# sauloal/pykmer

Measured on AMD Instinct MI355X. Metric: bp/s k-mer counted (k=15, 1 GPU), higher is better.
Workload: dtype u8; 1 GPU; k=15 canonical k-mer count of one 800 Mbp synthetic genome per GPU (SURVEY 8d C2, seed 2+rank), 4^15 table resident in HBM; fasta_bytes=813333854, num_kmers=766212116, parallelism=1 independent genome(s)

## Files before the change

pykmer_amd/csrc/kmer_count.hip:

```cpp
#include "fasta_fsm.h"
#include "pk_kernels.h"

namespace pk {

constexpr int L2_WAVES = 7;

__global__ __launch_bounds__(WG) void k_chunk_l1(const uint8_t *__restrict__ fasta, uint64_t n_bytes, uint32_t n_chunks,
                                                 L1 *__restrict__ chunk_l1) {
    const uint32_t lane = threadIdx.x & 63u;
    const uint32_t chunk = blockIdx.x * (WG / 64) + (threadIdx.x >> 6);
    if (chunk >= n_chunks) return;
    const uint64_t base = (uint64_t)chunk * CHUNK;
    const uint32_t nb = (uint32_t)(n_bytes - base < (uint64_t)CHUNK ? n_bytes - base : (uint64_t)CHUNK);
    auto window = [&](uint32_t w) -> uint32_t {
        const uint32_t off = w * 256u + lane * 4u;
        if (off + 4u <= nb) return *reinterpret_cast<const uint32_t *>(fasta + base + off);
        uint32_t v = 0;
        for (uint32_t j = 0; off + j < nb && j < 4u; j++) v |= (uint32_t)fasta[base + off + j] << (8u * j);
        return v;
    };
    const uint32_t n_win = (nb + 255u) / 256u;
    int last_term = -1;
    for (int w = (int)n_win - 1; w >= 0 && last_term < 0; w--) {
        const uint32_t v = window((uint32_t)w);
        uint32_t tm = 0;
#pragma unroll
        for (uint32_t j = 0; j < 4; j++) tm |= is_term((v >> (8u * j)) & 0xffu) ? (1u << j) : 0u;
        const unsigned long long any = __ballot(tm != 0u);
        if (any) {
            const int hl = 63 - __builtin_clzll(any);
            const uint32_t tmh = (uint32_t)__builtin_amdgcn_readlane((int)tm, hl);
            last_term = w * 256 + hl * 4 + (31 - __builtin_clz(tmh));
        }
    }
    const uint32_t from = (uint32_t)(last_term + 1);
    uint32_t state = LS_START;
    bool found = false;
    for (uint32_t w = from / 256u; w < n_win && !found; w++) {
        const uint32_t v = window(w);
        uint32_t nz = 0;
#pragma unroll
        for (uint32_t j = 0; j < 4; j++) {
            const uint32_t idx = w * 256u + lane * 4u + j;
            nz |= (idx >= from && idx < nb && !is_ws((v >> (8u * j)) & 0xffu)) ? (1u << j) : 0u;
        }
        const unsigned long long any = __ballot(nz != 0u);
        if (any) {
            const int ll = __builtin_ctzll(any);
            const uint32_t m = (uint32_t)__builtin_amdgcn_readlane((int)nz, ll);
            const uint32_t word = (uint32_t)__builtin_amdgcn_readlane((int)v, ll);
            const uint32_t c = (word >> (8u * (uint32_t)__builtin_ctz(m))) & 0xffu;
            state = c == '>' ? (uint32_t)LS_HEADER : (uint32_t)LS_SEQ;
            found = true;
        }
    }
    if (lane == 0) chunk_l1[chunk] = nb ? l1_make(last_term >= 0, state) : 0u;
}

__global__ __launch_bounds__(WG, L2_WAVES) void k_chunk_l2(const uint8_t *__restrict__ fasta, uint64_t n_bytes,
                                                 const L1 *__restrict__ chunk_l1_state, L2 *__restrict__ chunk_l2,
                                                 LaneState *__restrict__ lane_state, PiecePack *__restrict__ packs,
                                                 uint32_t *__restrict__ chunk_odd, uint32_t km1) {
    __shared__ __attribute__((aligned(16))) uint8_t lds[WG * LDS_STRIDE];
    __shared__ L1 sh1[WG / 64];
    __shared__ L2 sh2[WG / 64];
    __shared__ uint16_t queue[WG];
    __shared__ uint32_t n_queued[2], n_header_pieces;
    __shared__ uint32_t res1[WG];
    __shared__ uint8_t ls_of[WG];
    const uint64_t base = (uint64_t)blockIdx.x * CHUNK;
    if (threadIdx.x < 2) n_queued[threadIdx.x] = 0;
    if (threadIdx.x == 2) n_header_pieces = 0;
    stage_chunk(fasta, base, n_bytes, lds);
    __syncthreads();
    const uint32_t nb = piece_len(base, n_bytes);
    const uint8_t *mine = lds + threadIdx.x * LDS_STRIDE;
    PieceMasks pm;
    PiecePack pk;
    uint32_t cw[4];
    piece_scan(mine, nb, pm, cw);
    const bool full = nb == (uint32_t)PIECE;
    const bool plain = (pm.blank | pm.gt) == 0ull;
    {
        const unsigned long long S = ~pm.term;
        piece_compact(pm.valid, S & ~pm.valid, cw, plain, (uint32_t)__popcll(S), (S & 1ull) != 0ull, pk);
        uint4 *dst = reinterpret_cast<uint4 *>(packs + (uint64_t)blockIdx.x * WG + threadIdx.x);
        dst[0] = make_uint4((uint32_t)pk.c_lo, (uint32_t)(pk.c_lo >> 32), (uint32_t)pk.c_hi, (uint32_t)(pk.c_hi >> 32));
        dst[1] = make_uint4((uint32_t)pk.restart, (uint32_t)(pk.restart >> 32), pk.meta, 0u);
    }
    const bool masks1 = full && lines_start_plain(pm);
    L1 my1 = l1_of_piece(pm);
    bool dirty = !plain;
    const bool q1 = !masks1;
    if (q1) queue[atomicAdd(&n_queued[0], 1u)] = (uint16_t)threadIdx.x;
    __syncthreads();
    for (uint32_t q0 = (threadIdx.x >> 6) * 64u; q0 < n_queued[0]; q0 += WG) {
        const uint32_t qi = q0 + (threadIdx.x & 63u);
        const bool work = qi < n_queued[0];
        const uint32_t pc = work ? queue[qi] : 0u;
        bool d;
        const L1 r = piece_l1_at(lds + pc * LDS_STRIDE, work ? piece_len_of(pc, base, n_bytes) : 0u, d);
        if (work) res1[pc] = r | (d ? 0x100u : 0u);
    }
    __syncthreads();
    if (q1) { my1 = res1[threadIdx.x] & 0xffu; dirty = (res1[threadIdx.x] >> 8) & 1u; }
    L1 tot1;
    const L1 st1 = wg_excl_scan_l1(my1, chunk_l1_state[blockIdx.x], sh1, &tot1);
    const uint32_t ls_in = l1_kind(st1);
    ls_of[threadIdx.x] = (uint8_t)ls_in;
    const bool clean = !dirty && ls_in != LS_HEADER;
    bool header_piece = false;
    unsigned long long H = 0;
    if (__any(!clean && masks1)) {
        H = header_text(pm, ls_in);
        header_piece = !clean && masks1 && first_byte_plain(pm, ls_in) && (pm.blank & ~H) == 0ull;
    }
    L2 my2 = l2_identity();
    if (clean) my2 = l2_of_clean_piece(pm, pk, nb, ls_in, km1);
    if (__any(header_piece)) {
        const unsigned long long seq = ~pm.term & ~H, valid = pm.valid & seq;
        PiecePack hk;
        piece_compact(header_piece ? valid : 0ull, header_piece ? ((seq & ~valid) | H) : 0ull, cw, true, 0u, false, hk);
        if (header_piece)
            my2 = l2_of_masks(pm.term, valid, (seq & ~valid) | H, seq, (uint32_t)__popcll(header_starts(pm, ls_in)), hk, nb, ls_in, km1);
    }
    const bool q2 = !clean && !header_piece;
    if (q2) queue[atomicAdd(&n_queued[1], 1u)] = (uint16_t)threadIdx.x;
    const unsigned long long hp_wave = __ballot(header_piece);
    if ((threadIdx.x & 63u) == 0u && hp_wave) atomicAdd(&n_header_pieces, (uint32_t)__popcll(hp_wave));
    __syncthreads();
    for (uint32_t q0 = (threadIdx.x >> 6) * 64u; q0 < n_queued[1]; q0 += WG) {
        const uint32_t qi = q0 + (threadIdx.x & 63u);
        const bool work = qi < n_queued[1];
        const uint32_t pc = work ? queue[qi] : 0u;
        const L2 r = piece_l2_at(lds + pc * LDS_STRIDE, work ? piece_len_of(pc, base, n_bytes) : 0u, ls_of[pc], km1);
        if (work) {
            uint32_t *out = reinterpret_cast<uint32_t *>(lds + pc * LDS_STRIDE);
            out[0] = r.flags; out[1] = r.bits; out[2] = r.rec; out[3] = (uint32_t)r.p_tail;
        }
    }
    __syncthreads();
    if (q2) {
        const uint32_t *in = reinterpret_cast<const uint32_t *>(mine);
        my2.flags = in[0]; my2.bits = in[1]; my2.rec = in[2]; my2.p_tail = in[3];
    }
    L2 total;
    const L2 rel = wg_excl_scan_l2(my2, l2_identity(), sh2, &total, km1);
    lane_state[(uint64_t)blockIdx.x * WG + threadIdx.x] = lane_state_pack(rel, ls_in, q2, header_piece);
    if (threadIdx.x == 0) {
        chunk_l2[blockIdx.x] = total;
        chunk_odd[blockIdx.x] = n_queued[1] + n_header_pieces;
    }
}

constexpr int SCAN_T = 1024;

template <typename S, class Compose, class Shfl>
__device__ __forceinline__ S tile_scan(const S &mine, const S &seed, S *sh, S *total, Compose compose, Shfl shfl_up1) {
    const int lane = threadIdx.x & 63, w = threadIdx.x >> 6;
    S inc = mine;
#pragma unroll
    for (int d = 1; d < 64; d <<= 1) {
        S o = shfl_up1(inc, d);
        if (lane >= d) inc = compose(o, inc);
    }
    if (lane == 63) sh[w] = inc;
    __syncthreads();
    S pre = seed, tot = seed;
    for (int j = 0; j < SCAN_T / 64; j++) { if (j == w) pre = tot; tot = compose(tot, sh[j]); }
    *total = tot;
    S up = shfl_up1(inc, 1);
    return lane == 0 ? pre : compose(pre, up);
}

__global__ __launch_bounds__(SCAN_T) void k_scan_l1_reduce(const L1 *__restrict__ in, uint32_t n, L1 *__restrict__ tile_tot) {
    __shared__ L1 sh[SCAN_T / 64];
    const uint32_t i = blockIdx.x * SCAN_T + threadIdx.x;
    L1 tot;
    tile_scan<L1>(i < n ? in[i] : 0u, 0u, sh, &tot, [](L1 a, L1 b) { return l1_compose(a, b); }, [](L1 v, int d) { return (L1)__shfl_up(v, d, 64); });
    if (threadIdx.x == 0) tile_tot[blockIdx.x] = tot;
}
__global__ __launch_bounds__(SCAN_T) void k_scan_l1_tiles(L1 *__restrict__ tile_tot, uint32_t n_tiles, Carry *carry, uint32_t *__restrict__ zero_words,
                                                          uint32_t n_zero) {
    __shared__ L1 sh[SCAN_T / 64];
    if (threadIdx.x < n_zero) zero_words[threadIdx.x] = 0u;
    L1 run = carry->l1;
    for (uint32_t t0 = 0; t0 < n_tiles; t0 += SCAN_T) {
        const uint32_t i = t0 + threadIdx.x;
        L1 tot;
        L1 ex = tile_scan<L1>(i < n_tiles ? tile_tot[i] : 0u, run, sh, &tot, [](L1 a, L1 b) { return l1_compose(a, b); },
                              [](L1 v, int d) { return (L1)__shfl_up(v, d, 64); });
        if (i < n_tiles) tile_tot[i] = ex;
        run = tot;
        __syncthreads();
    }
    if (threadIdx.x == 0) carry->l1 = run;
}
__global__ __launch_bounds__(SCAN_T) void k_scan_l1_apply(const L1 *__restrict__ in, uint32_t n, const L1 *__restrict__ tile_seed,
                                                          L1 *__restrict__ out_state) {
    __shared__ L1 sh[SCAN_T / 64];
    const uint32_t i = blockIdx.x * SCAN_T + threadIdx.x;
    L1 tot;
    L1 ex = tile_scan<L1>(i < n ? in[i] : 0u, tile_seed[blockIdx.x], sh, &tot, [](L1 a, L1 b) { return l1_compose(a, b); },
                          [](L1 v, int d) { return (L1)__shfl_up(v, d, 64); });
    if (i < n) out_state[i] = ex;
}

__global__ __launch_bounds__(SCAN_T) void k_scan_l2_reduce(const L2 *__restrict__ in, uint32_t n, L2 *__restrict__ tile_tot, uint32_t km1) {
    __shared__ L2 sh[SCAN_T / 64];
    const uint32_t i = blockIdx.x * SCAN_T + threadIdx.x;
    L2 tot;
    tile_scan<L2>(i < n ? in[i] : l2_identity(), l2_identity(), sh, &tot, [km1](const L2 &a, const L2 &b) { return l2_compose(a, b, km1); },
                  [](const L2 &v, int d) { return shfl_up_l2(v, d); });
    if (threadIdx.x == 0) tile_tot[blockIdx.x] = tot;
}
__global__ __launch_bounds__(SCAN_T) void k_scan_l2_tiles(L2 *__restrict__ tile_tot, uint32_t n_tiles, Carry *carry, uint32_t km1) {
    __shared__ L2 sh[SCAN_T / 64];
    L2 run = carry->l2;
    for (uint32_t t0 = 0; t0 < n_tiles; t0 += SCAN_T) {
        const uint32_t i = t0 + threadIdx.x;
        L2 tot;
        L2 ex = tile_scan<L2>(i < n_tiles ? tile_tot[i] : l2_identity(), run, sh, &tot,
                              [km1](const L2 &a, const L2 &b) { return l2_compose(a, b, km1); }, [](const L2 &v, int d) { return shfl_up_l2(v, d); });
        if (i < n_tiles) tile_tot[i] = ex;
        run = tot;
        __syncthreads();
    }
    if (threadIdx.x == 0) { carry->l2 = run; carry->n_recs = run.rec; if (km1 > 16u) carry->deep_in = carry->deep_out; }
}
__global__ __launch_bounds__(SCAN_T) void k_scan_l2_apply(const L2 *__restrict__ in, uint32_t n, const L2 *__restrict__ tile_seed,
                                                          L2 *__restrict__ out_state, uint32_t km1) {
    __shared__ L2 sh[SCAN_T / 64];
    const uint32_t i = blockIdx.x * SCAN_T + threadIdx.x;
    L2 tot;
    L2 ex = tile_scan<L2>(i < n ? in[i] : l2_identity(), tile_seed[blockIdx.x], sh, &tot,
                          [km1](const L2 &a, const L2 &b) { return l2_compose(a, b, km1); }, [](const L2 &v, int d) { return shfl_up_l2(v, d); });
    if (i < n) out_state[i] = ex;
}

__global__ __launch_bounds__(WG) void k_hist(const uint8_t *__restrict__ src, uint64_t n, unsigned long long *__restrict__ hist ) {
    __shared__ uint32_t h[WG / 64][256];
    for (int i = threadIdx.x; i < (WG / 64) * 256; i += WG) (&h[0][0])[i] = 0;
    __syncthreads();
    uint32_t *myh = h[threadIdx.x >> 6];
    uint64_t ones = 0;
    const uint64_t n16 = n / 16;
    for (uint64_t g = (uint64_t)blockIdx.x * WG + threadIdx.x; g < n16; g += (uint64_t)gridDim.x * WG) {
        const uint4 a = reinterpret_cast<const uint4 *>(src)[g];
        const uint32_t t[4] = {a.x, a.y, a.z, a.w};
#pragma unroll
        for (int j = 0; j < 16; j++) {
            const uint32_t v = (t[j >> 2] >> (8 * (j & 3))) & 0xffu;
            if (v == 1u) ones++;
            else if (v) atomicAdd(&myh[v], 1u);
        }
    }
    if (blockIdx.x == 0) {
        for (uint64_t i = n16 * 16 + threadIdx.x; i < n; i += WG) {
            const uint32_t x = src[i];
            if (x == 1u) ones++;
            else if (x) atomicAdd(&myh[x], 1u);
        }
    }
    for (int d = 32; d; d >>= 1) ones += __shfl_down((unsigned long long)ones, d, 64);
    if ((threadIdx.x & 63) == 0 && ones) atomicAdd(&hist[1], (unsigned long long)ones);
    __syncthreads();
    for (int b = threadIdx.x; b < 256; b += WG) {
        unsigned long long s = 0;
        for (int w = 0; w < WG / 64; w++) s += h[w][b];
        if (s) atomicAdd(&hist[b], s);
    }
}

void launch_chunk_l1(const uint8_t *fasta, uint64_t n, L1 *chunk_l1, uint32_t n_chunks, hipStream_t s) {
    hipLaunchKernelGGL(k_chunk_l1, dim3((n_chunks + WG / 64 - 1) / (WG / 64)), dim3(WG), 0, s, fasta, n, n_chunks, chunk_l1);
}
void launch_scan_l1(const L1 *in, uint32_t n_chunks, Carry *carry, L1 *out, L1 *tile_ws, PartSignals *zeroed, hipStream_t s) {
    static_assert(sizeof(PartSignals) % 4 == 0 && sizeof(PartSignals) / 4 <= SCAN_T, "k_scan_l1_tiles zeroes one word per thread");
    const uint32_t n_tiles = (n_chunks + SCAN_T - 1) / SCAN_T;
    hipLaunchKernelGGL(k_scan_l1_reduce, dim3(n_tiles), dim3(SCAN_T), 0, s, in, n_chunks, tile_ws);
    hipLaunchKernelGGL(k_scan_l1_tiles, dim3(1), dim3(SCAN_T), 0, s, tile_ws, n_tiles, carry, (uint32_t *)zeroed, (uint32_t)(sizeof(PartSignals) / 4));
    hipLaunchKernelGGL(k_scan_l1_apply, dim3(n_tiles), dim3(SCAN_T), 0, s, in, n_chunks, (const L1 *)tile_ws, out);
}
void launch_chunk_l2(const uint8_t *fasta, uint64_t n, const L1 *st1, L2 *chunk_l2, LaneState *lane_state, PiecePack *packs, uint32_t *chunk_odd, uint32_t n_chunks,
                     uint32_t k, hipStream_t s) {
    hipLaunchKernelGGL(k_chunk_l2, dim3(n_chunks), dim3(WG), 0, s, fasta, n, st1, chunk_l2, lane_state, packs, chunk_odd, k - 1);
}
void launch_scan_l2(const L2 *in, uint32_t n_chunks, Carry *carry, L2 *out, L2 *tile_ws, uint32_t k, hipStream_t s) {
    const uint32_t n_tiles = (n_chunks + SCAN_T - 1) / SCAN_T;
    hipLaunchKernelGGL(k_scan_l2_reduce, dim3(n_tiles), dim3(SCAN_T), 0, s, in, n_chunks, tile_ws, k - 1);
    hipLaunchKernelGGL(k_scan_l2_tiles, dim3(1), dim3(SCAN_T), 0, s, tile_ws, n_tiles, carry, k - 1);
    hipLaunchKernelGGL(k_scan_l2_apply, dim3(n_tiles), dim3(SCAN_T), 0, s, in, n_chunks, (const L2 *)tile_ws, out, k - 1);
}
static uint32_t stream_grid(uint64_t items_per_thread_units) {
    uint64_t g = (items_per_thread_units + WG - 1) / WG;
    if (g > 256u * 8u) g = 256u * 8u;
    if (g == 0) g = 1;
    return (uint32_t)g;
}
void launch_hist8(const uint8_t *table8, uint64_t n, unsigned long long *hist, hipStream_t s) {
    hipLaunchKernelGGL(k_hist, dim3(stream_grid(n / 16 + 1)), dim3(WG), 0, s, table8, n, hist);
}

}
```

pykmer_amd/csrc/kmer_fuse.hip:

```cpp
#include "part_common.h"

namespace pk {

__device__ __forceinline__ uint32_t smear_up(uint32_t x, uint32_t n) {
    const uint32_t y1 = x | (x << 1), y2 = y1 | (y1 << 2), y3 = y2 | (y2 << 4);
    if (n >= 16u) return y3 | (y3 << 8);
    uint32_t acc = 0, off = 0;
    if (n & 8u) { acc |= y3; off = 8; }
    if (n & 4u) { acc |= y2 << off; off += 4; }
    if (n & 2u) { acc |= y1 << off; off += 2; }
    if (n & 1u) { acc |= x << off; }
    return acc;
}

__device__ __forceinline__ unsigned long long bases_before_slot(const uint32_t *__restrict__ codes, const uint32_t *__restrict__ n_bases, uint32_t c,
                                                                const unsigned long long *__restrict__ stream_before) {
    unsigned long long before = 0;
    uint32_t have = 0;
    for (uint32_t cc = c; cc > 0 && have < 32u;) {
        cc--;
        const uint32_t n_cc = n_bases[cc];
        const uint32_t take = min(n_cc, 32u - have);
        if (take == 0) continue;
        const uint32_t p0 = n_cc - take, d0 = p0 >> 4, sh = 2u * (p0 & 15u);
        const uint32_t *pw = codes + (uint64_t)cc * SLOT_CODE_WORDS;
        const unsigned long long w01 = ((unsigned long long)pw[min(d0 + 1u, SLOT_CODE_WORDS - 1u)] << 32) | pw[d0];
        const unsigned long long w2 = pw[min(d0 + 2u, SLOT_CODE_WORDS - 1u)];
        unsigned long long x = sh ? ((w01 >> sh) | (w2 << (64u - sh))) : w01;
        if (take < 32u) x &= (1ull << (2u * take)) - 1ull;
        before |= x << (2u * (32u - have - take));
        have += take;
    }
    if (have < 32u) before |= *stream_before >> (2u * have);
    return before;
}

__global__ void k_deep_tail(const uint32_t *__restrict__ codes, const uint32_t *__restrict__ n_bases, uint32_t n_chunks,
                            const unsigned long long *__restrict__ before_in, unsigned long long *__restrict__ before_out,
                            const uint32_t *__restrict__ flags) {
    if (threadIdx.x != 0 || flags[0]) return;
    *before_out = bases_before_slot(codes, n_bases, n_chunks, before_in);
}

template <typename KT, bool COUNT, int NT, int PER, int NB, uint32_t HS, bool SLICED, bool DEEP, uint32_t KC = 0>
__global__ __launch_bounds__(NT, 4) void k_walk_sort(const uint32_t *__restrict__ codes, const uint32_t *__restrict__ restarts,
                                                  const uint32_t *__restrict__ n_bases, const L2 *__restrict__ chunk_l2_state,
                                                  PartPlan pl, uint32_t n_items, uint32_t stride, void *__restrict__ out,
                                                  uint32_t *__restrict__ cursor1, const uint32_t *__restrict__ cap_end, uint32_t dump,
                                                  uint32_t *__restrict__ flags, uint32_t tally_shift, uint32_t n_tally,
                                                  uint32_t *__restrict__ tally_rows, unsigned long long *__restrict__ side,
                                                  unsigned long long *__restrict__ side_n, uint64_t side_cap,
                                                  const unsigned long long *__restrict__ deep_before) {
    static_assert(NT * PER == TILE && PER % 16 == 0, "one slot per workgroup");
    static_assert(!DEEP || (PER == 16 && sizeof(KT) == 8 && SLICED), "deep windows: 64-bit k-mers, one code dword per thread, sliced table");
    constexpr int NW = PER / 16;
    constexpr bool WIDE = sizeof(KT) == 8;
    extern __shared__ __attribute__((aligned(16))) uint8_t smem[];
    ScatterLdsT<NB> &L = *reinterpret_cast<ScatterLdsT<NB> *>(smem);
    uint32_t *tally = reinterpret_cast<uint32_t *>(smem);
    __shared__ HotTable<COUNT ? 2u : HS> hot;
    const uint32_t k = KC ? KC : pl.k, km1 = k - 1;
    if (COUNT && flags[0]) return;
    if (COUNT) {
        for (uint32_t i = threadIdx.x; i < n_tally; i += NT) tally[i] = 0u;
    } else {
        for (uint32_t i = threadIdx.x; i < HS; i += NT) { hot.key[i] = 0ull; hot.val[i] = 0u; }
        if (threadIdx.x == 0) { hot.used = 0; L.pad_[1] = flags[0]; }
        for (uint32_t i = threadIdx.x; i < NB; i += NT) { L.hist[i] = 0; L.run[i] = 0; }
    }
    const uint32_t B = KC == 17 ? 512u : pl.B1, shift = KC == 17 ? 25u : pl.addr_bits - pl.b1;
    const uint32_t low_mask = shift >= 32 ? 0xffffffffu : ((1u << shift) - 1u);
    const bool out16 = KC == 17 ? false : pl.b2 == 0;
    const KT mask = (KT)((2u * k >= sizeof(KT) * 8u) ? ~(KT)0 : (((KT)1 << (2u * k)) - 1));
    const KT local_mask = (KT)((pl.addr_bits >= sizeof(KT) * 8u) ? ~(KT)0 : (((KT)1 << pl.addr_bits) - 1));
    uint32_t t = threadIdx.x;
    __syncthreads();
    if (!COUNT && L.pad_[1]) return;
    const uint32_t i_lo = COUNT ? blockIdx.x : blockIdx.x * pl.G1, i_hi = COUNT ? n_items : min(i_lo + pl.G1, n_items);
    const uint32_t i_step = COUNT ? gridDim.x : 1u;
    struct Fetched { uint32_t nb, prev0, pprev0, r_here, r_before, st_flags, st_bits, cur[NW]; };
    auto fetch = [&](uint32_t c, uint32_t t, Fetched &f) {
        const uint32_t *cw = codes + (uint64_t)c * SLOT_CODE_WORDS;
        const uint32_t *rw = restarts + (uint64_t)c * SLOT_RST_WORDS;
        f.nb = n_bases[c];
#pragma unroll
        for (int w = 0; w < NW; w++) f.cur[w] = cw[NW * t + w];
        f.prev0 = cw[t ? NW * t - 1 : 0];
        f.pprev0 = cw[NW * t > 1 ? NW * t - 2 : 0];
        const uint32_t ri = NW == 2 ? t : (t >> 1);
        f.r_here = rw[ri];
        f.r_before = rw[ri ? ri - 1 : 0];
        f.st_flags = chunk_l2_state[c].flags;
        f.st_bits = chunk_l2_state[c].bits;
    };
    Fetched nxt;
    auto settle = [&]() {
        __builtin_amdgcn_s_waitcnt(0x0F70);
        asm volatile("" : "+v"(nxt.nb), "+v"(nxt.prev0), "+v"(nxt.pprev0), "+v"(nxt.r_here), "+v"(nxt.r_before), "+v"(nxt.st_flags), "+v"(nxt.st_bits));
#pragma unroll
        for (int w = 0; w < NW; w++) asm volatile("" : "+v"(nxt.cur[w]));
    };
    auto locate = [&](uint32_t it, uint32_t &c, uint32_t &tt) -> bool {
        if (!COUNT) { c = it; tt = threadIdx.x; return true; }
        constexpr uint32_t WPW = NT / 64;
        const uint64_t g = (uint64_t)it * WPW + (threadIdx.x >> 6);
        const uint64_t q = stride == 1u ? g : g * stride + g % stride;
        c = (uint32_t)(q / WPW); tt = (uint32_t)(q % WPW) * 64u + (threadIdx.x & 63u);
        return q / WPW < pl.n_chunks;
    };
    uint32_t c_n = 0, t_n = threadIdx.x;
    bool ok_n = false;
    if (i_lo < i_hi) { ok_n = locate(i_lo, c_n, t_n); if (ok_n) fetch(c_n, t_n, nxt); }
    settle();
    for (uint32_t it = i_lo; it < i_hi; it += i_step) {
        const Fetched me = nxt;
        const uint32_t c = c_n;
        const bool ok = ok_n;
        if (COUNT) t = t_n;
        if (it + i_step < i_hi) { ok_n = locate(it + i_step, c_n, t_n); if (ok_n) fetch(c_n, t_n, nxt); }
        if (COUNT && !ok) { settle(); continue; }
        const uint32_t nb = (uint32_t)__builtin_amdgcn_readfirstlane((int)me.nb);
        if (nb == 0) { settle(); continue; }
        const bool live = (uint32_t)PER * t < nb;
        uint32_t cur[NW], prev0 = me.prev0, rbits[NW];
#pragma unroll
        for (int w = 0; w < NW; w++) { cur[w] = live ? me.cur[w] : 0u; rbits[w] = 0; }
        if (NW == 2) {
            rbits[0] = (me.r_here << 16) | (me.r_before >> 16);
            rbits[NW - 1] = me.r_here;
        } else {
            rbits[0] = (t & 1u) ? me.r_here : ((me.r_here << 16) | (me.r_before >> 16));
        }
        uint32_t pprev0 = me.pprev0;
        bool have_pp[NW];
        if (NW == 2) {
            have_pp[0] = t != 0 && ((me.r_before >> 13) & 7u) == 0u;
            have_pp[NW - 1] = t != 0 && ((me.r_before >> 29) & 7u) == 0u;
        } else {
            const unsigned long long rb = ((((unsigned long long)me.r_here) << 32) | me.r_before) >> (16u * (t & 1u));
            have_pp[0] = t > 1 && (((uint32_t)rb >> 13) & 7u) == 0u;
        }
        unsigned long long rb64 = 0;
        if (!DEEP) {
            if (t == 0) {
                const uint32_t len = (me.st_flags >> 8) & 0xffu;
                prev0 = revpairs32(me.st_bits);
                rbits[0] &= 0xffff0000u;
                if (len < km1) rbits[0] |= 1u << (16u - len);
            }
        } else {
            uint32_t r_before = me.r_before;
            if (t < 2) {
                const uint32_t len = (me.st_flags >> 8) & 0xffu;
                unsigned long long before = (unsigned long long)revpairs32(me.st_bits) << 32;
                if (len > 16u) before = bases_before_slot(codes, n_bases, c, deep_before);
                const uint32_t va = (uint32_t)(before >> 32), vb = (uint32_t)before;
                if (t == 0) { prev0 = va; pprev0 = vb; } else { pprev0 = va; }
                r_before = (len != 0u && len < km1) ? (1u << (32u - len)) : 0u;
            }
            rb64 = ((((unsigned long long)me.r_here) << 32) | r_before) >> (16u * (t & 1u));
        }
        const uint32_t n_mine = live ? min((uint32_t)PER, nb - (uint32_t)PER * t) : 0u;

        KT r[PER];
        uint32_t okm = 0;
#pragma unroll
        for (int w = 0; w < NW; w++) {
            const uint32_t prev = w ? cur[w ? w - 1 : 0] : prev0;
            const uint32_t cnt = n_mine > 16u * w ? min(16u, n_mine - 16u * w) : 0u;
            uint32_t has_x;
            if (DEEP) {
                const unsigned long long y1 = rb64 | (rb64 << 1), y2 = y1 | (y1 << 2), y3 = y2 | (y2 << 4), y4 = y3 | (y3 << 8);
                unsigned long long acc = 0;
                uint32_t off = 0;
                if (km1 & 16u) { acc |= y4; off = 16; }
                if (km1 & 8u) { acc |= y3 << off; off += 8; }
                if (km1 & 4u) { acc |= y2 << off; off += 4; }
                if (km1 & 2u) { acc |= y1 << off; }
                has_x = (uint32_t)(acc >> 16);
            } else {
                has_x = smear_up(rbits[w], km1);
            }
            const uint32_t hasmask = ~(has_x >> 16) & ((1u << cnt) - 1u);
            const uint32_t fprev = revpairs32(prev), fcur = revpairs32(cur[w]);
            const unsigned long long fwd64 = ((unsigned long long)fprev << 32) | fcur;
            const uint32_t fpp = DEEP ? revpairs32(pprev0) : 0u;
            unsigned long long rev64;
            uint32_t rev_top = 0;
            if (DEEP) {
                const uint32_t pre = 2u * (33u - k);
                const unsigned long long lo = ~(((unsigned long long)prev << 32) | pprev0);
                const uint32_t top = ~cur[w];
                rev64 = (lo >> pre) | ((unsigned long long)top << (64u - pre));
                rev_top = top >> pre;
            } else {
                rev64 = (~(((unsigned long long)cur[w] << 32) | prev)) >> (2u * (17u - k));
            }
            const uint32_t rlo = (uint32_t)rev64, rhi = (uint32_t)(rev64 >> 32);
            const unsigned long long B64 = ((unsigned long long)cur[w] << 32) | prev;
            const uint32_t pp = w ? prev0 : pprev0;
            auto repeats = [&](uint32_t p, uint32_t xr) -> uint32_t {
                const unsigned long long x = B64 ^ ((B64 << (2u * p)) | (pp >> (32u - 2u * p)));
                const unsigned long long m = ~(x | (x >> 1)) & 0x5555555555555555ull & (have_pp[w] ? ~0ull : ~((1ull << (2u * p)) - 1ull));
                const unsigned long long a1 = m & (m << 2), a2 = a1 & (a1 << 4), a3 = a2 & (a2 << 8);
                unsigned long long acc = ~0ull;
                uint32_t off = 0;
                if (k & 16u) { acc &= a3 & (a3 << 16); off = 16; }
                if (k & 8u) { acc &= a3 << (2u * off); off += 8; }
                if (k & 4u) { acc &= a2 << (2u * off); off += 4; }
                if (k & 2u) { acc &= a1 << (2u * off); off += 2; }
                if (k & 1u) { acc &= m << (2u * off); }
                uint32_t e = (uint32_t)(acc >> 32);
                e = (e | (e >> 1)) & 0x33333333u; e = (e | (e >> 2)) & 0x0f0f0f0fu; e = (e | (e >> 4)) & 0x00ff00ffu; e = (e | (e >> 8)) & 0xffffu;
                return e & ~xr & hasmask;
            };
            const uint32_t x1 = has_x | (has_x << 1), x2 = x1 | (x1 << 1), x3 = x2 | (x2 << 1);
            const uint32_t d1 = repeats(1, x1 >> 16);
            const uint32_t d2 = repeats(2, x2 >> 16) & ~d1;
            const uint32_t d3 = repeats(3, x3 >> 16) & ~d1 & ~d2;
            const uint32_t dup = d1 | d2 | d3;
            uint32_t emit = hasmask & ~dup, in_slice = 0;
#pragma unroll
            for (int j = 0; j < 16; j++) {
                KT f, rv;
                if (sizeof(KT) == 4) {
                    f = (KT)__builtin_amdgcn_alignbit(fprev, fcur, 2u * (15u - j)) & mask;
                    rv = (KT)__builtin_amdgcn_alignbit(rhi, rlo, 2u * j) & mask;
                } else if (!DEEP) {
                    f = (KT)(fwd64 >> (2u * (15u - j))) & mask;
                    rv = (KT)(rev64 >> (2u * j)) & mask;
                } else {
                    f = (KT)((fwd64 >> (2u * (15u - j))) | (j < 15 ? ((unsigned long long)fpp << (64u - 2u * (15u - j))) : 0ull)) & mask;
                    rv = (KT)((rev64 >> (2u * j)) | (j > 0 ? ((unsigned long long)rev_top << (64u - 2u * j)) : 0ull)) & mask;
                }
                KT canon = f < rv ? f : rv;
                bool has = true;
                if (SLICED) {
                    has = (uint32_t)((unsigned long long)canon >> pl.addr_bits) == pl.slice_index;
                    canon &= local_mask;
                }
                r[16 * w + j] = canon;
                if (SLICED) in_slice |= has ? (1u << j) : 0u;
            }
            if (SLICED) emit &= in_slice;
            okm |= emit << (16 * w);
            if (!COUNT && __any(dup != 0u)) {
                uint32_t left = SLICED ? (dup & in_slice) : dup;
                while (left) {
                    const uint32_t q = (uint32_t)__builtin_ctz(left);
                    const uint32_t p = ((d1 >> q) & 1u) ? 1u : (((d2 >> q) & 1u) ? 2u : 3u);
                    const uint32_t dp = p == 1u ? d1 : (p == 2u ? d2 : d3);
                    uint32_t cls = 0;
                    for (uint32_t x = q; x < 16u && ((dp >> x) & 1u); x += p) cls |= 1u << x;
                    unsigned long long fq = fwd64 >> (2u * (15u - q)), rq = rev64 >> (2u * q);
                    if (DEEP) {
                        if (q < 15u) fq |= (unsigned long long)fpp << (64u - 2u * (15u - q));
                        if (q > 0u) rq |= (unsigned long long)rev_top << (64u - 2u * q);
                    }
                    const KT kf = (KT)fq & mask, kr = (KT)rq & mask;
                    KT key = kf < kr ? kf : kr;
                    if (SLICED) key &= local_mask;
                    hot_insert(hot, (uint64_t)key, (uint32_t)__builtin_popcount(SLICED ? (cls & in_slice) : cls), side, side_n, side_cap);
                    left &= ~cls;
                }
            }
        }
        if (COUNT) {
#pragma unroll
            for (int j = 0; j < PER; j++)
                if ((okm >> j) & 1u) atomicAdd(&tally[(uint32_t)((uint64_t)r[j] >> tally_shift)], 1u);
            settle();
            continue;
        }
        uint8_t *out_hi = (!WIDE && !out16) ? reinterpret_cast<uint8_t *>(out) + level1_hi_plane_offset(pl.capacity1) : nullptr;
        bool hot_full = false;
        scatter_tile<KT, WIDE, NT, PER, NB, false, (WIDE ? 0 : 8), !WIDE>(L, r, okm, ~0u, shift, B, low_mask, out16, out, settle, cursor1, cap_end, dump, flags, out_hi,
                                                                         &hot.used, HS / 2, &hot_full);
        if (hot_full) hot_flush(hot, side, side_n, side_cap);
    }
    if (COUNT) {
        __syncthreads();
        for (uint32_t i = threadIdx.x; i < n_tally; i += NT) tally_rows[(uint64_t)blockIdx.x * n_tally + i] = tally[i];
        return;
    }
    hot_flush(hot, side, side_n, side_cap);
}

__device__ __forceinline__ uint32_t block_excl_scan_1024(uint32_t v, uint32_t *wsum, uint32_t &total) {
    const int lane = threadIdx.x & 63, w = threadIdx.x >> 6;
    uint32_t inc = v;
#pragma unroll
    for (int d = 1; d < 64; d <<= 1) { uint32_t o = __shfl_up(inc, d, 64); if (lane >= d) inc += o; }
    __syncthreads();
    if (lane == 63) wsum[w] = inc;
    __syncthreads();
    uint32_t pre = 0;
    total = 0;
    for (int i = 0; i < 16; i++) { if (i < w) pre += wsum[i]; total += wsum[i]; }
    return pre + inc - v;
}

__device__ __forceinline__ uint32_t room_for(unsigned long long h, double scale, uint32_t stride, uint32_t slack) {
    if (stride == 1) return (uint32_t)h;
    const unsigned long long est = (unsigned long long)((double)h * scale) + 1ull;
    return (uint32_t)(est + est / 8 + slack);
}

constexpr int PROV_ROWS = 32;
__global__ __launch_bounds__(1024) void k_provision(const uint32_t *__restrict__ tot, uint32_t n_tally, PartPlan pl, uint32_t n_sampled,
                                                    uint32_t stride, uint32_t *__restrict__ bucket_base, uint32_t *__restrict__ cursor1,
                                                    uint32_t *__restrict__ cap_end, uint32_t *__restrict__ final_start,
                                                    uint32_t *__restrict__ cursor2, uint32_t *__restrict__ cap2_end, uint32_t *flags) {
    __shared__ uint32_t wsum[16];
    __shared__ unsigned long long sum1[512];
    if (flags[0]) return;
    const uint32_t B1 = pl.B1;
    const bool two = n_tally > B1;
    const double scale = (double)pl.n_chunks / (double)n_sampled;
    const uint32_t lane = threadIdx.x & 63u, w = threadIdx.x >> 6;
    for (uint32_t i = threadIdx.x; i < 512; i += 1024) sum1[i] = 0ull;
    __syncthreads();
    const uint32_t seg = (((n_tally + 15u) / 16u) + 63u) & ~63u;
    const uint32_t rows = seg / 64u;
    uint32_t h[PROV_ROWS], room[PROV_ROWS];
#pragma unroll
    for (int r = 0; r < PROV_ROWS; r++) {
        const uint32_t i = w * seg + (uint32_t)r * 64u + lane;
        h[r] = ((uint32_t)r < rows && i < n_tally) ? tot[i] : 0u;
    }
    uint32_t wave_total = 0;
#pragma unroll
    for (int r = 0; r < PROV_ROWS; r++) {
        room[r] = 0;
        if ((uint32_t)r < rows) {
            const uint32_t i = w * seg + (uint32_t)r * 64u + lane;
            const bool in = i < n_tally;
            if (two && pl.b2 >= 6u) {
                const uint32_t row = (uint32_t)__builtin_amdgcn_readlane((int)wave_incl_scan_u32(in ? h[r] : 0u), 63);
                if (lane == 0 && row) atomicAdd(&sum1[i >> pl.b2], (unsigned long long)row);
            } else if (in && h[r]) atomicAdd(&sum1[two ? (i >> pl.b2) : i], (unsigned long long)h[r]);
            if (two) {
                const uint32_t mine = in ? ((room_for(h[r], scale, stride, 2048u) + 7u) & ~7u) : 0u;
                const uint32_t inc = wave_incl_scan_u32(mine);
                room[r] = mine;
                h[r] = wave_total + inc - mine;
                wave_total += (uint32_t)__builtin_amdgcn_readlane((int)inc, 63);
            }
        }
    }
    if (two) {
        if (lane == 0) wsum[w] = wave_total;
        __syncthreads();
        uint32_t pre = 0, total2 = 0;
        for (uint32_t i = 0; i < 16; i++) { if (i < w) pre += wsum[i]; total2 += wsum[i]; }
#pragma unroll
        for (int r = 0; r < PROV_ROWS; r++) {
            const uint32_t i = w * seg + (uint32_t)r * 64u + lane;
            if ((uint32_t)r < rows && i < n_tally) {
                const uint32_t a = pre + h[r];
                final_start[i] = a; cursor2[i] = a; cap2_end[i] = a + room[r];
            }
        }
        if (threadIdx.x == 0) {
            final_start[n_tally] = total2;
            if ((uint64_t)total2 > pl.capacity2) flags[0] = 1u;
        }
    }
    __syncthreads();
    uint32_t room1 = 0;
    if (threadIdx.x < B1) room1 = (room_for(sum1[threadIdx.x], scale, stride, 4096u) + 3u) & ~3u;
    uint32_t total1;
    const uint32_t base = block_excl_scan_1024(room1, wsum, total1);
    if (threadIdx.x < B1) { bucket_base[threadIdx.x] = base; cursor1[threadIdx.x] = base; cap_end[threadIdx.x] = base + room1; }
    if (threadIdx.x == 0) {
        bucket_base[B1] = total1;
        if ((uint64_t)total1 > pl.capacity1) flags[0] = 1u;
    }
}

__global__ __launch_bounds__(1024) void k_level1_finish(const uint32_t *__restrict__ cursor1, const uint32_t *__restrict__ bucket_base,
                                                        const uint32_t *__restrict__ cap_end, PartPlan pl, uint32_t *__restrict__ bucket_end,
                                                        uint32_t *__restrict__ wg2_start, const uint32_t *__restrict__ flags) {
    __shared__ uint32_t wsum[16];
    if (flags[0]) return;
    const uint32_t d = threadIdx.x, B1 = pl.B1;
    if (d < B1) bucket_end[d] = min(cursor1[d], cap_end[d]);
    if (B1 >= 8u) {
        const uint32_t per = B1 >> 3;
        uint32_t g2 = 0;
        if (d < B1) {
            const uint32_t b = (d % per) * 8u + d / per;
            const uint32_t size2 = min(cursor1[b], cap_end[b]) - bucket_base[b];
            g2 = (uint32_t)(((uint64_t)size2 + pl.R2 - 1) / pl.R2);
        }
        uint32_t sum_g2;
        const uint32_t ps = block_excl_scan_1024(g2, wsum, sum_g2);
        if (d < B1) wg2_start[d] = ps;
        if (d == 0) wg2_start[B1] = sum_g2;
    }
}

__global__ __launch_bounds__(256) void k_tally_sum(const uint32_t *__restrict__ rows, uint32_t n_rows, uint32_t n_cols, uint32_t *__restrict__ tot) {
    const uint32_t col = blockIdx.x * 256u + threadIdx.x;
    if (col >= n_cols) return;
    uint32_t acc[16] = {0, 0, 0, 0, 0, 0, 0, 0, 0, 0, 0, 0, 0, 0, 0, 0};
    uint32_t r = 0;
    for (; r + 16 <= n_rows; r += 16) {
#pragma unroll
        for (int u = 0; u < 16; u++) acc[u] += rows[(uint64_t)(r + u) * n_cols + col];
    }
    for (; r < n_rows; r++) acc[0] += rows[(uint64_t)r * n_cols + col];
    uint32_t sum = 0;
#pragma unroll
    for (int u = 0; u < 16; u++) sum += acc[u];
    tot[col] = sum;
}

typedef ScatterLdsT<128> FuseLdsNarrow;
constexpr size_t FUSE_LDS_NARROW = offsetof(FuseLdsNarrow, dig);

#define PK_WS_NARROW(COUNT, SLICED) k_walk_sort<uint32_t, COUNT, 512, 32, 128, 512, SLICED, false>
#define PK_WS_K15(COUNT) k_walk_sort<uint32_t, COUNT, 512, 32, 128, 512, false, false, 15>
#define PK_WS_K17(COUNT) k_walk_sort<uint64_t, COUNT, 1024, 16, 512, 1024, false, false, 17>
#define PK_WS_WIDE(COUNT, SLICED) k_walk_sort<uint64_t, COUNT, 1024, 16, 512, 1024, SLICED, false>
#define PK_WS_DEEP(COUNT) k_walk_sort<uint64_t, COUNT, 1024, 16, 512, 1024, true, true>

void fuse_set_attributes() {
    auto set = [](const void *f, size_t bytes) { hipFuncSetAttribute(f, hipFuncAttributeMaxDynamicSharedMemorySize, (int)bytes); };
    set((const void *)PK_WS_NARROW(false, false), FUSE_LDS_NARROW); set((const void *)PK_WS_NARROW(false, true), FUSE_LDS_NARROW);
    set((const void *)PK_WS_NARROW(true, false), 131072); set((const void *)PK_WS_NARROW(true, true), 131072);
    set((const void *)PK_WS_K15(false), FUSE_LDS_NARROW); set((const void *)PK_WS_K15(true), 131072);
    set((const void *)PK_WS_K17(false), SCATTER_LDS_WIDE); set((const void *)PK_WS_K17(true), 65536);
    set((const void *)PK_WS_WIDE(false, false), SCATTER_LDS_WIDE); set((const void *)PK_WS_WIDE(false, true), SCATTER_LDS_WIDE);
    set((const void *)PK_WS_WIDE(true, false), 65536); set((const void *)PK_WS_WIDE(true, true), 65536);
    set((const void *)PK_WS_DEEP(false), SCATTER_LDS_WIDE); set((const void *)PK_WS_DEEP(true), 65536);
}

template <bool COUNT, typename... Args>
static void launch_ws(const PartPlan &pl, uint32_t grid, size_t lds, hipStream_t s, Args... args) {
    const bool sliced = pl.slice_bits != 0;
    if (pl.k > 17) hipLaunchKernelGGL((PK_WS_DEEP(COUNT)), dim3(grid), dim3(1024), lds, s, args...);
    else if (pl.k > 15) {
        if (sliced) hipLaunchKernelGGL((PK_WS_WIDE(COUNT, true)), dim3(grid), dim3(1024), lds, s, args...);
        else if (pl.k == 17 && pl.b1 == 9) hipLaunchKernelGGL((PK_WS_K17(COUNT)), dim3(grid), dim3(1024), lds, s, args...);
        else hipLaunchKernelGGL((PK_WS_WIDE(COUNT, false)), dim3(grid), dim3(1024), lds, s, args...);
    } else {
        if (sliced) hipLaunchKernelGGL((PK_WS_NARROW(COUNT, true)), dim3(grid), dim3(512), lds, s, args...);
        else if (pl.k == 15 && pl.b1 == 7) hipLaunchKernelGGL((PK_WS_K15(COUNT)), dim3(grid), dim3(512), lds, s, args...);
        else hipLaunchKernelGGL((PK_WS_NARROW(COUNT, false)), dim3(grid), dim3(512), lds, s, args...);
    }
}

void launch_provision(const PartPlan &pl, const PartBuffers &b, const L2 *st2, uint32_t stride, const Carry *carry, hipStream_t s) {
    const uint32_t n_sampled = (pl.n_chunks + stride - 1) / stride;
    const uint32_t grid = n_sampled < COUNT_WGS ? n_sampled : COUNT_WGS;
    const uint32_t n_tally = pl.n_tally;
    const uint32_t tally_shift = n_tally > pl.B1 ? pl.fb_bits : pl.addr_bits - pl.b1;
    launch_ws<true>(pl, grid, (size_t)n_tally * 4, s, b.codes, b.restarts, b.n_bases, st2, pl, n_sampled, stride, (void *)nullptr, (uint32_t *)nullptr,
                    (const uint32_t *)nullptr, 0u, b.flags, tally_shift, n_tally, b.tally_rows, (unsigned long long *)nullptr,
                    (unsigned long long *)nullptr, (uint64_t)0, (const unsigned long long *)&carry->deep_in);
    hipLaunchKernelGGL(k_tally_sum, dim3((n_tally + 255u) / 256u), dim3(256), 0, s, (const uint32_t *)b.tally_rows, grid, n_tally, b.tally_tot);
    hipLaunchKernelGGL(k_provision, dim3(1), dim3(1024), 0, s, (const uint32_t *)b.tally_tot, n_tally, pl, n_sampled, stride, b.bucket_base, b.cursor1,
                       b.cap_end, b.final_start, b.cursor2, b.cap2_end, b.flags);
}

void launch_walk_sort(const PartPlan &pl, const PartBuffers &b, const L2 *st2, const Carry *carry, hipStream_t s) {
    const uint32_t dump = (uint32_t)pl.capacity1;
    launch_ws<false>(pl, pl.n_wg1, pl.k > 15 ? SCATTER_LDS_WIDE : FUSE_LDS_NARROW, s, b.codes, b.restarts, b.n_bases, st2, pl, pl.n_chunks, 1u, b.out1,
                     b.cursor1, (const uint32_t *)b.cap_end, dump, b.flags, 0u, 0u, (uint32_t *)nullptr, b.side, b.side_n, b.side_cap,
                     (const unsigned long long *)&carry->deep_in);
    hipLaunchKernelGGL(k_level1_finish, dim3(1), dim3(1024), 0, s, (const uint32_t *)b.cursor1, (const uint32_t *)b.bucket_base,
                       (const uint32_t *)b.cap_end, pl, b.bucket_end, b.wg2_start, (const uint32_t *)b.flags);
}

void launch_deep_tail(const PartPlan &pl, const PartBuffers &b, Carry *carry, hipStream_t s) {
    hipLaunchKernelGGL(k_deep_tail, dim3(1), dim3(64), 0, s, (const uint32_t *)b.codes, (const uint32_t *)b.n_bases, pl.n_chunks,
                       (const unsigned long long *)&carry->deep_in, (unsigned long long *)&carry->deep_out, (const uint32_t *)b.flags);
}

}
```

pykmer_amd/csrc/kmer_part.hip:

```cpp
#include <cstddef>
#include <string>
#include <type_traits>
#include "../../include/pykmer_hip.h"
#include "part_common.h"

namespace pk {

int set_error(int code, const std::string &msg);

__global__ __launch_bounds__(1024) void k_sample2(const uint32_t *__restrict__ in, const uint32_t *__restrict__ bucket_base,
                                                  const uint32_t *__restrict__ bucket_end, PartPlan pl, uint32_t stride2,
                                                  uint32_t *__restrict__ tally, uint32_t *__restrict__ sampled_n,
                                                  const uint32_t *__restrict__ flags) {
    __shared__ uint32_t h[512];
    __shared__ uint32_t n_seen;
    if (flags[0]) return;
    const uint32_t b = blockIdx.x, lo = bucket_base[b], hi = bucket_end[b];
    if (threadIdx.x < 512) h[threadIdx.x] = 0;
    if (threadIdx.x == 0) n_seen = 0;
    __syncthreads();
    const uint32_t n_grp = (hi - lo + 255u) / 256u, n_sgrp = (n_grp + stride2 - 1u) / stride2;
    const uint32_t mask = pl.B2 - 1u, shift = pl.fb_bits, w = threadIdx.x >> 6, lane = threadIdx.x & 63u;
    uint32_t mine = 0;
    for (uint32_t s0 = 0; s0 < n_sgrp; s0 += 8u * 16u) {
        uint4 v[8];
        uint32_t n_ok[8];
#pragma unroll
        for (int u = 0; u < 8; u++) {
            const uint32_t sg = s0 + (uint32_t)u * 16u + w;
            const uint64_t i = (uint64_t)lo + (uint64_t)sg * stride2 * 256u + lane * 4u;
            n_ok[u] = (sg < n_sgrp && i < hi) ? (uint32_t)min((uint64_t)4, (uint64_t)hi - i) : 0u;
            v[u] = n_ok[u] ? *reinterpret_cast<const uint4 *>(in + i) : make_uint4(0, 0, 0, 0);
        }
#pragma unroll
        for (int u = 0; u < 8; u++) {
            const uint32_t r4[4] = {v[u].x, v[u].y, v[u].z, v[u].w};
#pragma unroll
            for (uint32_t e = 0; e < 4; e++)
                if (e < n_ok[u]) { atomicAdd(&h[(r4[e] >> shift) & mask], 1u); mine++; }
        }
    }
    for (int d = 32; d; d >>= 1) mine += __shfl_down(mine, d, 64);
    if ((threadIdx.x & 63) == 0 && mine) atomicAdd(&n_seen, mine);
    __syncthreads();
    if (threadIdx.x < pl.B2) tally[(uint64_t)b * pl.B2 + threadIdx.x] = h[threadIdx.x];
    if (threadIdx.x == 0) sampled_n[b] = n_seen;
}
__global__ __launch_bounds__(1024) void k_rooms2(const uint32_t *__restrict__ tally, const uint32_t *__restrict__ sampled_n,
                                                 const uint32_t *__restrict__ bucket_base, const uint32_t *__restrict__ bucket_end, PartPlan pl,
                                                 uint32_t stride2, uint32_t n_final, uint32_t *__restrict__ final_start,
                                                 uint32_t *__restrict__ cap2_end, uint32_t *__restrict__ block_tot, const uint32_t *__restrict__ flags) {
    __shared__ uint32_t wsum[16];
    if (flags[0]) return;
    const uint32_t i = blockIdx.x * 1024u + threadIdx.x;
    uint32_t room = 0;
    if (i < n_final) {
        const uint32_t b = i >> pl.b2, hcount = tally[i];
        if (stride2 == 1u) room = hcount;
        else {
            const uint32_t seen = sampled_n[b], n_b = bucket_end[b] - bucket_base[b];
            const unsigned long long est = seen ? (unsigned long long)((double)hcount * ((double)n_b / (double)seen)) + 1ull : 0ull;
            room = (uint32_t)(est + est / 4 + 4096u);
        }
        room = (room + 7u) & ~7u;
    }
    uint32_t inc = room;
    const int lane = threadIdx.x & 63, w = threadIdx.x >> 6;
#pragma unroll
    for (int d = 1; d < 64; d <<= 1) { const uint32_t o = __shfl_up(inc, d, 64); if (lane >= d) inc += o; }
    if (lane == 63) wsum[w] = inc;
    __syncthreads();
    uint32_t pre = 0, total = 0;
    for (int j = 0; j < 16; j++) { if (j < w) pre += wsum[j]; total += wsum[j]; }
    if (i < n_final) { final_start[i] = pre + inc - room; cap2_end[i] = room; }
    if (threadIdx.x == 0) block_tot[blockIdx.x] = total;
}
__global__ __launch_bounds__(1024) void k_bases2(uint32_t n_blocks, uint32_t n_final, PartPlan pl, uint32_t *__restrict__ block_tot,
                                                 uint32_t *__restrict__ final_start, uint32_t *__restrict__ flags) {
    __shared__ uint32_t wsum[16];
    if (flags[0]) return;
    const uint32_t v = threadIdx.x < n_blocks ? block_tot[threadIdx.x] : 0u;
    uint32_t inc = v;
    const int lane = threadIdx.x & 63, w = threadIdx.x >> 6;
#pragma unroll
    for (int d = 1; d < 64; d <<= 1) { const uint32_t o = __shfl_up(inc, d, 64); if (lane >= d) inc += o; }
    if (lane == 63) wsum[w] = inc;
    __syncthreads();
    uint32_t pre = 0, total = 0;
    for (int j = 0; j < 16; j++) { if (j < w) pre += wsum[j]; total += wsum[j]; }
    if (threadIdx.x < n_blocks) block_tot[threadIdx.x] = pre + inc - v;
    __shared__ unsigned long long total64;
    if (threadIdx.x == 0) total64 = 0ull;
    __syncthreads();
    unsigned long long mine = v;
    for (int d = 32; d; d >>= 1) mine += __shfl_down(mine, d, 64);
    if (lane == 0 && mine) atomicAdd(&total64, mine);
    __syncthreads();
    if (threadIdx.x == 0) {
        final_start[n_final] = total;
        if (total64 > pl.capacity2) flags[0] = 1u;
    }
}
__global__ __launch_bounds__(1024) void k_starts2(uint32_t n_final, const uint32_t *__restrict__ block_base, uint32_t *__restrict__ final_start,
                                                  uint32_t *__restrict__ cursor2, uint32_t *__restrict__ cap2_end, const uint32_t *__restrict__ flags) {
    if (flags[0]) return;
    const uint32_t i = blockIdx.x * 1024u + threadIdx.x;
    if (i >= n_final) return;
    const uint32_t a = block_base[blockIdx.x] + final_start[i];
    final_start[i] = a; cursor2[i] = a; cap2_end[i] = a + cap2_end[i];
}

template <int NT, int PER, bool REC24 = false>
__global__ __launch_bounds__(NT, 4) void k_scatter2(const uint32_t *__restrict__ in, const uint32_t *__restrict__ wg2_start,
                                                   const uint32_t *__restrict__ bucket_base, const uint32_t *__restrict__ bucket_end, PartPlan pl,
                                                   void *__restrict__ out, uint32_t *__restrict__ cursor, const uint32_t *__restrict__ cap_end,
                                                   uint32_t dump, uint32_t *__restrict__ flags) {
    extern __shared__ __attribute__((aligned(16))) uint8_t smem[];
    ScatterLds &L = *reinterpret_cast<ScatterLds *>(smem);
    if (flags[0]) return;
    const uint32_t B = pl.B2, shift = pl.fb_bits;
    const uint32_t low_mask = (1u << shift) - 1u;
    for (uint32_t i = threadIdx.x; i < 512; i += NT) { L.hist[i] = 0; L.run[i] = 0; }
    __syncthreads();
    typedef uint32_t Quad __attribute__((ext_vector_type(4)));
    typedef uint32_t Pair __attribute__((ext_vector_type(2)));
    const uint16_t *in_lo = reinterpret_cast<const uint16_t *>(in);
    const uint8_t *in_hi = reinterpret_cast<const uint8_t *>(in) + level1_hi_plane_offset(pl.capacity1);
    auto item = [&](uint32_t b, uint32_t lo, uint32_t hi) {
        auto fetch = [&](uint32_t win, Quad (&v)[PER / 4]) {
            const uint32_t v_hi = min(hi, win + (uint32_t)TILE);
#pragma unroll
            for (int j = 0; j < PER / 4; j++) {
                const uint32_t i = win + (threadIdx.x + j * NT) * 4u;
                v[j] = Quad{0u, 0u, 0u, 0u};
                if (i < v_hi) {
                    if (REC24) {
                        const Pair l = *reinterpret_cast<const Pair *>(in_lo + i);
                        v[j] = Quad{l.x, l.y, *reinterpret_cast<const uint32_t *>(in_hi + i), 0u};
                    } else v[j] = *reinterpret_cast<const Quad *>(in + i);
                }
            }
        };
        Quad nxt[PER / 4];
        auto settle = [&]() {
            __builtin_amdgcn_s_waitcnt(0x0F70);
#pragma unroll
            for (int j = 0; j < PER / 4; j++) asm volatile("" : "+v"(nxt[j]));
        };
        fetch(lo & ~3u, nxt);
        settle();
        for (uint32_t win = lo & ~3u; win < hi; win += TILE) {
            const uint32_t v_lo = max(lo, win), v_hi = min(hi, win + (uint32_t)TILE);
            const uint32_t n_tile = v_hi - v_lo;
            uint32_t r[PER];
#pragma unroll
            for (int j = 0; j < PER / 4; j++) {
                if (REC24) {
                    r[j * 4] = __builtin_amdgcn_perm(nxt[j].z, nxt[j].x, 0x0c040100u);
                    r[j * 4 + 1] = __builtin_amdgcn_perm(nxt[j].z, nxt[j].x, 0x0c050302u);
                    r[j * 4 + 2] = __builtin_amdgcn_perm(nxt[j].z, nxt[j].y, 0x0c060100u);
                    r[j * 4 + 3] = __builtin_amdgcn_perm(nxt[j].z, nxt[j].y, 0x0c070302u);
                } else { r[j * 4] = nxt[j].x; r[j * 4 + 1] = nxt[j].y; r[j * 4 + 2] = nxt[j].z; r[j * 4 + 3] = nxt[j].w; }
            }
            const bool full = v_lo == win && n_tile == (uint32_t)TILE;
            uint32_t okm = 0;
            if (!full) {
#pragma unroll
                for (int j = 0; j < PER / 4; j++) {
                    const uint32_t i = win + (threadIdx.x + j * NT) * 4u;
#pragma unroll
                    for (int e = 0; e < 4; e++) okm |= (i + e >= v_lo && i + e < v_hi) ? (1u << (j * 4 + e)) : 0u;
                }
            }
            if (win + TILE < hi) fetch(win + TILE, nxt);
            uint32_t *cl = cursor + (uint64_t)b * B;
            const uint32_t *ce = cap_end + (uint64_t)b * B;
            if (full) scatter_tile<uint32_t, false, NT, PER, 512, true, 8, REC24>(L, r, 0u, n_tile, shift, B, low_mask, true, out, settle, cl, ce, dump, flags);
            else scatter_tile<uint32_t, false, NT, PER, 512, false, 8, REC24>(L, r, okm, n_tile, shift, B, low_mask, true, out, settle, cl, ce, dump, flags);
        }
    };
    const uint32_t *pos = wg2_start;
    const uint32_t per = pl.B1 >> 3;
    const uint32_t o_lo = (blockIdx.x & 7u) * per, o_hi = o_lo + per, first = blockIdx.x >> 3, step = gridDim.x >> 3;
    const uint32_t w_end = pos[o_hi];
    for (uint32_t w = pos[o_lo] + first; w < w_end; w += step) {
        uint32_t a = o_lo, z = o_hi;
        while (z - a > 1) { const uint32_t m = (a + z) >> 1; if (pos[m] <= w) a = m; else z = m; }
        const uint32_t b = (a % per) * 8u + a / per;
        const uint64_t s = (uint64_t)bucket_base[b] + (uint64_t)(w - pos[a]) * pl.R2;
        const uint64_t e = min(s + pl.R2, (uint64_t)bucket_end[b]);
        item(b, (uint32_t)s, (uint32_t)e);
    }
}

constexpr uint32_t K6_PIECE = 65024;
constexpr int K6_BYTES_LDS = 65536 + 1024 + 128;

__device__ __forceinline__ int wave_sum_i32(int v) {
    v += __builtin_amdgcn_update_dpp(0, v, 0x128, 0xf, 0xf, false);
    v += __builtin_amdgcn_update_dpp(0, v, 0x124, 0xf, 0xf, false);
    v += __builtin_amdgcn_update_dpp(0, v, 0x122, 0xf, 0xf, false);
    v += __builtin_amdgcn_update_dpp(0, v, 0x121, 0xf, 0xf, false);
    return __builtin_amdgcn_readlane(v, 0) + __builtin_amdgcn_readlane(v, 16) + __builtin_amdgcn_readlane(v, 32) +
           __builtin_amdgcn_readlane(v, 48);
}

typedef unsigned short U16x2 __attribute__((ext_vector_type(2)));
__device__ __forceinline__ uint32_t clamp255_pair(uint32_t x) {
    const U16x2 lim = {255, 255};
    return __builtin_bit_cast(uint32_t, __builtin_elementwise_min(__builtin_bit_cast(U16x2, x), lim));
}
__device__ __forceinline__ uint32_t pack_low_bytes(uint32_t x0, uint32_t x1) {
    return __builtin_amdgcn_perm(x1, x0, 0x06040200u);
}

struct SliceTally {
    int d1 = 0, d2 = 0;
    __device__ __forceinline__ void add_dword(int *dh, uint32_t x, int sign) {
        uint32_t p0 = x & 0x01010101u, p1 = (x >> 1) & 0x01010101u;
        uint32_t rest = p0 & p1;
        const uint32_t high = x & 0xfcfcfcfcu;
        if (high) {
            const uint32_t big = (((high & 0x7f7f7f7fu) + 0x7f7f7f7fu) | high) & 0x80808080u;
            const uint32_t keep = ~(big >> 7);
            p0 &= keep; p1 &= keep;
            rest = (p0 & p1) | (big >> 7);
        }
        const int n1 = (int)__builtin_popcount(p0 & ~p1), n2 = (int)__builtin_popcount(p1 & ~p0);
        d1 += sign * n1; d2 += sign * n2;
        while (rest) {
            const int bit = __ffs(rest) - 1;
            atomicAdd(&dh[(x >> bit) & 0xffu], sign);
            rest &= rest - 1u;
        }
    }
};

template <int T, bool LEAN, bool NOREC = false>
__device__ __forceinline__ void bucket_count_body(const uint16_t *__restrict__ recs, const uint32_t *__restrict__ final_start,
                                                  const uint32_t *__restrict__ final_end, uint32_t fb_bits, uint32_t split_bits,
                                                  uint8_t *__restrict__ table8, uint32_t fresh, unsigned long long *__restrict__ hist_rep, uint8_t *smem,
                                                  int *dh, uint32_t wg) {
    uint32_t *cnt = reinterpret_cast<uint32_t *>(smem);
    const uint32_t fb = wg >> split_bits, part = wg & ((1u << split_bits) - 1u);
    const uint32_t start = final_start[fb], end = final_end ? final_end[fb] : final_start[fb + 1];
    const uint32_t part_bits = fb_bits - split_bits;
    const uint32_t n_addr = 1u << part_bits;
    uint8_t *slice = table8 + ((uint64_t)fb << fb_bits) + (uint64_t)part * n_addr;
    if (start == end) {
        if (fresh) {
            if (n_addr >= 16) for (uint32_t g = threadIdx.x; g < n_addr / 16; g += T) reinterpret_cast<uint4 *>(slice)[g] = make_uint4(0, 0, 0, 0);
            else for (uint32_t a = threadIdx.x; a < n_addr; a += T) slice[a] = 0;
        }
        return;
    }
    const uint32_t base = start & ~7u;
    const uint32_t i_first = base + threadIdx.x * 8;
    uint4 v_first = make_uint4(0, 0, 0, 0);
    if (i_first < min(base + K6_PIECE, end)) v_first = *reinterpret_cast<const uint4 *>(recs + i_first);
    const bool by_rec = NOREC ? false : (((end - start) >> split_bits) < n_addr / 4 || n_addr < 16);
    SliceTally tally;
    for (uint32_t i = threadIdx.x; i < 256; i += T) dh[i] = 0;
    if (fresh) {
        if (n_addr >= 8) for (uint32_t g = threadIdx.x; g < n_addr / 8; g += T) reinterpret_cast<uint4 *>(cnt)[g] = make_uint4(0, 0, 0, 0);
        else for (uint32_t a = threadIdx.x; a < max(n_addr / 2, 1u); a += T) cnt[a] = 0u;
    } else if (n_addr >= 16) {
        if (!by_rec) __syncthreads();
        for (uint32_t g = threadIdx.x; g < n_addr / 16; g += T) {
            uint4 v = reinterpret_cast<const uint4 *>(slice)[g];
            uint32_t w[4] = {v.x, v.y, v.z, v.w};
            if (!by_rec) {
#pragma unroll
                for (int q = 0; q < 4; q++) tally.add_dword(dh, w[q], -1);
            }
#pragma unroll
            for (int q = 0; q < 8; q++)
                cnt[g * 8 + q] = __builtin_amdgcn_perm(0u, w[q >> 1], (q & 1) ? 0x0c030c02u : 0x0c010c00u);
        }
    } else {
        for (uint32_t a = threadIdx.x; a < n_addr / 2; a += T) cnt[a] = slice[2 * a] | ((uint32_t)slice[2 * a + 1] << 16);
    }
    __syncthreads();
    auto bump = [&](uint32_t a, uint32_t n) {
        const uint32_t sh = 16u * (a & 1u);
        if (!by_rec) { atomicAdd(&cnt[a >> 1], n << sh); return; }
        int &d1 = tally.d1, &d2 = tally.d2;
        const uint32_t c = (atomicAdd(&cnt[a >> 1], n << sh) >> sh) & 0xffffu;
        const uint32_t oc = c > 255u ? 255u : c, nc = c + n > 255u ? 255u : c + n;
        if (oc == nc) return;
        if (nc == 1u) d1++;
        else if (nc == 2u && oc == 1u) { d2++; d1--; }
        else {
            atomicAdd(&dh[nc], 1);
            if (oc) atomicAdd(&dh[oc], -1);
        }
    };
    auto count8 = [&](const uint4 &v, uint32_t i) {
        const uint32_t w[4] = {v.x, v.y, v.z, v.w};
        if (LEAN && !by_rec) {
            const bool interior = i >= start && i + 8u <= end;
            uint8_t *cb = reinterpret_cast<uint8_t *>(cnt);
#pragma unroll
            for (int q = 0; q < 8; q++) {
                const uint32_t x = w[q >> 1];
                const uint32_t off = (q & 1) ? ((x >> 15) & 0x1fffcu) : ((x << 1) & 0x1fffcu);
                const uint32_t low = (q & 1) ? ((x >> 16) & 1u) : (x & 1u);
                uint32_t val = low * 0xffffu + 1u;
                if (!interior) val = (i + q >= start && i + q < end) ? val : 0u;
                __hip_atomic_fetch_add(reinterpret_cast<uint32_t *>(cb + off), val, __ATOMIC_RELAXED, __HIP_MEMORY_SCOPE_WORKGROUP);
            }
            return;
        }
        uint32_t pa = 0, pn = 0;
#pragma unroll
        for (int q = 0; q < 8; q++) {
            const uint32_t idx = i + q;
            const uint32_t full = (w[q >> 1] >> (16 * (q & 1))) & 0xffffu;
            const bool in = idx >= start && idx < end && (full >> part_bits) == part;
            const uint32_t a = full & (n_addr - 1u);
            if (in && pn && a == pa) pn++;
            else {
                if (pn) bump(pa, pn);
                pa = a; pn = in ? 1u : 0u;
            }
        }
        if (pn) bump(pa, pn);
    };
    auto count8_sparse = [&](const uint4 &v, uint32_t i) {
        const uint32_t w[4] = {v.x, v.y, v.z, v.w};
        uint32_t old[8];
        bool in[8];
        const bool interior = i >= start && i + 8u <= end;
#pragma unroll
        for (int q = 0; q < 8; q++) {
            const uint32_t idx = i + q;
            const uint32_t full = (w[q >> 1] >> (16 * (q & 1))) & 0xffffu;
            in[q] = (interior || (idx >= start && idx < end)) && (full >> part_bits) == part;
            const uint32_t a = full & (n_addr - 1u), sh = 16u * (a & 1u);
            old[q] = (atomicAdd(&cnt[a >> 1], in[q] ? (1u << sh) : 0u) >> sh) & 0xffffu;
        }
#pragma unroll
        for (int q = 0; q < 8; q++) {
            const uint32_t c = old[q];
            if (!in[q] || c >= 255u) continue;
            if (c == 0u) tally.d1++;
            else if (c == 1u) { tally.d2++; tally.d1--; }
            else { atomicAdd(&dh[c + 1u], 1); atomicAdd(&dh[c], -1); }
        }
    };
    constexpr int NIT = (K6_PIECE + T * 8 - 1) / (T * 8);
    if (end - base <= (uint32_t)T * 8u) {
        if (i_first < end) { if (by_rec) count8_sparse(v_first, i_first); else count8(v_first, i_first); }
        __syncthreads();
    } else {
        for (uint32_t p0 = base; p0 < end; p0 += K6_PIECE) {
            const uint32_t p1 = min(p0 + K6_PIECE, end);
            uint4 v[NIT];
#pragma unroll
            for (int it = 0; it < NIT; it++) {
                const uint32_t i = p0 + (threadIdx.x + it * T) * 8;
                v[it] = make_uint4(0, 0, 0, 0);
                if (i < p1) v[it] = (it == 0 && p0 == base) ? v_first : *reinterpret_cast<const uint4 *>(recs + i);
            }
#pragma unroll
            for (int it = 0; it < NIT; it++) {
                const uint32_t i = p0 + (threadIdx.x + it * T) * 8;
                if (i < p1) count8(v[it], i);
            }
            __syncthreads();
            if (p1 < end) {
                for (uint32_t a = threadIdx.x; a < max(n_addr / 2, 1u); a += T) {
                    cnt[a] = clamp255_pair(cnt[a]);
                }
                __syncthreads();
            }
        }
    }
    if (n_addr >= 16) {
        for (uint32_t g = threadIdx.x; g < n_addr / 16; g += T) {
            const uint4 c0 = reinterpret_cast<const uint4 *>(cnt)[g * 2], c1 = reinterpret_cast<const uint4 *>(cnt)[g * 2 + 1];
            const uint32_t o[4] = {pack_low_bytes(clamp255_pair(c0.x), clamp255_pair(c0.y)), pack_low_bytes(clamp255_pair(c0.z), clamp255_pair(c0.w)),
                                   pack_low_bytes(clamp255_pair(c1.x), clamp255_pair(c1.y)), pack_low_bytes(clamp255_pair(c1.z), clamp255_pair(c1.w))};
            if (!by_rec) {
#pragma unroll
                for (int q = 0; q < 4; q++) tally.add_dword(dh, o[q], 1);
            }
            reinterpret_cast<uint4 *>(slice)[g] = make_uint4(o[0], o[1], o[2], o[3]);
        }
    } else {
        for (uint32_t a = threadIdx.x; a < n_addr / 2; a += T) {
            uint32_t x = cnt[a], lo = x & 0xffffu, hi = x >> 16;
            slice[2 * a] = (uint8_t)(lo > 255u ? 255u : lo);
            slice[2 * a + 1] = (uint8_t)(hi > 255u ? 255u : hi);
        }
    }
    const int d1 = wave_sum_i32(tally.d1), d2 = wave_sum_i32(tally.d2);
    if ((threadIdx.x & 63) == 0) {
        if (d1) atomicAdd(&dh[1], d1);
        if (d2) atomicAdd(&dh[2], d2);
    }
    __syncthreads();
    for (uint32_t i = threadIdx.x; i < 256; i += T) {
        const int v = dh[i];
        if (v) atomicAdd(&hist_rep[(uint64_t)(blockIdx.x % HIST_REPLICAS) * 256 + i], (unsigned long long)(long long)v);
    }
}

template <int T>
__global__ __launch_bounds__(T) void k_bucket_count(const uint16_t *__restrict__ recs, const uint32_t *__restrict__ final_start,
                                                    const uint32_t *__restrict__ final_end, uint32_t fb_bits, uint32_t split_bits,
                                                    uint8_t *__restrict__ table8, uint32_t fresh, unsigned long long *__restrict__ hist_rep,
                                                    const uint32_t *__restrict__ flags) {
    extern __shared__ __attribute__((aligned(16))) uint8_t smem[];
    __shared__ int dh[256];
    if (flags[0]) return;
    bucket_count_body<T, true>(recs, final_start, final_end, fb_bits, split_bits, table8, fresh, hist_rep, smem, dh, blockIdx.x);
}
template <int T, bool FRESH>
__global__ __launch_bounds__(T) __attribute__((amdgpu_waves_per_eu(8, 8)))
void k_bucket_count_half_lean(const uint16_t *__restrict__ recs, const uint32_t *__restrict__ final_start, const uint32_t *__restrict__ final_end,
                              uint32_t fb_bits, uint32_t split_bits, uint8_t *__restrict__ table8, uint32_t fresh, unsigned long long *__restrict__ hist_rep,
                              const uint32_t *__restrict__ flags) {
    extern __shared__ __attribute__((aligned(16))) uint8_t smem[];
    __shared__ int dh[256];
    if (flags[0]) return;
    bucket_count_body<T, true, true>(recs, final_start, final_end, 15u, 0u, table8, FRESH ? 1u : 0u, hist_rep, smem, dh, blockIdx.x);
}

template <int T>
__global__ __launch_bounds__(T) __attribute__((amdgpu_waves_per_eu(8, 8)))
void k_bucket_count_bytes(const uint16_t *__restrict__ recs, const uint32_t *__restrict__ final_start, const uint32_t *__restrict__ final_end,
                          uint8_t *__restrict__ table8, uint32_t fresh, unsigned long long *__restrict__ hist_rep,
                          const uint32_t *__restrict__ flags) {
    extern __shared__ __attribute__((aligned(128))) uint8_t smem[];
    constexpr uint32_t N_ADDR = 65536u;
    int *dh = reinterpret_cast<int *>(smem + N_ADDR);
    uint32_t *wrap_flag = reinterpret_cast<uint32_t *>(smem + N_ADDR + 1024);
    if (flags[0]) return;
    const uint32_t fb = blockIdx.x;
    const uint32_t start = final_start[fb], end = final_end ? final_end[fb] : final_start[fb + 1];
    uint4 *slice = reinterpret_cast<uint4 *>(table8 + ((uint64_t)fb << 16));
    uint4 *img = reinterpret_cast<uint4 *>(smem);
    if (start == end) {
        if (fresh) for (uint32_t g = threadIdx.x; g < N_ADDR / 16; g += T) slice[g] = make_uint4(0, 0, 0, 0);
        return;
    }
    bool recount = end - start >= 16384u;
    int d1 = 0, d2 = 0;
    if (!recount) {
        const uint32_t base = start & ~7u;
        const uint32_t i_first = base + threadIdx.x * 8;
        uint4 v = make_uint4(0, 0, 0, 0);
        if (i_first < end) v = *reinterpret_cast<const uint4 *>(recs + i_first);
        for (uint32_t i = threadIdx.x; i < 256; i += T) dh[i] = 0;
        if (threadIdx.x == 0) *wrap_flag = 0u;
        if (fresh) { for (uint32_t g = threadIdx.x; g < N_ADDR / 16; g += T) img[g] = make_uint4(0, 0, 0, 0); }
        else { for (uint32_t g = threadIdx.x; g < N_ADDR / 16; g += T) img[g] = slice[g]; }
        __syncthreads();
        uint32_t *cnt = reinterpret_cast<uint32_t *>(smem);
        bool wrapped = false;
        for (uint32_t p0 = base; p0 < end; p0 += (uint32_t)T * 8u) {
            const uint32_t i = p0 + threadIdx.x * 8;
            if (i >= end) continue;
            if (p0 != base) v = *reinterpret_cast<const uint4 *>(recs + i);
            const uint32_t w[4] = {v.x, v.y, v.z, v.w};
            const bool interior = i >= start && i + 8u <= end;
            uint32_t old[8];
            bool in[8];
#pragma unroll
            for (int q = 0; q < 8; q++) {
                const uint32_t a = (w[q >> 1] >> (16 * (q & 1))) & 0xffffu, sh = 8u * (a & 3u);
                in[q] = interior || (i + q >= start && i + q < end);
                old[q] = (atomicAdd(&cnt[a >> 2], in[q] ? (1u << sh) : 0u) >> sh) & 0xffu;
            }
#pragma unroll
            for (int q = 0; q < 8; q++) {
                const uint32_t c = old[q];
                if (!in[q]) continue;
                if (c == 0u) d1++;
                else if (c == 1u) { d2++; d1--; }
                else if (c == 255u) wrapped = true;
                else { atomicAdd(&dh[c + 1u], 1); atomicAdd(&dh[c], -1); }
            }
        }
        if (wrapped) *wrap_flag = 1u;
        __syncthreads();
        recount = *wrap_flag != 0u;
        __syncthreads();
    }
    if (recount) {
        if (threadIdx.x == 0) atomicAdd(const_cast<uint32_t *>(&flags[1]), 1u);
        bucket_count_body<T, false>(recs, final_start, final_end, 16u, 1u, table8, fresh, hist_rep, smem, dh, 2u * fb);
        __syncthreads();
        bucket_count_body<T, false>(recs, final_start, final_end, 16u, 1u, table8, fresh, hist_rep, smem, dh, 2u * fb + 1u);
        return;
    }
    for (uint32_t g = threadIdx.x; g < N_ADDR / 16; g += T) slice[g] = img[g];
    d1 = wave_sum_i32(d1); d2 = wave_sum_i32(d2);
    if ((threadIdx.x & 63) == 0) {
        if (d1) atomicAdd(&dh[1], d1);
        if (d2) atomicAdd(&dh[2], d2);
    }
    __syncthreads();
    for (uint32_t i = threadIdx.x; i < 256; i += T) {
        const int x = dh[i];
        if (x) atomicAdd(&hist_rep[(uint64_t)(blockIdx.x % HIST_REPLICAS) * 256 + i], (unsigned long long)(long long)x);
    }
}

__device__ __forceinline__ void hist_reduce(unsigned long long *__restrict__ hist_rep, unsigned long long *__restrict__ hist) {
    if (threadIdx.x >= 256) return;
    unsigned long long acc = 0;
    for (uint32_t r = 0; r < HIST_REPLICAS; r++) {
        acc += hist_rep[(uint64_t)r * 256 + threadIdx.x];
        hist_rep[(uint64_t)r * 256 + threadIdx.x] = 0ull;
    }
    if (acc) atomicAdd(&hist[threadIdx.x], acc);
}

constexpr uint32_t AS_SLOTS = 4096, AS_WGS = 64;

__device__ __forceinline__ void table_sat_add(uint8_t *table8, uint64_t addr, uint32_t cnt, int *dh) {
    unsigned int *word = reinterpret_cast<unsigned int *>(table8 + (addr & ~3ull));
    const uint32_t sh = (uint32_t)(addr & 3ull) * 8u;
    unsigned int old = *word;
    while (true) {
        uint32_t b = (old >> sh) & 0xffu;
        uint32_t nb = b + cnt > 255u ? 255u : b + cnt;
        if (nb == b) return;
        unsigned int want = (old & ~(0xffu << sh)) | (nb << sh);
        unsigned int prev = atomicCAS(word, old, want);
        if (prev == old) {
            atomicAdd(&dh[nb], 1);
            if (b) atomicAdd(&dh[b], -1);
            return;
        }
        old = prev;
    }
}

__global__ __launch_bounds__(WG) void k_apply_side(const unsigned long long *__restrict__ side, const unsigned long long *__restrict__ side_n,
                                                   uint64_t side_cap, uint8_t *__restrict__ table8, unsigned long long *__restrict__ hist,
                                                   unsigned long long *__restrict__ hist_rep, const uint32_t *__restrict__ flags) {
    __shared__ unsigned long long key[AS_SLOTS];
    if (flags[0]) return;
    static_assert(WG >= 256, "one thread per histogram bin");
    if (blockIdx.x == 0) hist_reduce(hist_rep, hist);
    __shared__ uint32_t val[AS_SLOTS];
    __shared__ int dh[256];
    unsigned long long n = *side_n;
    if (n > side_cap) n = side_cap;
    const unsigned long long per = (n + gridDim.x - 1) / gridDim.x;
    const unsigned long long lo = per * blockIdx.x, hi = lo + per < n ? lo + per : n;
    if (lo >= hi) return;
    for (uint32_t i = threadIdx.x; i < AS_SLOTS; i += WG) { key[i] = 0ull; val[i] = 0u; }
    dh[threadIdx.x & 255u] = 0;
    __syncthreads();
    for (unsigned long long i = lo + threadIdx.x; i < hi; i += WG) {
        const unsigned long long e = side[i];
        const uint64_t addr = e >> SIDE_CNT_BITS;
        const uint32_t cnt = (uint32_t)(e & ((1ull << SIDE_CNT_BITS) - 1ull));
        const unsigned long long kk = addr + 1ull;
        uint32_t h = (uint32_t)((addr * 0x9E3779B97F4A7C15ull) >> 40) & (AS_SLOTS - 1u);
        bool done = false;
        for (uint32_t t = 0; t < 32 && !done; t++) {
            unsigned long long old = atomicCAS(&key[h], 0ull, kk);
            if (old == 0ull || old == kk) {
                uint32_t before = atomicAdd(&val[h], cnt);
                if (before + cnt < before) atomicExch(&val[h], 0xffffffffu);
                done = true;
            }
            h = (h + 1u) & (AS_SLOTS - 1u);
        }
        if (!done) table_sat_add(table8, addr, cnt > 255u ? 255u : cnt, dh);
    }
    __syncthreads();
    for (uint32_t i = threadIdx.x; i < AS_SLOTS; i += WG)
        if (key[i] != 0ull) table_sat_add(table8, key[i] - 1ull, val[i] > 255u ? 255u : val[i], dh);
    __syncthreads();
    if (threadIdx.x < 256 && dh[threadIdx.x]) atomicAdd(&hist[threadIdx.x], (unsigned long long)(long long)dh[threadIdx.x]);
}

PartPlan make_part_plan(uint32_t k, uint64_t n_bytes, uint32_t slice_bits, uint32_t slice_index) {
    PartPlan pl;
    pl.k = k;
    pl.slice_bits = slice_bits;
    pl.slice_index = slice_index;
    pl.addr_bits = 2 * k - slice_bits;
    pl.fb_bits = pl.addr_bits < 16 ? pl.addr_bits : 16;
    if (k <= 15 && pl.addr_bits >= 24 && n_bytes >= (((uint64_t)1 << pl.addr_bits) >> 3)) pl.fb_bits = 15;
    const uint32_t bucket_bits = pl.addr_bits - pl.fb_bits;
    const uint32_t one_level_max = k <= 15 ? 7u : 9u;
    pl.b1 = bucket_bits <= one_level_max ? bucket_bits : (bucket_bits + 1) / 2;
    if (pl.b1 > one_level_max) pl.b1 = one_level_max;
    pl.b2 = bucket_bits - pl.b1;
    pl.B1 = 1u << pl.b1;
    pl.B2 = 1u << pl.b2;
    pl.n_chunks = (uint32_t)((n_bytes + CHUNK - 1) / CHUNK);
    pl.n_wg0 = pl.n_chunks < 1024u ? pl.n_chunks : 1024u;
    if (pl.n_wg0 == 0) pl.n_wg0 = 1;
    pl.G = (pl.n_chunks + pl.n_wg0 - 1) / pl.n_wg0;
    if (pl.G == 0) pl.G = 1;
    const uint32_t wg1 = 4096u;
    pl.n_wg1 = pl.n_chunks < wg1 ? pl.n_chunks : wg1;
    if (pl.n_wg1 == 0) pl.n_wg1 = 1;
    pl.G1 = (pl.n_chunks + pl.n_wg1 - 1) / pl.n_wg1;
    if (pl.G1 == 0) pl.G1 = 1;
    pl.R2 = 4u * TILE;
    pl.sample_stride = pl.n_chunks >= 1024u ? 16u : 1u;
    const uint64_t nfb = (uint64_t)pl.B1 * pl.B2;
    pl.n_tally = (pl.b2 && nfb <= 32768 && pl.addr_bits <= 30) ? (uint32_t)nfb : pl.B1;
    pl.sample2 = (pl.b2 && pl.n_tally == pl.B1 && nfb <= 262144 && pl.B1 >= 8u) ? 1u : 0u;
    const uint64_t est1 = (uint64_t)pl.n_chunks * TILE + pl.B1, est2 = (uint64_t)pl.n_chunks * TILE + nfb;
    pl.capacity1 = est1 + est1 / 8 + (uint64_t)pl.B1 * 4100;
    pl.capacity2 = pl.sample2 ? est2 + est2 / 4 + nfb * 4104 : est2 + est2 / 8 + nfb * 2056;
    return pl;
}

static uint32_t bucket_split(const PartPlan &pl, uint64_t n_bytes) {
    return pl.fb_bits == 16 && n_bytes / ((uint64_t)pl.B1 * pl.B2) < 8192u ? 1u : 0u;
}

int part_plan_check(const PartPlan &pl, uint64_t n_bytes) {
    const auto no = [](const std::string &what) { return set_error(PK_ERR_HIP, "partition plan outside the kernels' limits: " + what); };
    const uint32_t max_B1 = pl.k <= 15 ? 128u : 512u;
    if (pl.B1 > max_B1 || pl.B2 > 512u || pl.fb_bits > 16u)
        return no(std::to_string(pl.B1) + " x " + std::to_string(pl.B2) + " buckets of 2^" + std::to_string(pl.fb_bits) + " addresses; the LDS arrays hold " +
                  std::to_string(max_B1) + " x 512 of 2^16");
    if (pl.b2 && pl.n_tally == pl.B1 && !pl.sample2) return no("two levels, but neither the sampling launch nor sample2 lays out the final buckets");
    if (pl.k <= 15 && pl.b2 && pl.addr_bits - pl.b1 > 24u)
        return no(std::to_string(pl.addr_bits - pl.b1) + " address bits behind the level-1 digit; its 3-byte records hold 24");
    if (bucket_split(pl, n_bytes) > 1u) return no("the bucket count is laid out for whole and half buckets");
    return PK_OK;
}

size_t part_workspace(const PartPlan &pl, uint64_t n_bytes, uint8_t *base, PartBuffers *view) {
    PartBuffers unused, &b = view ? *view : unused;
    const size_t nfb = (size_t)pl.B1 * pl.B2, rec1 = (size_t)(pl.capacity1 + TILE + 64);
    size_t o = 0;
    const auto place = [&](auto *&p, size_t bytes, bool packed = false) {
        p = reinterpret_cast<std::remove_reference_t<decltype(p)>>(reinterpret_cast<uintptr_t>(base) + o);
        o += bytes;
        if (!packed) o = (o + 255) & ~(size_t)255;
    };
    place(b.codes, (size_t)pl.n_chunks * SLOT_CODE_WORDS * 4);
    place(b.restarts, (size_t)pl.n_chunks * SLOT_RST_WORDS * 4);
    place(b.n_bases, (size_t)pl.n_chunks * 4);
    place(b.tally_rows, (size_t)COUNT_WGS * pl.n_tally * 4);
    const bool s2 = pl.sample2 != 0;
    place(b.tally_tot, (s2 ? nfb : pl.n_tally) * 4, s2);
    place(b.sampled_n, s2 ? (size_t)pl.B1 * 4 : 0, true);
    place(b.block_tot, s2 ? 1024 * 4 : 0);
    if (!s2) b.sampled_n = b.block_tot = nullptr;
    for (uint32_t **p : {&b.bucket_base, &b.bucket_end, &b.cursor1, &b.cap_end, &b.wg2_start}) place(*p, (size_t)(pl.B1 + 1) * 4);
    for (uint32_t **p : {&b.final_start, &b.cursor2, &b.cap2_end}) place(*p, (nfb + 1) * 4);
    place(b.out1, !pl.b2 ? rec1 * 2 : pl.k <= 15 ? level1_hi_plane_offset(pl.capacity1) + rec1 : rec1 * 4);
    place(b.out2, !pl.b2 ? 256 : (size_t)(pl.capacity2 + TILE + 64) * 2);
    b.side_cap = n_bytes + 16;
    place(b.side, (size_t)b.side_cap * 8);
    place(b.signals, sizeof(PartSignals));
    b.side_n = &b.signals->side_n;
    b.flags = b.signals->flags;
    return o;
}

void part_set_attributes() {
    fuse_set_attributes();
    hipFuncSetAttribute((const void *)k_scatter2<512, 32>, hipFuncAttributeMaxDynamicSharedMemorySize, (int)SCATTER_LDS_NARROW);
    hipFuncSetAttribute((const void *)k_scatter2<512, 32, true>, hipFuncAttributeMaxDynamicSharedMemorySize, (int)SCATTER_LDS_NARROW);
    hipFuncSetAttribute((const void *)k_bucket_count<1024>, hipFuncAttributeMaxDynamicSharedMemorySize, 128 * 1024);
    hipFuncSetAttribute((const void *)k_bucket_count_half_lean<1024, true>, hipFuncAttributeMaxDynamicSharedMemorySize, 128 * 1024);
    hipFuncSetAttribute((const void *)k_bucket_count_half_lean<1024, false>, hipFuncAttributeMaxDynamicSharedMemorySize, 128 * 1024);
    hipFuncSetAttribute((const void *)k_bucket_count_bytes<1024>, hipFuncAttributeMaxDynamicSharedMemorySize, K6_BYTES_LDS);
}

extern "C" int pk_diag_occupancy(int which) {
    int n = -1;
    hipError_t e = hipErrorInvalidValue;
    if (which == 0) e = hipOccupancyMaxActiveBlocksPerMultiprocessor(&n, (const void *)k_bucket_count<1024>, 1024, 128 * 1024);
    if (which == 1) e = hipOccupancyMaxActiveBlocksPerMultiprocessor(&n, (const void *)k_bucket_count_bytes<1024>, 1024, K6_BYTES_LDS);
    if (which == 2) e = hipOccupancyMaxActiveBlocksPerMultiprocessor(&n, (const void *)k_bucket_count_half_lean<1024, true>, 1024, 65536);
    if (which == 3) e = hipOccupancyMaxActiveBlocksPerMultiprocessor(&n, (const void *)k_scatter2<512, 32>, 512, SCATTER_LDS_NARROW);
    return e == hipSuccess ? n : -(int)e;
}

int launch_partitioned(const PartPlan &pl, const PartBuffers &b, const L2 *st2, uint64_t n_bytes, uint32_t stride, const Carry *carry, uint8_t *table8,
                       unsigned long long *hist, unsigned long long *hist_rep, bool fresh, const PartEvents &ev, hipStream_t s) {
    const uint32_t nfb = pl.B1 * pl.B2;
    const uint32_t *flags = b.flags;
    const char *failed = nullptr;
    hipError_t why = hipSuccess;
    const auto stage = [&](const char *name) { if (!failed && (why = hipGetLastError()) != hipSuccess) failed = name; };
    launch_provision(pl, b, st2, stride, carry, s);
    stage("bucket layout");
    hipEventRecord(ev.sort_begin, s);
    launch_walk_sort(pl, b, st2, carry, s);
    stage("level-1 sort");
    hipEventRecord(ev.sort_end, s);
    const uint16_t *final_recs = (const uint16_t *)b.out1;
    const uint32_t *k6_start = b.bucket_base, *k6_end = b.bucket_end;
    if (pl.sample2) {
        const uint32_t stride2 = stride == 1u ? 1u : 16u, n_blocks = (nfb + 1023u) / 1024u;
        const uint32_t *base1 = b.bucket_base, *end1 = b.bucket_end;
        hipLaunchKernelGGL(k_sample2, dim3(pl.B1), dim3(1024), 0, s, (const uint32_t *)b.out1, base1, end1, pl, stride2, b.tally_tot, b.sampled_n, flags);
        hipLaunchKernelGGL(k_rooms2, dim3(n_blocks), dim3(1024), 0, s, (const uint32_t *)b.tally_tot, (const uint32_t *)b.sampled_n, base1, end1, pl, stride2,
                           nfb, b.final_start, b.cap2_end, b.block_tot, flags);
        hipLaunchKernelGGL(k_bases2, dim3(1), dim3(1024), 0, s, n_blocks, nfb, pl, b.block_tot, b.final_start, b.flags);
        hipLaunchKernelGGL(k_starts2, dim3(n_blocks), dim3(1024), 0, s, nfb, (const uint32_t *)b.block_tot, b.final_start, b.cursor2, b.cap2_end, flags);
        stage("final-bucket rooms");
    }
    if (pl.b2) {
        const uint32_t grid2 = 4096u;
        hipLaunchKernelGGL((pl.k <= 15 ? &k_scatter2<512, 32, true> : &k_scatter2<512, 32>), dim3(grid2), dim3(512), SCATTER_LDS_NARROW, s,
                           (const uint32_t *)b.out1, b.wg2_start, b.bucket_base, b.bucket_end, pl, b.out2, b.cursor2, (const uint32_t *)b.cap2_end,
                           (uint32_t)pl.capacity2, b.flags);
        stage("level 2");
        final_recs = (const uint16_t *)b.out2; k6_start = b.final_start; k6_end = b.cursor2;
    }
    hipEventRecord(ev.part_end, s);
    const uint32_t split = bucket_split(pl, n_bytes);
    const size_t part_addrs = (size_t)1 << (pl.fb_bits - split);
    const size_t lds6 = part_addrs * 2 < 64 ? 64 : part_addrs * 2;
    const uint32_t n_rows6 = (uint32_t)(nfb << split);
    const auto count = [&](auto kernel, uint32_t grid, size_t lds, auto... geometry) {
        hipLaunchKernelGGL(kernel, dim3(grid), dim3(1024), lds, s, final_recs, k6_start, k6_end, geometry..., table8, fresh ? 1u : 0u, hist_rep, flags);
    };
    if (pl.fb_bits == 15 && fresh) count(k_bucket_count_half_lean<1024, true>, n_rows6, lds6, pl.fb_bits, split);
    else if (pl.fb_bits == 15) count(k_bucket_count_half_lean<1024, false>, n_rows6, lds6, pl.fb_bits, split);
    else if (split) count(k_bucket_count_bytes<1024>, nfb, K6_BYTES_LDS);
    else count(k_bucket_count<1024>, n_rows6, lds6, pl.fb_bits, split);
    stage("bucket count");
    hipLaunchKernelGGL(k_apply_side, dim3(AS_WGS), dim3(WG), 0, s, b.side, b.side_n, b.side_cap, table8, hist, hist_rep, flags);
    stage("side list");
    return failed ? set_error(PK_ERR_HIP, std::string("partition pipeline: the launch of the ") + failed + " failed: " + hipGetErrorString(why)) : PK_OK;
}

}
```

pykmer_amd/csrc/pk_api.hip:

```cpp
#include <hip/hip_runtime.h>

#include <algorithm>
#include <array>
#include <cstdarg>
#include <cstdio>
#include <cstdlib>
#include <cstring>
#include <functional>
#include <memory>
#include <mutex>
#include <string>
#include <thread>
#include <vector>

#include "../../include/pykmer_hip.h"
#include "pk_kernels.h"

using namespace pk;

static thread_local std::string g_err;

static int fail(int code, const char *fmt, ...) {
    char buf[512];
    va_list ap;
    va_start(ap, fmt);
    vsnprintf(buf, sizeof buf, fmt, ap);
    va_end(ap);
    g_err = buf;
    return code;
}

namespace pk { int set_error(int code, const std::string &msg) { g_err = msg; return code; } }

#define HIPCHK(expr)                                                                                          \
    do {                                                                                                      \
        hipError_t _e = (expr);                                                                               \
        if (_e != hipSuccess) return fail(PK_ERR_HIP, "%s failed: %s (%s:%d)", #expr, hipGetErrorString(_e), __FILE__, __LINE__); \
    } while (0)

extern "C" int pk_version(void) { return PK_ABI_VERSION; }

extern "C" int pk_last_error(char *buf, size_t n) {
    if (!buf || n == 0) return PK_ERR_ARG;
    snprintf(buf, n, "%s", g_err.c_str());
    return PK_OK;
}

extern "C" int pk_device_count(void) {
    int n = 0;
    if (hipGetDeviceCount(&n) != hipSuccess) return 0;
    return n;
}

extern "C" int pk_warm(int device) {
    HIPCHK(hipSetDevice(device));
    HIPCHK(hipFree(nullptr));
    pk::part_set_attributes();
    return PK_OK;
}

static int check_k(int k, int slice_bits = 0, int slice_index = 0) {
    if (k <= 0 || (k % 2) == 0) return fail(PK_ERR_ARG, "kmer_len must be positive and odd (tools.py:165-167), got %d", k);
    if (k > 21) return fail(PK_ERR_ARG, "kmer_len %d not supported by the device path (max 21)", k);
    if (slice_bits < 0 || slice_bits > 2 * k || slice_bits > 16) return fail(PK_ERR_ARG, "bad number of address slices for kmer_len %d", k);
    if (2 * k - slice_bits > 34)
        return fail(PK_ERR_ARG, "kmer_len %d needs a table of 4^%d bytes; one indexer holds 2^34 (16 GiB): count it in %d address slices "
                                "(pk_indexer_create_slice)", k, k, 1 << (2 * k - 34));
    if (slice_index < 0 || slice_index >= (1 << slice_bits)) return fail(PK_ERR_ARG, "slice index %d outside 0..%d", slice_index, (1 << slice_bits) - 1);
    return PK_OK;
}

namespace {
int reserve_exact(void **p, size_t *cap, size_t need) {
    if (need <= *cap) return PK_OK;
    if (*p) HIPCHK(hipFree(*p));
    *p = nullptr;
    *cap = 0;
    HIPCHK(hipMalloc(p, need));
    *cap = need;
    return PK_OK;
}

template <class T> struct DevBuf {
    T *p = nullptr;
    size_t bytes = 0;
    DevBuf() = default;
    DevBuf(DevBuf &&o) noexcept { swap(o); }
    DevBuf &operator=(DevBuf &&o) noexcept { swap(o); return *this; }
    ~DevBuf() { if (p) hipFree(p); }
    void swap(DevBuf &o) { std::swap(p, o.p); std::swap(bytes, o.bytes); }
    int reserve(size_t need) { return reserve_exact((void **)&p, &bytes, need); }
    int grow_keep(size_t need, hipStream_t s) {
        if (need <= bytes) return PK_OK;
        DevBuf larger;
        int rc = larger.reserve(need);
        if (rc) return rc;
        HIPCHK(hipMemsetAsync(larger.p, 0, need, s));
        if (bytes) HIPCHK(hipMemcpyAsync(larger.p, p, bytes, hipMemcpyDeviceToDevice, s));
        HIPCHK(hipStreamSynchronize(s));
        swap(larger);
        return PK_OK;
    }
};
}

namespace {
constexpr int MAX_DEVICES = 64;
constexpr size_t BOUNCE_HALF = 8u << 20;
constexpr int MAX_COPY_THREADS = 16;
struct Bouncer {
    std::mutex mu;
    int threads = 0;
    uint8_t *pinned[MAX_COPY_THREADS] = {};
    hipStream_t stream[MAX_COPY_THREADS] = {};
    hipEvent_t ev[MAX_COPY_THREADS][2] = {};
};
Bouncer g_bounce[MAX_DEVICES];

int bouncer_for(int device, Bouncer **out) {
    if (device < 0 || device >= MAX_DEVICES) return fail(PK_ERR_ARG, "device ordinal %d out of range", device);
    Bouncer &b = g_bounce[device];
    static std::mutex init_mu;
    std::lock_guard<std::mutex> init_lock(init_mu);
    if (!b.threads) {
        const char *env = getenv("PK_COPY_THREADS");
        int t = env ? atoi(env) : 8;
        t = std::max(1, std::min(t, MAX_COPY_THREADS));
        auto make = [&]() -> int {
            for (int i = 0; i < t; i++) {
                HIPCHK(hipHostMalloc((void **)&b.pinned[i], 2 * BOUNCE_HALF, hipHostMallocDefault));
                HIPCHK(hipStreamCreateWithFlags(&b.stream[i], hipStreamNonBlocking));
                HIPCHK(hipEventCreateWithFlags(&b.ev[i][0], hipEventDisableTiming));
                HIPCHK(hipEventCreateWithFlags(&b.ev[i][1], hipEventDisableTiming));
            }
            return PK_OK;
        };
        if (int rc = make()) {
            for (int i = 0; i < t; i++) {
                if (b.pinned[i]) hipHostFree(b.pinned[i]);
                if (b.stream[i]) hipStreamDestroy(b.stream[i]);
                for (auto &e : b.ev[i]) if (e) hipEventDestroy(e);
                b.pinned[i] = nullptr; b.stream[i] = nullptr; b.ev[i][0] = b.ev[i][1] = nullptr;
            }
            return rc;
        }
        b.threads = t;
    }
    *out = &b;
    return PK_OK;
}

int bounce_copy(void *dev, void *host, size_t n, bool to_device, int device) {
    if (n == 0) return PK_OK;
    HIPCHK(hipSetDevice(device));
    if (n < (4u << 20)) {
        HIPCHK(to_device ? hipMemcpy(dev, host, n, hipMemcpyHostToDevice) : hipMemcpy(host, dev, n, hipMemcpyDeviceToHost));
        return PK_OK;
    }
    Bouncer *b = nullptr;
    int rc = bouncer_for(device, &b);
    if (rc) return rc;
    std::lock_guard<std::mutex> lock(b->mu);
    const size_t n_pieces = (n + BOUNCE_HALF - 1) / BOUNCE_HALF;
    const int T = (int)std::min<size_t>((size_t)b->threads, n_pieces);
    std::vector<hipError_t> errs(T, hipSuccess);
    auto work = [&](int t) {
        hipError_t e = hipSetDevice(device);
        size_t pending_off[2] = {0, 0}, pending_len[2] = {0, 0};
        int h = 0;
        for (size_t p = (size_t)t; p < n_pieces && e == hipSuccess; p += (size_t)T, h ^= 1) {
            const size_t off = p * BOUNCE_HALF, len = std::min(BOUNCE_HALF, n - off);
            uint8_t *half = b->pinned[t] + (size_t)h * BOUNCE_HALF;
            if (to_device) {
                e = hipEventSynchronize(b->ev[t][h]);
                if (e != hipSuccess) break;
                memcpy(half, (const uint8_t *)host + off, len);
                e = hipMemcpyAsync((uint8_t *)dev + off, half, len, hipMemcpyHostToDevice, b->stream[t]);
                if (e == hipSuccess) e = hipEventRecord(b->ev[t][h], b->stream[t]);
            } else {
                if (pending_len[h]) {
                    e = hipEventSynchronize(b->ev[t][h]);
                    if (e != hipSuccess) break;
                    memcpy((uint8_t *)host + pending_off[h], half, pending_len[h]);
                }
                e = hipMemcpyAsync(half, (const uint8_t *)dev + off, len, hipMemcpyDeviceToHost, b->stream[t]);
                if (e == hipSuccess) e = hipEventRecord(b->ev[t][h], b->stream[t]);
                pending_off[h] = off; pending_len[h] = len;
            }
        }
        if (e == hipSuccess) e = hipStreamSynchronize(b->stream[t]);
        if (!to_device && e == hipSuccess)
            for (int q = 0; q < 2; q++)
                if (pending_len[q]) memcpy((uint8_t *)host + pending_off[q], b->pinned[t] + (size_t)q * BOUNCE_HALF, pending_len[q]);
        errs[t] = e;
    };
    std::vector<std::thread> th;
    for (int t = 1; t < T; t++) th.emplace_back(work, t);
    work(0);
    for (auto &x : th) x.join();
    for (int t = 0; t < T; t++)
        if (errs[t] != hipSuccess) return fail(PK_ERR_HIP, "host <-> device copy failed: %s", hipGetErrorString(errs[t]));
    return PK_OK;
}
}

extern "C" int pk_dev_alloc(void **dev_out, uint64_t n_bytes, int device) {
    if (!dev_out) return fail(PK_ERR_ARG, "null output pointer");
    HIPCHK(hipSetDevice(device));
    HIPCHK(hipMalloc(dev_out, n_bytes + 64));
    return PK_OK;
}
extern "C" int pk_dev_free(void *dev, int device) {
    if (!dev) return PK_OK;
    HIPCHK(hipSetDevice(device));
    HIPCHK(hipFree(dev));
    return PK_OK;
}
extern "C" int pk_dev_upload(void *dev_dst, const void *host_src, uint64_t n_bytes, int device) {
    if (n_bytes && (!dev_dst || !host_src)) return fail(PK_ERR_ARG, "null pointer");
    return bounce_copy(dev_dst, const_cast<void *>(host_src), n_bytes, true, device);
}
extern "C" int pk_dev_download(void *host_dst, const void *dev_src, uint64_t n_bytes, int device) {
    if (n_bytes && (!host_dst || !dev_src)) return fail(PK_ERR_ARG, "null pointer");
    return bounce_copy(const_cast<void *>(dev_src), host_dst, n_bytes, false, device);
}

extern "C" int pk_dev_mem_info(uint64_t *free_out, uint64_t *total_out, int device) {
    HIPCHK(hipSetDevice(device));
    size_t f = 0, t = 0;
    HIPCHK(hipMemGetInfo(&f, &t));
    if (free_out) *free_out = f;
    if (total_out) *total_out = t;
    return PK_OK;
}

namespace {
struct Stream {
    hipStream_t s = nullptr;
    Stream() = default;
    Stream(const Stream &) = delete;
    ~Stream() { if (s) hipStreamDestroy(s); }
    operator hipStream_t() const { return s; }
};

struct Events {
    hipEvent_t reset_begin = nullptr, reset_end = nullptr;
    hipEvent_t scan_begin = nullptr, scan_end = nullptr;
    hipEvent_t squeeze_begin = nullptr, squeeze_end = nullptr;
    hipEvent_t sort_begin = nullptr, sort_end = nullptr;
    hipEvent_t part_end = nullptr;
    hipEvent_t bucket_end = nullptr;
    hipEvent_t final_begin = nullptr, final_end = nullptr;
    hipEvent_t lookup_begin = nullptr, lookup_end = nullptr;
    Events() = default;
    Events(const Events &) = delete;
    ~Events() { for (hipEvent_t *e : all()) if (*e) hipEventDestroy(*e); }
    std::array<hipEvent_t *, 14> all() {
        return {&reset_begin, &reset_end, &scan_begin, &scan_end, &squeeze_begin, &squeeze_end, &sort_begin, &sort_end, &part_end, &bucket_end,
                &final_begin, &final_end, &lookup_begin, &lookup_end};
    }
};
}

struct pk_indexer {
    int k = 0, device = 0;
    int slice_bits = 0, slice_index = 0;
    uint64_t n = 0;
    Stream stream;
    Events ev;
    DevBuf<uint8_t> table8;
    struct Tail { Carry carry; unsigned long long hist[256]; FqCarry fq; };
    DevBuf<Tail> tail, tail0;
    struct Pinned { Tail tail; uint32_t flags[4]; } *pin = nullptr;
    bool tail_on_host = false;
    bool zero_timed = true;
    DevBuf<unsigned long long> hist_rep;
    DevBuf<DevRec> recs;
    DevBuf<L1> c_l1, c_l1s;
    DevBuf<L2> c_l2, c_l2s;
    DevBuf<LaneState> lane_state;
    DevBuf<PiecePack> packs;
    DevBuf<uint32_t> chunk_odd;
    DevBuf<L1> t_l1;
    DevBuf<L2> t_l2;
    DevBuf<uint8_t> staging[2];
    uint64_t bytes_fed = 0, n_recs = 0;
    bool finished = false;
    double t_scan = 0, t_squeeze = 0, t_sort = 0, t_final = 0, t_zero = 0, t_part = 0, t_bucket = 0;
    int feeds = 0, relayouts = 0;
    uint64_t recounted = 0;
    bool table_fresh = true;
    DevBuf<uint8_t> ws;
    int format = PK_FORMAT_FASTA;
    bool fed = false;
    DevBuf<FqSum> fq_sums;
    DevBuf<FqState> fq_st;
    DevBuf<uint8_t> fq_out[2];
    int fq_buf = 0;
    uint64_t fq_pending = 0;
    DevBuf<FqRec> fq_recs;
    uint64_t fq_need = 0;
    bool fq_failed = false;
    std::string fq_err;
    bool query = false;
    std::vector<const uint8_t *> q_tables;
    int q_min = 1, q_max = 255;
    DevBuf<unsigned long long> q_P;
    DevBuf<unsigned long long> q_hits, q_depth;
    uint64_t q_windows = 0, q_p_done = 0;

    uint64_t recs_cap() const { return recs.bytes / sizeof(DevRec); }
    uint64_t fq_recs_cap() const { return fq_recs.bytes / sizeof(FqRec); }
    ~pk_indexer() {
        hipSetDevice(device);
        if (stream) hipStreamSynchronize(stream);
        if (pin) hipHostFree(pin);
    }
};

static int ix_reset(pk_indexer *ix) {
    HIPCHK(hipSetDevice(ix->device));
    HIPCHK(hipEventRecord(ix->ev.reset_begin, ix->stream));
    HIPCHK(hipMemcpyAsync(ix->tail.p, ix->tail0.p, sizeof(pk_indexer::Tail), hipMemcpyDeviceToDevice, ix->stream));
    ix->tail_on_host = false;
    if (ix->recs.p) HIPCHK(hipMemsetAsync(ix->recs.p, 0, ix->recs.bytes, ix->stream));
    for (DevBuf<unsigned long long> *b : {&ix->q_P, &ix->q_hits, &ix->q_depth})
        if (b->p) HIPCHK(hipMemsetAsync(b->p, 0, b->bytes, ix->stream));
    ix->q_windows = ix->q_p_done = 0;
    HIPCHK(hipEventRecord(ix->ev.reset_end, ix->stream));
    ix->zero_timed = false;
    ix->t_zero = 0;
    ix->bytes_fed = ix->n_recs = 0;
    ix->finished = false;
    ix->table_fresh = true;
    ix->t_scan = ix->t_squeeze = ix->t_sort = ix->t_final = ix->t_part = ix->t_bucket = 0;
    ix->feeds = ix->relayouts = 0; ix->recounted = 0;
    ix->fed = false;
    ix->fq_pending = 0; ix->fq_need = 0; ix->fq_failed = false; ix->fq_err.clear();
    return PK_OK;
}

static void time_reset(pk_indexer *ix) {
    if (ix->zero_timed) return;
    float ms = 0;
    if (hipEventElapsedTime(&ms, ix->ev.reset_begin, ix->ev.reset_end) == hipSuccess) ix->t_zero = ms * 1e-3;
    ix->zero_timed = true;
}

static int read_tail(pk_indexer *ix) {
    HIPCHK(hipMemcpyAsync(&ix->pin->tail, ix->tail.p, sizeof(pk_indexer::Tail), hipMemcpyDeviceToHost, ix->stream));
    HIPCHK(hipStreamSynchronize(ix->stream));
    HIPCHK(hipGetLastError());
    time_reset(ix);
    ix->tail_on_host = true;
    return PK_OK;
}

static void hist_with_zeros(const unsigned long long *h, uint64_t n, uint64_t hist256_out[256]) {
    uint64_t nonzero = 0;
    for (int v = 1; v < 256; v++) { hist256_out[v] = h[v]; nonzero += h[v]; }
    hist256_out[0] = n - nonzero;
}

extern "C" void pk_indexer_destroy(pk_indexer *ix) { delete ix; }

static int create_indexer(pk_indexer **out, int k, int device, int slice_index, int n_slices, bool query);

extern "C" int pk_indexer_create(pk_indexer **out, int k, int device) { return create_indexer(out, k, device, 0, 1, false); }

extern "C" int pk_indexer_create_slice(pk_indexer **out, int k, int device, int slice_index, int n_slices) {
    return create_indexer(out, k, device, slice_index, n_slices, false);
}

extern "C" int pk_query_create(pk_indexer **out, int k, int device) {
    if (k > 17) return fail(PK_ERR_ARG, "a query takes kmer_len <= 17 (one unsliced table), got %d", k);
    return create_indexer(out, k, device, 0, 1, true);
}

static int create_indexer(pk_indexer **out, int k, int device, int slice_index, int n_slices, bool query) {
    if (!out) return fail(PK_ERR_ARG, "null output pointer");
    *out = nullptr;
    int slice_bits = 0;
    while (slice_bits < 30 && (1 << slice_bits) < n_slices) slice_bits++;
    if (n_slices < 1 || (1 << slice_bits) != n_slices) return fail(PK_ERR_ARG, "the number of address slices must be a power of two, got %d", n_slices);
    int rc = check_k(k, slice_bits, slice_index);
    if (rc) return rc;
    HIPCHK(hipSetDevice(device));
    std::unique_ptr<pk_indexer> ix(new pk_indexer());
    ix->k = k; ix->device = device; ix->slice_bits = slice_bits; ix->slice_index = slice_index;
    ix->n = 1ULL << (2 * k - slice_bits);
    ix->query = query;
    HIPCHK(hipStreamCreateWithFlags(&ix->stream.s, hipStreamNonBlocking));
    for (hipEvent_t *e : ix->ev.all()) HIPCHK(hipEventCreate(e));
    if (!query && (rc = ix->table8.reserve(std::max<uint64_t>(ix->n, 16)))) return rc;
    if ((rc = ix->tail.reserve(sizeof(pk_indexer::Tail)))) return rc;
    if ((rc = ix->tail0.reserve(sizeof(pk_indexer::Tail)))) return rc;
    HIPCHK(hipHostMalloc(&ix->pin, sizeof(*ix->pin), hipHostMallocDefault));
    {
        Carry c;
        memset(&c, 0, sizeof c);
        c.l1 = 8u | 1u | (LS_START << 1);
        c.l2.flags = F_NONID | F_PRESET | F_BRK;
        HIPCHK(hipMemset(ix->tail0.p, 0, sizeof(pk_indexer::Tail)));
        HIPCHK(hipMemcpy(&ix->tail0.p->carry, &c, sizeof c, hipMemcpyHostToDevice));
        FqCarry q;
        memset(&q, 0, sizeof q);
        q.st.ws = q.in.ws = 1;
        q.err = q.trail = ~0ull;
        q.prev4 = q.prev4_in = 0x0a0a0a0au;
        HIPCHK(hipMemcpy(&ix->tail0.p->fq, &q, sizeof q, hipMemcpyHostToDevice));
    }
    if ((rc = ix->hist_rep.reserve((size_t)HIST_REPLICAS * 256 * sizeof(unsigned long long)))) return rc;
    HIPCHK(hipMemset(ix->hist_rep.p, 0, ix->hist_rep.bytes));
    if ((rc = ix->recs.reserve(4096 * sizeof(DevRec)))) return rc;
    if (query && (rc = ix->q_P.reserve(4096 * sizeof(unsigned long long)))) return rc;
    part_set_attributes();
    if ((rc = ix_reset(ix.get()))) return rc;
    *out = ix.release();
    return PK_OK;
}

extern "C" int pk_indexer_reset(pk_indexer *ix) {
    if (!ix) return fail(PK_ERR_ARG, "null indexer");
    return ix_reset(ix);
}

static int ensure_chunks(pk_indexer *ix, uint32_t n_chunks) {
    const size_t n = n_chunks;
    int rc;
    if ((rc = ix->c_l1.reserve(n * sizeof(L1)))) return rc;
    if ((rc = ix->c_l1s.reserve(n * sizeof(L1)))) return rc;
    if ((rc = ix->c_l2.reserve(n * sizeof(L2)))) return rc;
    if ((rc = ix->c_l2s.reserve(n * sizeof(L2)))) return rc;
    if ((rc = ix->lane_state.reserve(n * WG * sizeof(LaneState)))) return rc;
    if ((rc = ix->packs.reserve(n * WG * sizeof(PiecePack)))) return rc;
    if ((rc = ix->chunk_odd.reserve(n * sizeof(uint32_t)))) return rc;
    if ((rc = ix->t_l1.reserve((n / 1024 + 1) * sizeof(L1)))) return rc;
    return ix->t_l2.reserve((n / 1024 + 1) * sizeof(L2));
}

static int ensure_recs(pk_indexer *ix, uint64_t need) {
    if (need <= ix->recs_cap()) return PK_OK;
    const uint64_t cap = std::max<uint64_t>(need, std::max<uint64_t>(1024, ix->recs_cap() * 2));
    int rc = ix->recs.grow_keep(cap * sizeof(DevRec), ix->stream);
    if (rc || !ix->query) return rc;
    const size_t row = ix->q_tables.size() * sizeof(unsigned long long);
    if ((rc = ix->q_P.grow_keep(cap * sizeof(unsigned long long), ix->stream))) return rc;
    if ((rc = ix->q_hits.grow_keep(cap * row, ix->stream))) return rc;
    return ix->q_depth.grow_keep(cap * row, ix->stream);
}

static const uint64_t FEED_MAX = 2ULL << 30;
static uint64_t feed_max_for(int k) { return k <= 15 ? (1ULL << 30) : FEED_MAX; }

static bool plan_fits_u32(const PartPlan &pl) {
    const uint64_t lim = (pl.k <= 15 ? (1ULL << 31) : (1ULL << 32)) - (16384 + 64);
    return pl.capacity1 < lim && pl.capacity2 < lim;
}

extern "C" int pk_diag_plan(int k, uint64_t n_bytes, uint64_t out[8]) {
    if (!out) return fail(PK_ERR_ARG, "null output");
    int rc = check_k(k, k > 17 ? 2 * k - 34 : 0, 0);
    if (rc) return rc;
    if (n_bytes == 0) n_bytes = feed_max_for(k);
    const PartPlan pl = make_part_plan((uint32_t)k, n_bytes, k > 17 ? (uint32_t)(2 * k - 34) : 0u, 0u);
    out[0] = feed_max_for(k); out[1] = pl.capacity1; out[2] = pl.capacity2; out[3] = pl.B1; out[4] = pl.B2; out[5] = pl.fb_bits;
    out[6] = pl.n_chunks; out[7] = plan_fits_u32(pl) ? 1 : 0;
    return PK_OK;
}

static int query_feed_piece(pk_indexer *ix, const uint8_t *f, uint64_t n_bytes);

static int feed_piece(pk_indexer *ix, const uint8_t *f, uint64_t n_bytes) {
    if (ix->query) return query_feed_piece(ix, f, n_bytes);
    const uint32_t n_chunks = (uint32_t)((n_bytes + CHUNK - 1) / CHUNK);
    int rc = ensure_chunks(ix, n_chunks);
    if (rc) return rc;
    PartPlan pl = make_part_plan((uint32_t)ix->k, n_bytes, (uint32_t)ix->slice_bits, (uint32_t)ix->slice_index);
    if (!plan_fits_u32(pl)) return fail(PK_ERR_ARG, "feed of %llu bytes needs record positions beyond 2^32 (internal limit); split it", (unsigned long long)n_bytes);
    if ((rc = part_plan_check(pl, n_bytes))) return rc;
    if ((rc = ix->ws.reserve(part_workspace(pl, n_bytes)))) return rc;
    PartBuffers pb;
    part_workspace(pl, n_bytes, ix->ws.p, &pb);
    Carry *carry = &ix->tail.p->carry;
    const Events &ev = ix->ev;
    HIPCHK(hipEventRecord(ev.scan_begin, ix->stream));
    launch_chunk_l1(f, n_bytes, ix->c_l1.p, n_chunks, ix->stream);
    launch_scan_l1(ix->c_l1.p, n_chunks, carry, ix->c_l1s.p, ix->t_l1.p, pb.signals, ix->stream);
    launch_chunk_l2(f, n_bytes, ix->c_l1s.p, ix->c_l2.p, ix->lane_state.p, ix->packs.p, ix->chunk_odd.p, n_chunks, (uint32_t)ix->k, ix->stream);
    launch_scan_l2(ix->c_l2.p, n_chunks, carry, ix->c_l2s.p, ix->t_l2.p, (uint32_t)ix->k, ix->stream);
    HIPCHK(hipEventRecord(ev.scan_end, ix->stream));
    bool squeeze = true;
    uint64_t squeezed_cap = 0;
    uint32_t stride = pl.sample_stride;
    for (int attempt = 0;; attempt++) {
        if (attempt) HIPCHK(hipMemsetAsync(pb.signals, 0, sizeof(PartSignals), ix->stream));
        if (squeeze) {
            squeezed_cap = ix->recs_cap();
            HIPCHK(hipEventRecord(ev.squeeze_begin, ix->stream));
            launch_squeeze(pl, pb, f, n_bytes, ix->bytes_fed, ix->lane_state.p, ix->packs.p, ix->c_l2s.p, ix->chunk_odd.p, ix->recs.p, squeezed_cap, carry,
                           ix->stream);
            if (ix->k > 17) launch_deep_tail(pl, pb, carry, ix->stream);
            HIPCHK(hipEventRecord(ev.squeeze_end, ix->stream));
        }
        if ((rc = launch_partitioned(pl, pb, ix->c_l2s.p, n_bytes, stride, carry, ix->table8.p, ix->tail.p->hist, ix->hist_rep.p, ix->table_fresh,
                                     {ev.sort_begin, ev.sort_end, ev.part_end}, ix->stream)))
            return rc;
        HIPCHK(hipEventRecord(ev.bucket_end, ix->stream));
        volatile uint32_t *got = ix->pin->flags;
        HIPCHK(hipMemcpyAsync(ix->pin->flags, pb.flags, sizeof ix->pin->flags, hipMemcpyDeviceToHost, ix->stream));
        if ((rc = read_tail(ix))) return rc;
        if (!got[0]) { ix->recounted += got[1]; break; }
        if (attempt >= 3) return fail(PK_ERR_HIP, "the feed's layout did not settle (internal error, flag %u)", got[0]);
        if (got[0] == 2u) {
            rc = ensure_recs(ix, ix->pin->tail.carry.n_recs);
            if (rc) return rc;
            squeeze = true;
        } else {
            if (stride == 1) return fail(PK_ERR_HIP, "level-1 buckets overflowed an exact layout (internal error)");
            stride = 1;
            squeeze = false;
            ix->relayouts++;
        }
    }
    if (ix->pin->tail.carry.n_recs > squeezed_cap)
        return fail(PK_ERR_HIP, "feed counted without its squeeze: %llu records, %llu slots (internal error)",
                    (unsigned long long)ix->pin->tail.carry.n_recs, (unsigned long long)squeezed_cap);
    const uint64_t recs_before = ix->n_recs;
    ix->n_recs = ix->pin->tail.carry.n_recs;
    rc = ensure_recs(ix, ix->n_recs + 2 * (ix->n_recs - recs_before) + 1024);
    if (rc) return rc;
    ix->table_fresh = false;
    float scan = 0, squeeze_ms = 0, part = 0, bucket = 0, sort = 0;
    HIPCHK(hipEventElapsedTime(&scan, ev.scan_begin, ev.scan_end));
    HIPCHK(hipEventElapsedTime(&squeeze_ms, ev.squeeze_begin, ev.squeeze_end));
    HIPCHK(hipEventElapsedTime(&part, ev.squeeze_end, ev.part_end));
    HIPCHK(hipEventElapsedTime(&bucket, ev.part_end, ev.bucket_end));
    HIPCHK(hipEventElapsedTime(&sort, ev.sort_begin, ev.sort_end));
    ix->t_scan += scan * 1e-3; ix->t_squeeze += squeeze_ms * 1e-3; ix->t_part += part * 1e-3; ix->t_bucket += bucket * 1e-3; ix->t_sort += sort * 1e-3;
    ix->feeds++;
    ix->bytes_fed += n_bytes;
    return PK_OK;
}

static int query_feed_piece(pk_indexer *ix, const uint8_t *f, uint64_t n_bytes) {
    if (ix->q_tables.empty()) return fail(PK_ERR_STATE, "pk_query_set_tables comes before the first feed");
    const uint32_t n_chunks = (uint32_t)((n_bytes + CHUNK - 1) / CHUNK);
    int rc = ensure_chunks(ix, n_chunks);
    if (rc) return rc;
    const PartPlan pl = make_part_plan((uint32_t)ix->k, n_bytes, 0u, 0u);
    if ((rc = ix->ws.reserve(query_workspace(n_chunks)))) return rc;
    PartBuffers pb;
    QueryBuffers qb;
    query_workspace(n_chunks, ix->ws.p, &pb, &qb);
    Carry *carry = &ix->tail.p->carry;
    const Events &ev = ix->ev;
    const uint32_t N = (uint32_t)ix->q_tables.size();
    HIPCHK(hipEventRecord(ev.scan_begin, ix->stream));
    launch_chunk_l1(f, n_bytes, ix->c_l1.p, n_chunks, ix->stream);
    launch_scan_l1(ix->c_l1.p, n_chunks, carry, ix->c_l1s.p, ix->t_l1.p, pb.signals, ix->stream);
    launch_chunk_l2(f, n_bytes, ix->c_l1s.p, ix->c_l2.p, ix->lane_state.p, ix->packs.p, ix->chunk_odd.p, n_chunks, (uint32_t)ix->k, ix->stream);
    launch_scan_l2(ix->c_l2.p, n_chunks, carry, ix->c_l2s.p, ix->t_l2.p, (uint32_t)ix->k, ix->stream);
    HIPCHK(hipEventRecord(ev.scan_end, ix->stream));
    uint64_t squeezed_cap = 0;
    for (int attempt = 0;; attempt++) {
        if (attempt) HIPCHK(hipMemsetAsync(pb.signals, 0, sizeof(PartSignals), ix->stream));
        squeezed_cap = ix->recs_cap();
        HIPCHK(hipEventRecord(ev.squeeze_begin, ix->stream));
        launch_squeeze(pl, pb, f, n_bytes, ix->bytes_fed, ix->lane_state.p, ix->packs.p, ix->c_l2s.p, ix->chunk_odd.p, ix->recs.p, squeezed_cap, carry,
                       ix->stream);
        HIPCHK(hipEventRecord(ev.squeeze_end, ix->stream));
        HIPCHK(hipEventRecord(ev.lookup_begin, ix->stream));
        launch_query_scan(pl, pb, qb, ix->c_l2s.p, ix->q_windows, ix->recs.p, carry, ix->q_p_done, ix->q_P.p, ix->stream);
        for (uint32_t t0 = 0; t0 < N; t0 += QUERY_MAX_TABLES)
            launch_query_lookup(pl, pb, qb, ix->c_l2s.p, ix->q_P.p, carry, ix->q_tables.data() + t0, std::min(QUERY_MAX_TABLES, N - t0), N, t0,
                                (uint32_t)ix->q_min, (uint32_t)ix->q_max, ix->q_hits.p, ix->q_depth.p, ix->stream);
        HIPCHK(hipEventRecord(ev.lookup_end, ix->stream));
        HIPCHK(hipGetLastError());
        volatile uint32_t *got = ix->pin->flags;
        HIPCHK(hipMemcpyAsync(ix->pin->flags, pb.flags, sizeof ix->pin->flags, hipMemcpyDeviceToHost, ix->stream));
        if ((rc = read_tail(ix))) return rc;
        if (!got[0]) break;
        if (got[0] != 2u || attempt >= 3) return fail(PK_ERR_HIP, "the query feed did not settle (internal error, flag %u)", got[0]);
        if ((rc = ensure_recs(ix, ix->pin->tail.carry.n_recs))) return rc;
    }
    if (ix->pin->tail.carry.n_recs > squeezed_cap)
        return fail(PK_ERR_HIP, "feed looked up without its squeeze: %llu records, %llu slots (internal error)",
                    (unsigned long long)ix->pin->tail.carry.n_recs, (unsigned long long)squeezed_cap);
    const uint64_t recs_before = ix->n_recs;
    ix->n_recs = ix->pin->tail.carry.n_recs;
    ix->q_windows = ix->pin->tail.carry.num_kmers;
    ix->q_p_done = ix->n_recs;
    if ((rc = ensure_recs(ix, ix->n_recs + 2 * (ix->n_recs - recs_before) + 1024))) return rc;
    float scan = 0, squeeze_ms = 0, lookup = 0;
    HIPCHK(hipEventElapsedTime(&scan, ev.scan_begin, ev.scan_end));
    HIPCHK(hipEventElapsedTime(&squeeze_ms, ev.squeeze_begin, ev.squeeze_end));
    HIPCHK(hipEventElapsedTime(&lookup, ev.lookup_begin, ev.lookup_end));
    ix->t_scan += scan * 1e-3; ix->t_squeeze += squeeze_ms * 1e-3; ix->t_part += lookup * 1e-3;
    ix->feeds++;
    ix->bytes_fed += n_bytes;
    return PK_OK;
}

extern "C" int pk_query_set_tables(pk_indexer *ix, const void *const *dev_tables, int N, int min_count, int max_count) {
    if (!ix) return fail(PK_ERR_ARG, "null indexer");
    if (!ix->query) return fail(PK_ERR_STATE, "not a query indexer (pk_query_create)");
    if (ix->fed || ix->finished) return fail(PK_ERR_STATE, "the tables are set before the first feed (reset the indexer first)");
    if (N < 1 || !dev_tables) return fail(PK_ERR_ARG, "need at least one table");
    if (min_count < 1 || max_count > 255 || min_count > max_count) return fail(PK_ERR_ARG, "count window must satisfy 1 <= min <= max <= 255, got %d-%d", min_count, max_count);
    for (int i = 0; i < N; i++)
        if (!dev_tables[i]) return fail(PK_ERR_ARG, "table %d is a null pointer", i);
    HIPCHK(hipSetDevice(ix->device));
    ix->q_tables.assign((const uint8_t *const *)dev_tables, (const uint8_t *const *)dev_tables + N);
    ix->q_min = min_count; ix->q_max = max_count;
    const size_t need = ix->recs_cap() * (size_t)N * sizeof(unsigned long long);
    for (DevBuf<unsigned long long> *b : {&ix->q_hits, &ix->q_depth}) {
        int rc = b->reserve(need);
        if (rc) return rc;
        HIPCHK(hipMemsetAsync(b->p, 0, b->bytes, ix->stream));
    }
    return PK_OK;
}

extern "C" int pk_query_results(pk_indexer *ix, uint64_t *hits_out, uint64_t *depth_out, uint64_t recs_cap) {
    if (!ix) return fail(PK_ERR_ARG, "null indexer");
    if (!ix->query) return fail(PK_ERR_STATE, "not a query indexer (pk_query_create)");
    if (!ix->finished) return fail(PK_ERR_STATE, "call pk_indexer_finish first");
    if (ix->n_recs > recs_cap) return fail(PK_ERR_RECS_CAP, "%llu records, capacity %llu", (unsigned long long)ix->n_recs, (unsigned long long)recs_cap);
    if (ix->n_recs == 0) return PK_OK;
    if (!hits_out || !depth_out) return fail(PK_ERR_ARG, "null output pointer");
    HIPCHK(hipSetDevice(ix->device));
    const size_t n = ix->n_recs * ix->q_tables.size() * sizeof(uint64_t);
    HIPCHK(hipMemcpy(hits_out, ix->q_hits.p, n, hipMemcpyDeviceToHost));
    HIPCHK(hipMemcpy(depth_out, ix->q_depth.p, n, hipMemcpyDeviceToHost));
    return PK_OK;
}

static const char *fq_rule_text(uint32_t rule) {
    switch (rule) {
    case FQ_RULE_AT: return "line 1 must begin with '@' (after an empty line 1 only line terminators may follow)";
    case FQ_RULE_GT: return "line 2 must not begin with '>'";
    case FQ_RULE_PLUS: return "line 3 must begin with '+'";
    case FQ_RULE_LEN: return "line 4 must be as long as line 2";
    default: return "the stream ends inside the record";
    }
}

static int fq_fail(pk_indexer *ix, uint64_t rec, uint32_t rule) {
    uint64_t line1 = 0;
    if (rec < ix->fq_recs_cap()) HIPCHK(hipMemcpy(&line1, &ix->fq_recs.p[rec].line1, sizeof line1, hipMemcpyDeviceToHost));
    fail(PK_ERR_FORMAT, "malformed FASTQ: record %llu (line 1 at byte %llu): %s", (unsigned long long)rec + 1, (unsigned long long)line1,
         fq_rule_text(rule));
    ix->fq_failed = true;
    ix->fq_err = g_err;
    return PK_ERR_FORMAT;
}

static int fq_verdict(pk_indexer *ix) {
    const FqCarry &q = ix->pin->tail.fq;
    uint64_t rec = ~0ull;
    uint32_t rule = 0;
    if (q.err != ~0ull) { rec = q.err >> 3; rule = (uint32_t)(q.err & 7u); }
    if (q.trail != ~0ull) {
        const uint64_t tr = q.trail / 4u;
        if (rec != ~0ull && rec >= tr) rec = ~0ull;
        if (q.full > q.trail + 1u && tr < rec) { rec = tr; rule = FQ_RULE_AT; }
    }
    return rec == ~0ull ? PK_OK : fq_fail(ix, rec, rule);
}

static int fq_ensure_recs(pk_indexer *ix, uint64_t need) {
    if (need <= ix->fq_recs_cap()) return PK_OK;
    return ix->fq_recs.grow_keep(std::max<uint64_t>(need, 2 * ix->fq_recs_cap()) * sizeof(FqRec), ix->stream);
}

static int fq_flush(pk_indexer *ix) {
    if (ix->fq_pending) {
        const uint64_t n = ix->fq_pending;
        ix->fq_pending = 0;
        return feed_piece(ix, ix->fq_out[ix->fq_buf ^ 1].p, n);
    }
    return read_tail(ix);
}

static int fq_feed_piece(pk_indexer *ix, const uint8_t *f, uint64_t n) {
    const uint32_t n_chunks = (uint32_t)((n + CHUNK - 1) / CHUNK);
    const int b = ix->fq_buf;
    int rc;
    if ((rc = ix->fq_sums.reserve((size_t)n_chunks * sizeof(FqSum)))) return rc;
    if ((rc = ix->fq_st.reserve((size_t)n_chunks * sizeof(FqState)))) return rc;
    if ((rc = ix->fq_out[b].reserve(n + 64))) return rc;
    if ((rc = fq_ensure_recs(ix, ix->fq_need + n / 256 + 1024))) return rc;
    FqCarry *carry = &ix->tail.p->fq;
    launch_fq_front(f, n, ix->fq_sums.p, ix->fq_st.p, ix->fq_out[b].p, ix->fq_recs.p, ix->fq_recs_cap(), carry, ix->stream);
    HIPCHK(hipGetLastError());
    if ((rc = fq_flush(ix))) return rc;
    if (ix->pin->tail.fq.need > ix->fq_recs_cap()) {
        if ((rc = fq_ensure_recs(ix, ix->pin->tail.fq.need + n / 256 + 1024))) return rc;
        launch_fq_write(f, n, ix->fq_st.p, ix->fq_out[b].p, ix->fq_recs.p, ix->fq_recs_cap(), carry, ix->stream);
        HIPCHK(hipGetLastError());
        if ((rc = fq_flush(ix))) return rc;
    }
    const FqCarry &q = ix->pin->tail.fq;
    ix->fq_need = q.need;
    if ((rc = fq_verdict(ix))) return rc;
    ix->fq_pending = q.st.out - q.in.out;
    ix->fq_buf = b ^ 1;
    return PK_OK;
}

static int fq_end_check(pk_indexer *ix) {
    const FqCarry &q = ix->pin->tail.fq;
    if (q.trail != ~0ull) return PK_OK;
    const uint32_t role = (uint32_t)(q.st.line & 3u);
    const uint64_t rec = q.st.line / 4u;
    if (role == 0u && q.st.curlen == 0) return PK_OK;
    if (role == 3u && q.st.curlen > 0) {
        uint64_t len2 = 0;
        if (rec < ix->fq_recs_cap()) HIPCHK(hipMemcpy(&len2, &ix->fq_recs.p[rec].len2, sizeof len2, hipMemcpyDeviceToHost));
        return len2 == q.st.curlen ? PK_OK : fq_fail(ix, rec, FQ_RULE_LEN);
    }
    return fq_fail(ix, rec, FQ_RULE_END);
}

extern "C" int pk_indexer_set_format(pk_indexer *ix, int format) {
    if (!ix) return fail(PK_ERR_ARG, "null indexer");
    if (format != PK_FORMAT_FASTA && format != PK_FORMAT_FASTQ) return fail(PK_ERR_ARG, "unknown input format %d", format);
    if (ix->fed || ix->finished) return fail(PK_ERR_STATE, "the input format is set before the first feed (reset the indexer first)");
    ix->format = format;
    return PK_OK;
}

extern "C" int pk_indexer_fastq_stats(pk_indexer *ix, uint64_t out[4]) {
    if (!ix || !out) return fail(PK_ERR_ARG, "null argument");
    if (ix->format != PK_FORMAT_FASTQ) return fail(PK_ERR_STATE, "not a FASTQ indexer");
    for (int i = 0; i < 4; i++) out[i] = 0;
    if (!ix->fed) return PK_OK;
    const FqCarry &q = ix->pin->tail.fq;
    const uint64_t lines = q.st.line + (q.st.curlen > 0 ? 1u : 0u);
    out[0] = q.trail != ~0ull ? q.trail / 4u : (lines + 3u) / 4u;
    out[1] = lines;
    out[2] = q.bytes_fed;
    out[3] = q.st.out;
    return PK_OK;
}

extern "C" int pk_indexer_feed_device(pk_indexer *ix, const void *dev_fasta, uint64_t n_bytes) {
    if (!ix) return fail(PK_ERR_ARG, "null indexer");
    if (ix->finished) return fail(PK_ERR_STATE, "indexer already finished; reset it first");
    if (n_bytes == 0) return PK_OK;
    if (!dev_fasta || ((uintptr_t)dev_fasta & 15u)) return fail(PK_ERR_ARG, "device FASTA pointer must be non-null and 16-byte aligned");
    if (n_bytes > (1ULL << 40)) return fail(PK_ERR_ARG, "feed of %llu bytes too large; split it", (unsigned long long)n_bytes);
    HIPCHK(hipSetDevice(ix->device));
    const uint8_t *f = (const uint8_t *)dev_fasta;
    const uint64_t piece_max = feed_max_for(ix->k);
    const bool fastq = ix->format == PK_FORMAT_FASTQ;
    if (fastq && ix->fq_failed) return fail(PK_ERR_FORMAT, "%s", ix->fq_err.c_str());
    ix->fed = true;
    for (uint64_t off = 0; off < n_bytes; off += piece_max) {
        const uint64_t len = std::min(piece_max, n_bytes - off);
        int rc = fastq ? fq_feed_piece(ix, f + off, len) : feed_piece(ix, f + off, len);
        if (rc) return rc;
    }
    return PK_OK;
}

extern "C" int pk_indexer_feed(pk_indexer *ix, const uint8_t *host_fasta, uint64_t n_bytes) {
    if (!ix) return fail(PK_ERR_ARG, "null indexer");
    if (n_bytes == 0) return PK_OK;
    if (!host_fasta) return fail(PK_ERR_ARG, "null FASTA pointer");
    HIPCHK(hipSetDevice(ix->device));
    const char *env = getenv("PK_FEED_PIECE");
    uint64_t piece = env ? strtoull(env, nullptr, 10) : (256ULL << 20);
    piece = std::max<uint64_t>(1 << 20, std::min<uint64_t>(piece, 1ULL << 30)) & ~15ULL;
    const uint64_t n_pieces = (n_bytes + piece - 1) / piece;
    const uint64_t buf_bytes = std::min(piece, n_bytes) + 64;
    const int n_bufs = n_pieces > 1 ? 2 : 1;
    int rc = PK_OK;
    for (int i = 0; i < n_bufs; i++)
        if ((rc = ix->staging[i].reserve(buf_bytes))) return rc;
    auto upload = [&](uint64_t p) -> int {
        const uint64_t off = p * piece, len = std::min(piece, n_bytes - off);
        return bounce_copy(ix->staging[p & 1].p, const_cast<uint8_t *>(host_fasta) + off, len, true, ix->device);
    };
    if ((rc = upload(0))) return rc;
    for (uint64_t p = 0; p < n_pieces; p++) {
        int up_rc = PK_OK;
        std::string up_err;
        std::thread next;
        if (p + 1 < n_pieces) next = std::thread([&]() { up_rc = upload(p + 1); if (up_rc) up_err = g_err; });
        const uint64_t off = p * piece, len = std::min(piece, n_bytes - off);
        rc = pk_indexer_feed_device(ix, ix->staging[p & 1].p, len);
        if (next.joinable()) next.join();
        if (rc) return rc;
        if (up_rc) { g_err = up_err; return up_rc; }
    }
    return PK_OK;
}

extern "C" int pk_indexer_finish(pk_indexer *ix, uint64_t *num_kmers_out, uint64_t *total_bp_out, uint64_t hist256_out[256],
                                 uint64_t *n_recs_out) {
    if (!ix) return fail(PK_ERR_ARG, "null indexer");
    HIPCHK(hipSetDevice(ix->device));
    if (!ix->finished && ix->format == PK_FORMAT_FASTQ) {
        if (ix->fq_failed) return fail(PK_ERR_FORMAT, "%s", ix->fq_err.c_str());
        if (ix->fq_pending) {
            int rc = fq_flush(ix);
            if (rc) return rc;
        }
    }
    if (!ix->finished) {
        if (ix->tail_on_host && (!ix->table_fresh || ix->query)) {
            ix->t_final = 0;
        } else {
            HIPCHK(hipEventRecord(ix->ev.final_begin, ix->stream));
            if (ix->table_fresh && !ix->query) {
                HIPCHK(hipMemsetAsync(ix->table8.p, 0, ix->table8.bytes, ix->stream));
                ix->table_fresh = false;
            }
            HIPCHK(hipEventRecord(ix->ev.final_end, ix->stream));
            int rc = read_tail(ix);
            if (rc) return rc;
            float ms = 0;
            HIPCHK(hipEventElapsedTime(&ms, ix->ev.final_begin, ix->ev.final_end));
            ix->t_final = ms * 1e-3;
        }
        if (ix->format == PK_FORMAT_FASTQ) {
            int rc = fq_end_check(ix);
            if (rc) return rc;
        }
        ix->finished = true;
    }
    const Carry &c = ix->pin->tail.carry;
    if (num_kmers_out) *num_kmers_out = c.num_kmers;
    if (total_bp_out) *total_bp_out = c.total_bp;
    if (n_recs_out) *n_recs_out = c.n_recs;
    if (hist256_out) {
        if (ix->query) memset(hist256_out, 0, 256 * sizeof(uint64_t));
        else hist_with_zeros(ix->pin->tail.hist, ix->n, hist256_out);
    }
    return PK_OK;
}

extern "C" int pk_indexer_records(pk_indexer *ix, pk_record *recs_out, uint64_t recs_cap) {
    if (!ix) return fail(PK_ERR_ARG, "null indexer");
    if (ix->n_recs > recs_cap) return fail(PK_ERR_RECS_CAP, "%llu records, capacity %llu", (unsigned long long)ix->n_recs, (unsigned long long)recs_cap);
    if (ix->n_recs == 0) return PK_OK;
    if (!recs_out) return fail(PK_ERR_ARG, "null records pointer");
    HIPCHK(hipSetDevice(ix->device));
    std::vector<DevRec> tmp(ix->n_recs);
    HIPCHK(hipMemcpy(tmp.data(), ix->recs.p, ix->n_recs * sizeof(DevRec), hipMemcpyDeviceToHost));
    for (uint64_t i = 0; i < ix->n_recs; i++) {
        recs_out[i].name_off = tmp[i].name_off;
        recs_out[i].name_len = tmp[i].name_end > tmp[i].name_off ? tmp[i].name_end - tmp[i].name_off : 0;
        recs_out[i].seq_len = tmp[i].seq_len;
        recs_out[i].n_valid_kmers = tmp[i].n_valid;
    }
    if (ix->format == PK_FORMAT_FASTQ) {
        if (ix->n_recs > ix->fq_recs_cap()) return fail(PK_ERR_HIP, "FASTQ record array too small (internal error)");
        std::vector<FqRec> fq(ix->n_recs);
        HIPCHK(hipMemcpy(fq.data(), ix->fq_recs.p, ix->n_recs * sizeof(FqRec), hipMemcpyDeviceToHost));
        for (uint64_t i = 0; i < ix->n_recs; i++) recs_out[i].name_off = fq[i].line1 + 1;
    }
    return PK_OK;
}

extern "C" int pk_indexer_table_to_host(pk_indexer *ix, uint8_t *table_out) {
    if (!ix || !table_out) return fail(PK_ERR_ARG, "null argument");
    if (ix->query) return fail(PK_ERR_STATE, "a query indexer holds no table");
    if (!ix->finished) return fail(PK_ERR_STATE, "call pk_indexer_finish first");
    return bounce_copy(ix->table8.p, table_out, ix->n, false, ix->device);
}

extern "C" int pk_indexer_table_slice_to_host(pk_indexer *ix, uint8_t *dst, uint64_t offset, uint64_t n_bytes) {
    if (!ix || !dst) return fail(PK_ERR_ARG, "null argument");
    if (ix->query) return fail(PK_ERR_STATE, "a query indexer holds no table");
    if (!ix->finished) return fail(PK_ERR_STATE, "call pk_indexer_finish first");
    if (offset > ix->n || n_bytes > ix->n - offset) return fail(PK_ERR_ARG, "slice outside the table");
    return bounce_copy(ix->table8.p + offset, dst, n_bytes, false, ix->device);
}

extern "C" int pk_indexer_table_device(pk_indexer *ix, const void **dev_table_out) {
    if (!ix || !dev_table_out) return fail(PK_ERR_ARG, "null argument");
    if (ix->query) return fail(PK_ERR_STATE, "a query indexer holds no table");
    if (!ix->finished) return fail(PK_ERR_STATE, "call pk_indexer_finish first");
    *dev_table_out = ix->table8.p;
    return PK_OK;
}

extern "C" int pk_indexer_table_slice_to_device(pk_indexer *ix, void *dev_dst, uint64_t offset, uint64_t n_bytes) {
    if (!ix || !dev_dst) return fail(PK_ERR_ARG, "null argument");
    if (ix->query) return fail(PK_ERR_STATE, "a query indexer holds no table");
    if (!ix->finished) return fail(PK_ERR_STATE, "call pk_indexer_finish first");
    if (offset > ix->n || n_bytes > ix->n - offset) return fail(PK_ERR_ARG, "slice outside the table");
    HIPCHK(hipSetDevice(ix->device));
    HIPCHK(hipMemcpy(dev_dst, ix->table8.p + offset, n_bytes, hipMemcpyDeviceToDevice));
    return PK_OK;
}

extern "C" int pk_indexer_timings(pk_indexer *ix, double out[10]) {
    if (!ix || !out) return fail(PK_ERR_ARG, "null argument");
    for (int i = 0; i < 10; i++) out[i] = 0;
    out[0] = ix->t_scan; out[1] = ix->t_squeeze; out[2] = ix->t_final; out[3] = ix->t_zero; out[4] = (double)ix->feeds;
    out[5] = ix->t_part; out[6] = ix->t_bucket; out[7] = ix->t_sort; out[8] = (double)ix->relayouts; out[9] = (double)ix->recounted;
    return PK_OK;
}

static pk_indexer *g_cached_indexer = nullptr;

extern "C" int pk_count_release(void) {
    if (g_cached_indexer) { pk_indexer_destroy(g_cached_indexer); g_cached_indexer = nullptr; }
    return PK_OK;
}

extern "C" int pk_count_fasta(const uint8_t *fasta, uint64_t n_bytes, int k, uint8_t *table_out, uint64_t *num_kmers_out,
                              uint64_t *total_bp_out, uint64_t hist256_out[256], pk_record *recs_out, uint64_t recs_cap,
                              uint64_t *n_recs_out, int device) {
    int rc = check_k(k);
    if (rc) return rc;
    if (!table_out) return fail(PK_ERR_ARG, "null table pointer");
    if (n_bytes && !fasta) return fail(PK_ERR_ARG, "null FASTA pointer");
    static std::mutex cache_mu;
    std::lock_guard<std::mutex> cache_lock(cache_mu);
    pk_indexer *&ix = g_cached_indexer;
    if (ix && (ix->k != k || ix->device != device)) { pk_indexer_destroy(ix); ix = nullptr; }
    if (!ix) {
        rc = pk_indexer_create(&ix, k, device);
        if (rc) { ix = nullptr; return rc; }
    } else if ((rc = pk_indexer_reset(ix))) {
        return rc;
    }
    if ((rc = pk_indexer_feed(ix, fasta, n_bytes))) return rc;
    uint64_t n_recs = 0;
    if ((rc = pk_indexer_finish(ix, num_kmers_out, total_bp_out, hist256_out, &n_recs))) return rc;
    if (n_recs_out) *n_recs_out = n_recs;
    if ((rc = pk_indexer_table_to_host(ix, table_out))) return rc;
    if (n_recs > recs_cap) return fail(PK_ERR_RECS_CAP, "%llu records, capacity %llu", (unsigned long long)n_recs, (unsigned long long)recs_cap);
    return pk_indexer_records(ix, recs_out, recs_cap);
}

extern "C" int pk_table_stats(const uint8_t *table, uint64_t n, uint64_t hist256_out[256], int device) {
    if (!hist256_out || (n && !table)) return fail(PK_ERR_ARG, "null argument");
    HIPCHK(hipSetDevice(device));
    DevBuf<unsigned long long> d_hist;
    DevBuf<uint8_t> d_t;
    unsigned long long h[256];
    int rc;
    if ((rc = d_hist.reserve(sizeof h))) return rc;
    if ((rc = d_t.reserve(std::max<uint64_t>(n, 16)))) return rc;
    if (hipMemset(d_hist.p, 0, sizeof h) != hipSuccess || hipMemcpy(d_t.p, table, n, hipMemcpyHostToDevice) != hipSuccess)
        return fail(PK_ERR_HIP, "upload failed");
    launch_hist8(d_t.p, n, d_hist.p, 0);
    if (hipDeviceSynchronize() != hipSuccess || hipMemcpy(h, d_hist.p, sizeof h, hipMemcpyDeviceToHost) != hipSuccess)
        return fail(PK_ERR_HIP, "histogram kernel failed: %s", hipGetErrorString(hipGetLastError()));
    hist_with_zeros(h, n, hist256_out);
    return PK_OK;
}

static int check_counts(int N, int min_count, int max_count) {
    if (N < 1) return fail(PK_ERR_ARG, "need at least one table");
    if (N > 128) return fail(PK_ERR_ARG, "at most 128 tables per call (got %d)", N);
    if (min_count < 1 || max_count > 255) return fail(PK_ERR_ARG, "min_count must be >= 1 and max_count <= 255 (merger.py:90-91)");
    return PK_OK;
}

extern "C" int pk_gram_expand(const uint64_t *pair, int N, uint64_t *matrix_out) {
    if (!pair || !matrix_out || N < 1) return fail(PK_ERR_ARG, "bad argument");
    for (int i = 0; i < N; i++)
        for (int j = 0; j < N; j++) {
            uint64_t *m = matrix_out + ((uint64_t)i * N + j) * 3;
            if (i == j) { m[0] = m[1] = m[2] = 0; continue; }
            m[0] = pair[(uint64_t)i * N + i];
            m[1] = pair[(uint64_t)j * N + j];
            m[2] = i < j ? pair[(uint64_t)i * N + j] : pair[(uint64_t)j * N + i];
        }
    return PK_OK;
}

namespace {
struct GramCtx {
    std::mutex mu;
    const uint8_t **d_ptrs = nullptr;
    hipStream_t stream = nullptr;
    hipEvent_t e0 = nullptr, e1 = nullptr;
    unsigned long long *d_pair = nullptr;
    const uint8_t **d_gtab = nullptr;
    std::vector<const uint8_t *> h_gtab;
    uint8_t *d_occ = nullptr;
    size_t occ_cap = 0;
};
GramCtx g_gram[MAX_DEVICES];

int gram_ctx(int device, GramCtx **out) {
    if (device < 0 || device >= MAX_DEVICES) return fail(PK_ERR_ARG, "device ordinal %d out of range", device);
    GramCtx &c = g_gram[device];
    static std::mutex init_mu;
    std::lock_guard<std::mutex> init_lock(init_mu);
    if (!c.d_ptrs) {
        HIPCHK(hipMalloc(&c.d_ptrs, 128 * sizeof(void *)));
        HIPCHK(hipMalloc(&c.d_pair, 128 * 128 * sizeof(unsigned long long)));
        HIPCHK(hipStreamCreateWithFlags(&c.stream, hipStreamNonBlocking));
        HIPCHK(hipEventCreate(&c.e0));
        HIPCHK(hipEventCreate(&c.e1));
        HIPCHK(hipMalloc(&c.d_gtab, (size_t)spectrum_groups(128) * 16 * sizeof(void *)));
        c.h_gtab.assign((size_t)spectrum_groups(128) * 16, nullptr);
    }
    *out = &c;
    return PK_OK;
}

using PassStep = std::function<int(GramCtx &)>;

int timed_pass(const char *what, const void *const *dev_tables, int N, int device, double *kernel_seconds_out,
               const PassStep &before, const PassStep &launch, const PassStep &after = nullptr) {
    if (!dev_tables) return fail(PK_ERR_ARG, "null table list");
    for (int i = 0; i < N; i++)
        if (!dev_tables[i] || ((uintptr_t)dev_tables[i] & 15u)) return fail(PK_ERR_ARG, "table %d: device pointer must be 16-byte aligned", i);
    HIPCHK(hipSetDevice(device));
    GramCtx *c = nullptr;
    int rc = gram_ctx(device, &c);
    if (rc) return rc;
    std::lock_guard<std::mutex> lock(c->mu);
    if (before && (rc = before(*c))) return rc;
    HIPCHK(hipEventRecord(c->e0, c->stream));
    if (launch(*c)) return fail(PK_ERR_HIP, "%s kernel launch failed: %s", what, hipGetErrorString(hipGetLastError()));
    HIPCHK(hipEventRecord(c->e1, c->stream));
    if (after && (rc = after(*c))) return rc;
    HIPCHK(hipStreamSynchronize(c->stream));
    if (kernel_seconds_out) { float ms = 0; HIPCHK(hipEventElapsedTime(&ms, c->e0, c->e1)); *kernel_seconds_out = ms * 1e-3; }
    return PK_OK;
}

PassStep upload_pointers(const void *const *dev_tables, int N) {
    return [=](GramCtx &c) -> int {
        HIPCHK(hipMemcpyAsync(c.d_ptrs, dev_tables, N * sizeof(void *), hipMemcpyHostToDevice, c.stream));
        return PK_OK;
    };
}
}

extern "C" int pk_gram_device_partial(const void *const *dev_tables, int N, uint64_t n_slice, int min_count, int max_count,
                                      uint64_t *pair_out, void *dev_pair_out, int device, double *kernel_seconds_out) {
    int rc = check_counts(N, min_count, max_count);
    if (rc) return rc;
    auto d_pair = [=](GramCtx &c) { return dev_pair_out ? (unsigned long long *)dev_pair_out : c.d_pair; };
    return timed_pass(
        "gram", dev_tables, N, device, kernel_seconds_out, upload_pointers(dev_tables, N),
        [&](GramCtx &c) { return launch_gram(c.d_ptrs, N, n_slice, min_count, max_count, d_pair(c), true, c.stream); },
        [&](GramCtx &c) -> int {
            if (pair_out) HIPCHK(hipMemcpyAsync(pair_out, d_pair(c), (size_t)N * N * sizeof(uint64_t), hipMemcpyDeviceToHost, c.stream));
            return PK_OK;
        });
}

extern "C" int pk_gram_device_accumulate(const void *const *dev_tables, int N, uint64_t n_slice, int min_count, int max_count,
                                         void *dev_pair_accum, int device, double *kernel_seconds_out) {
    return pk_gram_device_accumulate_windows(dev_tables, N, n_slice, &min_count, &max_count, 1, dev_pair_accum, device, kernel_seconds_out);
}

extern "C" int pk_gram_device_accumulate_windows(const void *const *dev_tables, int N, uint64_t n_slice, const int *min_counts,
                                                 const int *max_counts, int n_windows, void *dev_pair_accum, int device,
                                                 double *kernel_seconds_out) {
    if (!dev_pair_accum) return fail(PK_ERR_ARG, "null accumulator");
    if (n_windows < 1 || n_windows > 255 || !min_counts || !max_counts) return fail(PK_ERR_ARG, "between 1 and 255 windows per call");
    int rc = PK_OK;
    for (int w = 0; w < n_windows; w++)
        if ((rc = check_counts(N, min_counts[w], max_counts[w]))) return rc;
    const int per_pass = gram_windows_per_pass(N);
    unsigned long long *acc = (unsigned long long *)dev_pair_accum;
    return timed_pass("gram", dev_tables, N, device, kernel_seconds_out, upload_pointers(dev_tables, N), [&](GramCtx &c) {
        std::vector<int> order(n_windows);
        for (int w = 0; w < n_windows; w++) order[w] = w;
        std::stable_sort(order.begin(), order.end(), [&](int a, int b) { return min_counts[a] < min_counts[b]; });
        for (int at = 0; at < n_windows;) {
            const int take = (per_pass >= 2 && n_windows - at >= 2) ? std::min(per_pass, n_windows - at) : 1;
            int lrc;
            if (take == 1) {
                const int w = order[at];
                lrc = launch_gram(c.d_ptrs, N, n_slice, min_counts[w], max_counts[w], acc + (size_t)w * N * N, false, c.stream);
            } else {
                int mn[8], mx[8], out[8];
                for (int i = 0; i < take; i++) { mn[i] = min_counts[order[at + i]]; mx[i] = max_counts[order[at + i]]; out[i] = order[at + i]; }
                lrc = launch_gram_windows(c.d_ptrs, N, n_slice, mn, mx, out, take, acc, c.stream);
            }
            if (lrc) return lrc;
            at += take;
        }
        return 0;
    });
}

extern "C" int pk_spectrum_device_accumulate(const void *const *dev_tables, int N, uint64_t n_slice, void *dev_spec_accum, int device,
                                             double *kernel_seconds_out) {
    if (N < 2 || N > 128) return fail(PK_ERR_ARG, "a spectrum pass takes 2 to 128 tables (got %d)", N);
    if (!dev_spec_accum) return fail(PK_ERR_ARG, "null accumulator");
    return timed_pass("spectrum", dev_tables, N, device, kernel_seconds_out, nullptr, [&](GramCtx &c) {
        return launch_spectrum(dev_tables, N, n_slice, (unsigned long long *)dev_spec_accum, c.h_gtab.data(), c.d_gtab, c.stream);
    });
}

extern "C" int pk_occgram_device_accumulate(const void *const *dev_tables, int N, uint64_t n_slice, void *dev_accum, int device,
                                            double *kernel_seconds_out) {
    if (N < 2 || N > 128) return fail(PK_ERR_ARG, "an occgram pass takes 2 to 128 tables (got %d)", N);
    if (!dev_accum) return fail(PK_ERR_ARG, "null accumulator");
    auto grow_scratch = [&](GramCtx &c) -> int {
        const size_t need = occgram_scratch_bytes(N, n_slice);
        if (need > c.occ_cap) HIPCHK(hipStreamSynchronize(c.stream));
        return reserve_exact((void **)&c.d_occ, &c.occ_cap, need);
    };
    return timed_pass("occgram", dev_tables, N, device, kernel_seconds_out, grow_scratch, [&](GramCtx &c) {
        return launch_occgram(dev_tables, N, n_slice, (unsigned long long *)dev_accum, c.d_ptrs, c.d_occ, c.stream);
    });
}

extern "C" int pk_extract_device(const void *const *dev_tables, int n_present, int n_absent, uint64_t n_slice, uint64_t first_addr,
                                 int min_count, int max_count, int min_present, int max_absent, void *dev_addr_out, void *dev_counts_out,
                                 uint64_t cap, uint64_t *n_selected_out, int device, double *kernel_seconds_out) {
    if (n_present < 1 || n_absent < 0 || n_present > 128 || n_absent > 128 || n_present + n_absent > 128)
        return fail(PK_ERR_ARG, "an extraction takes 1 to 128 tables, at least one of them present (got %d present, %d absent)", n_present, n_absent);
    if (min_count < 1 || max_count > 255 || min_count > max_count)
        return fail(PK_ERR_ARG, "the count window must satisfy 1 <= min <= max <= 255 (got %d-%d)", min_count, max_count);
    if (min_present < 1 || min_present > n_present) return fail(PK_ERR_ARG, "min_present must lie in 1..%d (got %d)", n_present, min_present);
    if (max_absent < 0 || max_absent > n_absent) return fail(PK_ERR_ARG, "max_absent must lie in 0..%d (got %d)", n_absent, max_absent);
    if (!n_selected_out) return fail(PK_ERR_ARG, "null n_selected_out");
    if (n_slice > (1ull << 40) || first_addr + n_slice < first_addr) return fail(PK_ERR_ARG, "slice of %llu addresses is out of range", (unsigned long long)n_slice);
    if (cap && (!dev_addr_out || !dev_counts_out || ((uintptr_t)dev_addr_out & 15u) || ((uintptr_t)dev_counts_out & 15u)))
        return fail(PK_ERR_ARG, "a capacity needs both output arrays, 16-byte aligned");
    if (cap > (1ull << 40)) return fail(PK_ERR_ARG, "capacity out of range");
    const int N = n_present + n_absent;
    const uint32_t n_wg = extract_workgroups(n_slice);
    DevBuf<uint16_t> d_masks;
    DevBuf<unsigned long long> d_wg;
    unsigned long long total = 0;
    if (n_slice == 0) {
        if (!dev_tables) return fail(PK_ERR_ARG, "null table list");
        *n_selected_out = 0;
        return PK_OK;
    }
    int rc = timed_pass(
        "extract", dev_tables, N, device, kernel_seconds_out,
        [&](GramCtx &c) -> int {
            int r = upload_pointers(dev_tables, N)(c);
            if (!r) r = d_wg.reserve(((size_t)n_wg + 1) * sizeof(unsigned long long));
            if (!r && cap) r = d_masks.reserve(extract_mask_words(n_slice) * sizeof(uint16_t));
            return r;
        },
        [&](GramCtx &c) {
            return launch_extract(c.d_ptrs, n_present, n_absent, n_slice, first_addr, min_count, max_count, min_present, max_absent, d_masks.p, d_wg.p,
                                  (unsigned long long *)dev_addr_out, (uint8_t *)dev_counts_out, cap, c.stream);
        },
        [&](GramCtx &c) -> int {
            HIPCHK(hipMemcpyAsync(&total, d_wg.p + n_wg, sizeof total, hipMemcpyDeviceToHost, c.stream));
            return PK_OK;
        });
    if (rc) return rc;
    *n_selected_out = total;
    if (total > cap && (cap || dev_addr_out || dev_counts_out))
        return fail(PK_ERR_RECS_CAP, "%llu addresses selected, room for %llu", total, (unsigned long long)cap);
    return PK_OK;
}

extern "C" int pk_extract_text(const void *dev_addr, uint64_t m, int k, void *dev_text_out, int device) {
    if (k < 1 || k > 32) return fail(PK_ERR_ARG, "kmer_len must lie in 1..32 (got %d)", k);
    if (m > (1ull << 40)) return fail(PK_ERR_ARG, "too many addresses");
    if (m == 0) return PK_OK;
    if (!dev_addr || !dev_text_out || ((uintptr_t)dev_addr & 7u) || ((uintptr_t)dev_text_out & 15u))
        return fail(PK_ERR_ARG, "address array (8-byte aligned) and text array (16-byte aligned) must not be null");
    HIPCHK(hipSetDevice(device));
    GramCtx *c = nullptr;
    int rc = gram_ctx(device, &c);
    if (rc) return rc;
    std::lock_guard<std::mutex> lock(c->mu);
    if (launch_extract_text((const unsigned long long *)dev_addr, m, k, (uint8_t *)dev_text_out, c->stream))
        return fail(PK_ERR_HIP, "extract text kernel launch failed: %s", hipGetErrorString(hipGetLastError()));
    HIPCHK(hipStreamSynchronize(c->stream));
    return PK_OK;
}

extern "C" int pk_gram(const uint8_t *const *tables, int N, uint64_t n, int min_count, int max_count, uint64_t *matrix_out,
                       const int *devices, int n_devices) {
    int rc = check_counts(N, min_count, max_count);
    if (rc) return rc;
    if (!tables || !matrix_out) return fail(PK_ERR_ARG, "null argument");
    int dev0 = 0;
    if (!devices || n_devices <= 0) { devices = &dev0; n_devices = 1; }
    const uint64_t per = ((n + n_devices - 1) / n_devices + 31u) & ~31ULL;
    std::vector<std::vector<uint64_t>> parts(n_devices, std::vector<uint64_t>((size_t)N * N, 0));
    std::vector<int> rcs(n_devices, PK_OK);
    std::vector<std::string> errs(n_devices);
    auto work = [&](int d) {
        const uint64_t lo = std::min<uint64_t>(n, per * d), hi = std::min<uint64_t>(n, lo + per);
        if (hi <= lo) return;
        auto run = [&]() -> int {
            HIPCHK(hipSetDevice(devices[d]));
            size_t free_b = 0, total_b = 0;
            HIPCHK(hipMemGetInfo(&free_b, &total_b));
            uint64_t sub = hi - lo;
            const uint64_t budget = (uint64_t)(free_b * 0.8);
            if ((uint64_t)N * (sub + 64) > budget) sub = std::max<uint64_t>(1 << 20, (budget / N - 64) & ~2047ULL);
            std::vector<DevBuf<uint8_t>> slices(N);
            std::vector<const void *> dptr(N, nullptr);
            int r;
            for (int i = 0; i < N; i++) {
                if ((r = slices[i].reserve(std::min(sub, hi - lo) + 64))) return r;
                dptr[i] = slices[i].p;
            }
            std::vector<uint64_t> one((size_t)N * N);
            for (uint64_t a = lo; a < hi; a += sub) {
                const uint64_t b = std::min(hi, a + sub);
                for (int i = 0; i < N; i++)
                    if (hipMemcpy(slices[i].p, tables[i] + a, b - a, hipMemcpyHostToDevice) != hipSuccess) return fail(PK_ERR_HIP, "table upload failed");
                if ((r = pk_gram_device_partial(dptr.data(), N, b - a, min_count, max_count, one.data(), nullptr, devices[d], nullptr))) return r;
                for (size_t i = 0; i < one.size(); i++) parts[d][i] += one[i];
            }
            return PK_OK;
        };
        rcs[d] = run();
        if (rcs[d]) errs[d] = g_err;
    };
    if (n_devices == 1) work(0);
    else {
        std::vector<std::thread> th;
        for (int d = 0; d < n_devices; d++) th.emplace_back(work, d);
        for (auto &t : th) t.join();
    }
    for (int d = 0; d < n_devices; d++)
        if (rcs[d]) { g_err = errs[d]; return rcs[d]; }
    std::vector<uint64_t> pair((size_t)N * N, 0);
    for (int d = 0; d < n_devices; d++)
        for (size_t i = 0; i < pair.size(); i++) pair[i] += parts[d][i];
    return pk_gram_expand(pair.data(), N, matrix_out);
}
```

pykmer_amd/csrc/pk_kernels.h:

```cpp
#pragma once
#include <hip/hip_runtime.h>
#include <stdint.h>
#include "fasta_fsm.h"

namespace pk {

struct DevRec {
    uint64_t name_off;
    uint64_t name_end;
    uint64_t seq_len;
    uint64_t n_valid;
};

struct Carry {
    L2 l2;
    L1 l1;
    uint32_t pad;
    uint64_t n_recs;
    uint64_t total_bp;
    uint64_t num_kmers;
    uint64_t deep_in, deep_out;
};

struct PartSignals {
    unsigned long long side_n;
    uint32_t flags[4];
};

void launch_chunk_l1(const uint8_t *fasta, uint64_t n, L1 *chunk_l1, uint32_t n_chunks, hipStream_t s);
void launch_scan_l1(const L1 *in, uint32_t n_chunks, Carry *carry, L1 *out, L1 *tile_ws, PartSignals *zeroed, hipStream_t s);
void launch_chunk_l2(const uint8_t *fasta, uint64_t n, const L1 *st1, L2 *chunk_l2, LaneState *lane_state, PiecePack *packs, uint32_t *chunk_odd, uint32_t n_chunks,
                     uint32_t k, hipStream_t s);
void launch_scan_l2(const L2 *in, uint32_t n_chunks, Carry *carry, L2 *out, L2 *tile_ws, uint32_t k, hipStream_t s);
void launch_hist8(const uint8_t *table8, uint64_t n, unsigned long long *hist, hipStream_t s);

constexpr uint32_t SLOT_CODE_WORDS = 1024;
constexpr uint32_t SLOT_RST_WORDS = 512;

struct PartPlan {
    uint32_t k, addr_bits;
    uint32_t slice_bits, slice_index;
    uint32_t fb_bits;
    uint32_t b1, b2, B1, B2;
    uint32_t n_chunks;
    uint32_t n_wg0, G;
    uint32_t n_wg1, G1;
    uint64_t R2;
    uint32_t sample_stride;
    uint32_t n_tally;
    uint32_t sample2;
    uint64_t capacity1;
    uint64_t capacity2;
};
constexpr uint32_t COUNT_WGS = 256;
constexpr uint32_t HIST_REPLICAS = 64;
struct PartBuffers {
    uint32_t *codes, *restarts, *n_bases;
    uint32_t *tally_rows, *tally_tot;
    uint32_t *sampled_n, *block_tot;
    uint32_t *bucket_base, *bucket_end, *cursor1, *cap_end, *wg2_start;
    uint32_t *final_start, *cursor2, *cap2_end;
    void *out1, *out2;
    unsigned long long *side, *side_n;
    uint64_t side_cap;
    PartSignals *signals;
    uint32_t *flags;
};
struct PartEvents { hipEvent_t sort_begin, sort_end, part_end; };
PartPlan make_part_plan(uint32_t k, uint64_t n_bytes, uint32_t slice_bits, uint32_t slice_index);
int part_plan_check(const PartPlan &pl, uint64_t n_bytes);
size_t part_workspace(const PartPlan &pl, uint64_t n_bytes, uint8_t *base = nullptr, PartBuffers *view = nullptr);
void part_set_attributes();
void fuse_set_attributes();
void launch_squeeze(const PartPlan &pl, const PartBuffers &b, const uint8_t *fasta, uint64_t n, uint64_t stream_off, const LaneState *lane_state,
                    const PiecePack *packs, const L2 *st2, const uint32_t *chunk_odd, DevRec *recs, uint64_t recs_cap, Carry *carry, hipStream_t s);
void launch_deep_tail(const PartPlan &pl, const PartBuffers &b, Carry *carry, hipStream_t s);
void launch_provision(const PartPlan &pl, const PartBuffers &b, const L2 *st2, uint32_t stride, const Carry *carry, hipStream_t s);
void launch_walk_sort(const PartPlan &pl, const PartBuffers &b, const L2 *st2, const Carry *carry, hipStream_t s);
int launch_partitioned(const PartPlan &pl, const PartBuffers &b, const L2 *st2, uint64_t n_bytes, uint32_t stride, const Carry *carry, uint8_t *table8,
                       unsigned long long *hist, unsigned long long *hist_rep, bool fresh, const PartEvents &ev, hipStream_t s);

constexpr uint32_t QUERY_MAX_TABLES = 16;
struct QueryTables { const uint8_t *t[QUERY_MAX_TABLES]; };
struct QueryBuffers {
    uint32_t *slot_count;
    unsigned long long *slot_first;
};
size_t query_workspace(uint32_t n_chunks, uint8_t *base = nullptr, PartBuffers *view = nullptr, QueryBuffers *qview = nullptr);
void launch_query_scan(const PartPlan &pl, const PartBuffers &b, const QueryBuffers &qb, const L2 *st2, uint64_t windows_before, const DevRec *recs,
                       const Carry *carry, uint64_t p_done, unsigned long long *P, hipStream_t s);
void launch_query_lookup(const PartPlan &pl, const PartBuffers &b, const QueryBuffers &qb, const L2 *st2, const unsigned long long *P, const Carry *carry,
                         const uint8_t *const *tables, uint32_t n_tab, uint32_t N, uint32_t t0, uint32_t min_count, uint32_t max_count,
                         unsigned long long *hits, unsigned long long *depth, hipStream_t s);

struct FqState {
    uint64_t line;
    uint64_t out;
    uint64_t curlen;
    uint32_t ws, pad;
};
struct FqSum {
    uint32_t nt;
    uint32_t tail;
    uint32_t kept[4];
    uint32_t ws, pad;
};
struct FqRec {
    uint64_t line1;
    uint64_t len2, len4;
};
enum : uint32_t { FQ_RULE_AT = 1, FQ_RULE_GT = 2, FQ_RULE_PLUS = 3, FQ_RULE_LEN = 4, FQ_RULE_END = 5 };
struct FqCarry {
    FqState st;
    FqState in;
    uint64_t bytes_fed, in_bytes;
    uint64_t err;
    uint64_t trail;
    uint64_t full;
    uint64_t need;
    uint32_t prev4, prev4_in;
};
void launch_fq_front(const uint8_t *fastq, uint64_t n, FqSum *sums, FqState *st, uint8_t *out, FqRec *recs, uint64_t recs_cap,
                     FqCarry *carry, hipStream_t s);
void launch_fq_write(const uint8_t *fastq, uint64_t n, const FqState *st, uint8_t *out, FqRec *recs, uint64_t recs_cap, FqCarry *carry,
                     hipStream_t s);

int launch_gram(const uint8_t *const *dev_tables, int N, uint64_t n_slice, int min_count, int max_count,
                unsigned long long *dev_pair, bool zero_first, hipStream_t s);

int gram_windows_per_pass(int N);
int launch_gram_windows(const uint8_t *const *dev_tables, int N, uint64_t n_slice, const int *min_counts, const int *max_counts,
                        const int *out_index, int W, unsigned long long *dev_pair, hipStream_t s);

int spectrum_groups(int N);
int launch_spectrum(const void *const *dev_tables, int N, uint64_t n_slice, unsigned long long *dev_accum, const uint8_t **host_gtab,
                    const uint8_t **dev_gtab, hipStream_t s);

uint64_t occgram_scratch_bytes(int N, uint64_t n_slice);
int launch_occgram(const void *const *dev_tables, int N, uint64_t n_slice, unsigned long long *dev_accum, const uint8_t **dev_ptrs,
                   uint8_t *occ_scratch, hipStream_t s);

uint32_t extract_workgroups(uint64_t n_slice);
uint64_t extract_mask_words(uint64_t n_slice);
int launch_extract(const uint8_t *const *dev_tables, int P, int A, uint64_t n_slice, uint64_t first_addr, int min_count, int max_count, int min_present,
                   int max_absent, uint16_t *masks, unsigned long long *wg, unsigned long long *addr_out, uint8_t *counts_out, uint64_t cap,
                   hipStream_t s);
int launch_extract_text(const unsigned long long *addr, uint64_t m, int k, uint8_t *text, hipStream_t s);

}
```

Baseline: 216.6 billion bp/s.

## Fold single-block scan, provision and tail readback into last-workgroup tickets

```diff
diff --git a/pykmer_amd/csrc/kmer_count.hip b/pykmer_amd/csrc/kmer_count.hip
--- a/pykmer_amd/csrc/kmer_count.hip
+++ b/pykmer_amd/csrc/kmer_count.hip
@@ -1,3 +1,4 @@
+#include <algorithm>
 #include "fasta_fsm.h"
 #include "pk_kernels.h"
 
@@ -173,24 +174,22 @@
     return lane == 0 ? pre : compose(pre, up);
 }
 
-__global__ __launch_bounds__(SCAN_T) void k_scan_l1_reduce(const L1 *__restrict__ in, uint32_t n, L1 *__restrict__ tile_tot) {
+__global__ __launch_bounds__(SCAN_T) void k_scan_l1_reduce(const L1 *__restrict__ in, uint32_t n, L1 *tile_tot, uint32_t n_tiles, Carry *carry,
+                                                           uint32_t *__restrict__ zero_words, uint32_t n_zero) {
     __shared__ L1 sh[SCAN_T / 64];
+    const auto compose = [](L1 a, L1 b) { return l1_compose(a, b); };
+    const auto shfl = [](L1 v, int d) { return (L1)__shfl_up(v, d, 64); };
     const uint32_t i = blockIdx.x * SCAN_T + threadIdx.x;
     L1 tot;
-    tile_scan<L1>(i < n ? in[i] : 0u, 0u, sh, &tot, [](L1 a, L1 b) { return l1_compose(a, b); }, [](L1 v, int d) { return (L1)__shfl_up(v, d, 64); });
+    tile_scan<L1>(i < n ? in[i] : 0u, 0u, sh, &tot, compose, shfl);
     if (threadIdx.x == 0) tile_tot[blockIdx.x] = tot;
-}
-__global__ __launch_bounds__(SCAN_T) void k_scan_l1_tiles(L1 *__restrict__ tile_tot, uint32_t n_tiles, Carry *carry, uint32_t *__restrict__ zero_words,
-                                                          uint32_t n_zero) {
-    __shared__ L1 sh[SCAN_T / 64];
+    if (!last_workgroup(&carry->ticket, gridDim.x)) return;
     if (threadIdx.x < n_zero) zero_words[threadIdx.x] = 0u;
     L1 run = carry->l1;
     for (uint32_t t0 = 0; t0 < n_tiles; t0 += SCAN_T) {
-        const uint32_t i = t0 + threadIdx.x;
-        L1 tot;
-        L1 ex = tile_scan<L1>(i < n_tiles ? tile_tot[i] : 0u, run, sh, &tot, [](L1 a, L1 b) { return l1_compose(a, b); },
-                              [](L1 v, int d) { return (L1)__shfl_up(v, d, 64); });
-        if (i < n_tiles) tile_tot[i] = ex;
+        const uint32_t t = t0 + threadIdx.x;
+        L1 ex = tile_scan<L1>(t < n_tiles ? tile_tot[t] : 0u, run, sh, &tot, compose, shfl);
+        if (t < n_tiles) tile_tot[t] = ex;
         run = tot;
         __syncthreads();
     }
@@ -206,23 +205,21 @@
     if (i < n) out_state[i] = ex;
 }
 
-__global__ __launch_bounds__(SCAN_T) void k_scan_l2_reduce(const L2 *__restrict__ in, uint32_t n, L2 *__restrict__ tile_tot, uint32_t km1) {
+__global__ __launch_bounds__(SCAN_T) void k_scan_l2_reduce(const L2 *__restrict__ in, uint32_t n, L2 *tile_tot, uint32_t n_tiles, Carry *carry,
+                                                           uint32_t km1) {
     __shared__ L2 sh[SCAN_T / 64];
+    const auto compose = [km1](const L2 &a, const L2 &b) { return l2_compose(a, b, km1); };
+    const auto shfl = [](const L2 &v, int d) { return shfl_up_l2(v, d); };
     const uint32_t i = blockIdx.x * SCAN_T + threadIdx.x;
     L2 tot;
-    tile_scan<L2>(i < n ? in[i] : l2_identity(), l2_identity(), sh, &tot, [km1](const L2 &a, const L2 &b) { return l2_compose(a, b, km1); },
-                  [](const L2 &v, int d) { return shfl_up_l2(v, d); });
+    tile_scan<L2>(i < n ? in[i] : l2_identity(), l2_identity(), sh, &tot, compose, shfl);
     if (threadIdx.x == 0) tile_tot[blockIdx.x] = tot;
-}
-__global__ __launch_bounds__(SCAN_T) void k_scan_l2_tiles(L2 *__restrict__ tile_tot, uint32_t n_tiles, Carry *carry, uint32_t km1) {
-    __shared__ L2 sh[SCAN_T / 64];
+    if (!last_workgroup(&carry->ticket, gridDim.x)) return;
     L2 run = carry->l2;
     for (uint32_t t0 = 0; t0 < n_tiles; t0 += SCAN_T) {
-        const uint32_t i = t0 + threadIdx.x;
-        L2 tot;
-        L2 ex = tile_scan<L2>(i < n_tiles ? tile_tot[i] : l2_identity(), run, sh, &tot,
-                              [km1](const L2 &a, const L2 &b) { return l2_compose(a, b, km1); }, [](const L2 &v, int d) { return shfl_up_l2(v, d); });
-        if (i < n_tiles) tile_tot[i] = ex;
+        const uint32_t t = t0 + threadIdx.x;
+        L2 ex = tile_scan<L2>(t < n_tiles ? tile_tot[t] : l2_identity(), run, sh, &tot, compose, shfl);
+        if (t < n_tiles) tile_tot[t] = ex;
         run = tot;
         __syncthreads();
     }
@@ -272,14 +269,32 @@
     }
 }
 
+__global__ __launch_bounds__(WG) void k_reset(unsigned long long *__restrict__ copy_dst, const unsigned long long *__restrict__ copy_src,
+                                              uint64_t copy_words, ZeroSpans zero) {
+    const uint64_t t = (uint64_t)blockIdx.x * WG + threadIdx.x, step = (uint64_t)gridDim.x * WG;
+    for (uint64_t i = t; i < copy_words; i += step) copy_dst[i] = copy_src[i];
+#pragma unroll
+    for (int j = 0; j < 4; j++) {
+        unsigned long long *p = reinterpret_cast<unsigned long long *>(zero.p[j]);
+        const uint64_t words = p ? zero.bytes[j] / 8u : 0u;
+        for (uint64_t i = t; i < words; i += step) p[i] = 0ull;
+    }
+}
+
+void launch_reset(void *copy_dst, const void *copy_src, uint64_t copy_bytes, const ZeroSpans &zero, hipStream_t s) {
+    uint64_t most = copy_bytes;
+    for (int j = 0; j < 4; j++) if (zero.p[j] && zero.bytes[j] > most) most = zero.bytes[j];
+    const uint64_t grid = std::min<uint64_t>(256u, std::max<uint64_t>(1u, most / (8u * WG * 8u)));
+    hipLaunchKernelGGL(k_reset, dim3((uint32_t)grid), dim3(WG), 0, s, (unsigned long long *)copy_dst, (const unsigned long long *)copy_src, copy_bytes / 8u, zero);
+}
 void launch_chunk_l1(const uint8_t *fasta, uint64_t n, L1 *chunk_l1, uint32_t n_chunks, hipStream_t s) {
     hipLaunchKernelGGL(k_chunk_l1, dim3((n_chunks + WG / 64 - 1) / (WG / 64)), dim3(WG), 0, s, fasta, n, n_chunks, chunk_l1);
 }
 void launch_scan_l1(const L1 *in, uint32_t n_chunks, Carry *carry, L1 *out, L1 *tile_ws, PartSignals *zeroed, hipStream_t s) {
-    static_assert(sizeof(PartSignals) % 4 == 0 && sizeof(PartSignals) / 4 <= SCAN_T, "k_scan_l1_tiles zeroes one word per thread");
+    static_assert(sizeof(PartSignals) % 4 == 0 && sizeof(PartSignals) / 4 <= SCAN_T, "k_scan_l1_reduce zeroes one word per thread");
     const uint32_t n_tiles = (n_chunks + SCAN_T - 1) / SCAN_T;
-    hipLaunchKernelGGL(k_scan_l1_reduce, dim3(n_tiles), dim3(SCAN_T), 0, s, in, n_chunks, tile_ws);
-    hipLaunchKernelGGL(k_scan_l1_tiles, dim3(1), dim3(SCAN_T), 0, s, tile_ws, n_tiles, carry, (uint32_t *)zeroed, (uint32_t)(sizeof(PartSignals) / 4));
+    hipLaunchKernelGGL(k_scan_l1_reduce, dim3(n_tiles), dim3(SCAN_T), 0, s, in, n_chunks, tile_ws, n_tiles, carry, (uint32_t *)zeroed,
+                       (uint32_t)(sizeof(PartSignals) / 4));
     hipLaunchKernelGGL(k_scan_l1_apply, dim3(n_tiles), dim3(SCAN_T), 0, s, in, n_chunks, (const L1 *)tile_ws, out);
 }
 void launch_chunk_l2(const uint8_t *fasta, uint64_t n, const L1 *st1, L2 *chunk_l2, LaneState *lane_state, PiecePack *packs, uint32_t *chunk_odd, uint32_t n_chunks,
@@ -288,8 +303,7 @@
 }
 void launch_scan_l2(const L2 *in, uint32_t n_chunks, Carry *carry, L2 *out, L2 *tile_ws, uint32_t k, hipStream_t s) {
     const uint32_t n_tiles = (n_chunks + SCAN_T - 1) / SCAN_T;
-    hipLaunchKernelGGL(k_scan_l2_reduce, dim3(n_tiles), dim3(SCAN_T), 0, s, in, n_chunks, tile_ws, k - 1);
-    hipLaunchKernelGGL(k_scan_l2_tiles, dim3(1), dim3(SCAN_T), 0, s, tile_ws, n_tiles, carry, k - 1);
+    hipLaunchKernelGGL(k_scan_l2_reduce, dim3(n_tiles), dim3(SCAN_T), 0, s, in, n_chunks, tile_ws, n_tiles, carry, k - 1);
     hipLaunchKernelGGL(k_scan_l2_apply, dim3(n_tiles), dim3(SCAN_T), 0, s, in, n_chunks, (const L2 *)tile_ws, out, k - 1);
 }
 static uint32_t stream_grid(uint64_t items_per_thread_units) {
diff --git a/pykmer_amd/csrc/kmer_fuse.hip b/pykmer_amd/csrc/kmer_fuse.hip
--- a/pykmer_amd/csrc/kmer_fuse.hip
+++ b/pykmer_amd/csrc/kmer_fuse.hip
@@ -307,13 +307,12 @@
 }
 
 constexpr int PROV_ROWS = 32;
-__global__ __launch_bounds__(1024) void k_provision(const uint32_t *__restrict__ tot, uint32_t n_tally, PartPlan pl, uint32_t n_sampled,
-                                                    uint32_t stride, uint32_t *__restrict__ bucket_base, uint32_t *__restrict__ cursor1,
-                                                    uint32_t *__restrict__ cap_end, uint32_t *__restrict__ final_start,
-                                                    uint32_t *__restrict__ cursor2, uint32_t *__restrict__ cap2_end, uint32_t *flags) {
+__device__ __forceinline__ void provision(const uint32_t *tot, uint32_t n_tally, const PartPlan &pl, uint32_t n_sampled,
+                                          uint32_t stride, uint32_t *__restrict__ bucket_base, uint32_t *__restrict__ cursor1,
+                                          uint32_t *__restrict__ cap_end, uint32_t *__restrict__ final_start,
+                                          uint32_t *__restrict__ cursor2, uint32_t *__restrict__ cap2_end, uint32_t *flags) {
     __shared__ uint32_t wsum[16];
     __shared__ unsigned long long sum1[512];
-    if (flags[0]) return;
     const uint32_t B1 = pl.B1;
     const bool two = n_tally > B1;
     const double scale = (double)pl.n_chunks / (double)n_sampled;
@@ -400,20 +399,49 @@
     }
 }
 
-__global__ __launch_bounds__(256) void k_tally_sum(const uint32_t *__restrict__ rows, uint32_t n_rows, uint32_t n_cols, uint32_t *__restrict__ tot) {
-    const uint32_t col = blockIdx.x * 256u + threadIdx.x;
-    if (col >= n_cols) return;
-    uint32_t acc[16] = {0, 0, 0, 0, 0, 0, 0, 0, 0, 0, 0, 0, 0, 0, 0, 0};
-    uint32_t r = 0;
-    for (; r + 16 <= n_rows; r += 16) {
-#pragma unroll
-        for (int u = 0; u < 16; u++) acc[u] += rows[(uint64_t)(r + u) * n_cols + col];
-    }
-    for (; r < n_rows; r++) acc[0] += rows[(uint64_t)r * n_cols + col];
-    uint32_t sum = 0;
-#pragma unroll
-    for (int u = 0; u < 16; u++) sum += acc[u];
-    tot[col] = sum;
+constexpr uint32_t TS_COLS = 256;
+__global__ __launch_bounds__(1024) void k_tally_provision(const uint32_t *__restrict__ rows, uint32_t n_rows, uint32_t n_tally, uint32_t *tot,
+                                                          PartPlan pl, uint32_t n_sampled, uint32_t stride, uint32_t *__restrict__ bucket_base,
+                                                          uint32_t *__restrict__ cursor1, uint32_t *__restrict__ cap_end,
+                                                          uint32_t *__restrict__ final_start, uint32_t *__restrict__ cursor2,
+                                                          uint32_t *__restrict__ cap2_end, uint32_t *flags, uint32_t *ticket) {
+    __shared__ uint32_t part[16][TS_COLS];
+    const bool backed_out = flags[0] != 0u;
+    if (!backed_out) {
+        const uint32_t lane = threadIdx.x & 63u, w = threadIdx.x >> 6;
+        const uint32_t c0 = blockIdx.x * TS_COLS + lane * 4u;
+        uint32_t acc[4] = {0u, 0u, 0u, 0u};
+        if ((n_tally & 3u) == 0u) {
+            if (c0 < n_tally) {
+                for (uint32_t r0 = w; r0 < n_rows; r0 += 16u * 8u) {
+                    uint4 v[8];
+#pragma unroll
+                    for (uint32_t u = 0; u < 8u; u++) {
+                        const uint32_t r = r0 + 16u * u;
+                        v[u] = r < n_rows ? *reinterpret_cast<const uint4 *>(rows + (uint64_t)r * n_tally + c0) : make_uint4(0u, 0u, 0u, 0u);
+                    }
+#pragma unroll
+                    for (uint32_t u = 0; u < 8u; u++) { acc[0] += v[u].x; acc[1] += v[u].y; acc[2] += v[u].z; acc[3] += v[u].w; }
+                }
+            }
+        } else {
+            for (uint32_t r = w; r < n_rows; r += 16u)
+                for (uint32_t j = 0; j < 4u; j++)
+                    if (c0 + j < n_tally) acc[j] += rows[(uint64_t)r * n_tally + c0 + j];
+        }
+#pragma unroll
+        for (uint32_t j = 0; j < 4u; j++) part[w][lane * 4u + j] = acc[j];
+        __syncthreads();
+        if (threadIdx.x < TS_COLS) {
+            uint32_t sum = 0;
+#pragma unroll
+            for (uint32_t u = 0; u < 16u; u++) sum += part[u][threadIdx.x];
+            const uint32_t col = blockIdx.x * TS_COLS + threadIdx.x;
+            if (col < n_tally) tot[col] = sum;
+        }
+    }
+    if (!last_workgroup(ticket, gridDim.x) || backed_out) return;
+    provision(tot, n_tally, pl, n_sampled, stride, bucket_base, cursor1, cap_end, final_start, cursor2, cap2_end, flags);
 }
 
 typedef ScatterLdsT<128> FuseLdsNarrow;
@@ -459,9 +487,9 @@
     launch_ws<true>(pl, grid, (size_t)n_tally * 4, s, b.codes, b.restarts, b.n_bases, st2, pl, n_sampled, stride, (void *)nullptr, (uint32_t *)nullptr,
                     (const uint32_t *)nullptr, 0u, b.flags, tally_shift, n_tally, b.tally_rows, (unsigned long long *)nullptr,
                     (unsigned long long *)nullptr, (uint64_t)0, (const unsigned long long *)&carry->deep_in);
-    hipLaunchKernelGGL(k_tally_sum, dim3((n_tally + 255u) / 256u), dim3(256), 0, s, (const uint32_t *)b.tally_rows, grid, n_tally, b.tally_tot);
-    hipLaunchKernelGGL(k_provision, dim3(1), dim3(1024), 0, s, (const uint32_t *)b.tally_tot, n_tally, pl, n_sampled, stride, b.bucket_base, b.cursor1,
-                       b.cap_end, b.final_start, b.cursor2, b.cap2_end, b.flags);
+    hipLaunchKernelGGL(k_tally_provision, dim3((n_tally + TS_COLS - 1u) / TS_COLS), dim3(1024), 0, s, (const uint32_t *)b.tally_rows, grid, n_tally,
+                       b.tally_tot, pl, n_sampled, stride, b.bucket_base, b.cursor1, b.cap_end, b.final_start, b.cursor2, b.cap2_end, b.flags,
+                       &b.signals->ticket[0]);
 }
 
 void launch_walk_sort(const PartPlan &pl, const PartBuffers &b, const L2 *st2, const Carry *carry, hipStream_t s) {
diff --git a/pykmer_amd/csrc/kmer_part.hip b/pykmer_amd/csrc/kmer_part.hip
--- a/pykmer_amd/csrc/kmer_part.hip
+++ b/pykmer_amd/csrc/kmer_part.hip
@@ -539,11 +539,10 @@
     }
 }
 
-__global__ __launch_bounds__(WG) void k_apply_side(const unsigned long long *__restrict__ side, const unsigned long long *__restrict__ side_n,
-                                                   uint64_t side_cap, uint8_t *__restrict__ table8, unsigned long long *__restrict__ hist,
-                                                   unsigned long long *__restrict__ hist_rep, const uint32_t *__restrict__ flags) {
+__device__ __forceinline__ void apply_side(const unsigned long long *__restrict__ side, const unsigned long long *__restrict__ side_n,
+                                           uint64_t side_cap, uint8_t *__restrict__ table8, unsigned long long *__restrict__ hist,
+                                           unsigned long long *__restrict__ hist_rep) {
     __shared__ unsigned long long key[AS_SLOTS];
-    if (flags[0]) return;
     static_assert(WG >= 256, "one thread per histogram bin");
     if (blockIdx.x == 0) hist_reduce(hist_rep, hist);
     __shared__ uint32_t val[AS_SLOTS];
@@ -579,6 +578,18 @@
         if (key[i] != 0ull) table_sat_add(table8, key[i] - 1ull, val[i] > 255u ? 255u : val[i], dh);
     __syncthreads();
     if (threadIdx.x < 256 && dh[threadIdx.x]) atomicAdd(&hist[threadIdx.x], (unsigned long long)(long long)dh[threadIdx.x]);
+}
+
+__global__ __launch_bounds__(WG) void k_apply_side(const unsigned long long *__restrict__ side, const unsigned long long *__restrict__ side_n,
+                                                   uint64_t side_cap, uint8_t *__restrict__ table8, unsigned long long *__restrict__ hist,
+                                                   unsigned long long *__restrict__ hist_rep, uint32_t *flags, HostTail to_host,
+                                                   uint32_t *ticket) {
+    if (!flags[0]) apply_side(side, side_n, side_cap, table8, hist, hist_rep);
+    if (!last_workgroup(ticket, gridDim.x)) return;
+    for (uint32_t i = threadIdx.x; i < to_host.words; i += WG)
+        to_host.dst[i] = __hip_atomic_load(const_cast<unsigned long long *>(to_host.src) + i, __ATOMIC_RELAXED, __HIP_MEMORY_SCOPE_AGENT);
+    if (threadIdx.x < 4u) to_host.flags[threadIdx.x] = __hip_atomic_load(flags + threadIdx.x, __ATOMIC_RELAXED, __HIP_MEMORY_SCOPE_AGENT);
+    __threadfence_system();
 }
 
 PartPlan make_part_plan(uint32_t k, uint64_t n_bytes, uint32_t slice_bits, uint32_t slice_index) {
@@ -685,7 +696,7 @@
 }
 
 int launch_partitioned(const PartPlan &pl, const PartBuffers &b, const L2 *st2, uint64_t n_bytes, uint32_t stride, const Carry *carry, uint8_t *table8,
-                       unsigned long long *hist, unsigned long long *hist_rep, bool fresh, const PartEvents &ev, hipStream_t s) {
+                       unsigned long long *hist, unsigned long long *hist_rep, bool fresh, const PartEvents &ev, const HostTail &to_host, hipStream_t s) {
     const uint32_t nfb = pl.B1 * pl.B2;
     const uint32_t *flags = b.flags;
     const char *failed = nullptr;
@@ -730,7 +741,8 @@
     else if (split) count(k_bucket_count_bytes<1024>, nfb, K6_BYTES_LDS);
     else count(k_bucket_count<1024>, n_rows6, lds6, pl.fb_bits, split);
     stage("bucket count");
-    hipLaunchKernelGGL(k_apply_side, dim3(AS_WGS), dim3(WG), 0, s, b.side, b.side_n, b.side_cap, table8, hist, hist_rep, flags);
+    hipLaunchKernelGGL(k_apply_side, dim3(AS_WGS), dim3(WG), 0, s, b.side, b.side_n, b.side_cap, table8, hist, hist_rep, b.flags, to_host,
+                       &b.signals->ticket[2]);
     stage("side list");
     return failed ? set_error(PK_ERR_HIP, std::string("partition pipeline: the launch of the ") + failed + " failed: " + hipGetErrorString(why)) : PK_OK;
 }
diff --git a/pykmer_amd/csrc/pk_api.hip b/pykmer_amd/csrc/pk_api.hip
--- a/pykmer_amd/csrc/pk_api.hip
+++ b/pykmer_amd/csrc/pk_api.hip
@@ -272,6 +272,7 @@
     struct Tail { Carry carry; unsigned long long hist[256]; FqCarry fq; };
     DevBuf<Tail> tail, tail0;
     struct Pinned { Tail tail; uint32_t flags[4]; } *pin = nullptr;
+    Pinned *pin_dev = nullptr;
     bool tail_on_host = false;
     bool zero_timed = true;
     DevBuf<unsigned long long> hist_rep;
@@ -318,14 +319,27 @@
     }
 };
 
+static const uint64_t RESET_KERNEL_MAX = 4ULL << 20;
+
 static int ix_reset(pk_indexer *ix) {
     HIPCHK(hipSetDevice(ix->device));
     HIPCHK(hipEventRecord(ix->ev.reset_begin, ix->stream));
-    HIPCHK(hipMemcpyAsync(ix->tail.p, ix->tail0.p, sizeof(pk_indexer::Tail), hipMemcpyDeviceToDevice, ix->stream));
+    static_assert(sizeof(pk_indexer::Tail) % 8 == 0, "k_reset and k_apply_side move the tail as 8-byte words");
+    ZeroSpans zero = {{ix->recs.p, ix->q_P.p, ix->q_hits.p, ix->q_depth.p}, {ix->recs.bytes, ix->q_P.bytes, ix->q_hits.bytes, ix->q_depth.bytes}};
+    uint64_t to_clear = 0;
+    for (int j = 0; j < 4; j++) {
+        if (!zero.p[j]) zero.bytes[j] = 0;
+        to_clear += zero.bytes[j];
+    }
+    if (to_clear <= RESET_KERNEL_MAX) {
+        launch_reset(ix->tail.p, ix->tail0.p, sizeof(pk_indexer::Tail), zero, ix->stream);
+        HIPCHK(hipGetLastError());
+    } else {
+        HIPCHK(hipMemcpyAsync(ix->tail.p, ix->tail0.p, sizeof(pk_indexer::Tail), hipMemcpyDeviceToDevice, ix->stream));
+        for (int j = 0; j < 4; j++)
+            if (zero.bytes[j]) HIPCHK(hipMemsetAsync(zero.p[j], 0, zero.bytes[j], ix->stream));
+    }
     ix->tail_on_host = false;
-    if (ix->recs.p) HIPCHK(hipMemsetAsync(ix->recs.p, 0, ix->recs.bytes, ix->stream));
-    for (DevBuf<unsigned long long> *b : {&ix->q_P, &ix->q_hits, &ix->q_depth})
-        if (b->p) HIPCHK(hipMemsetAsync(b->p, 0, b->bytes, ix->stream));
     ix->q_windows = ix->q_p_done = 0;
     HIPCHK(hipEventRecord(ix->ev.reset_end, ix->stream));
     ix->zero_timed = false;
@@ -347,13 +361,17 @@
     ix->zero_timed = true;
 }
 
-static int read_tail(pk_indexer *ix) {
-    HIPCHK(hipMemcpyAsync(&ix->pin->tail, ix->tail.p, sizeof(pk_indexer::Tail), hipMemcpyDeviceToHost, ix->stream));
+static int wait_tail(pk_indexer *ix) {
     HIPCHK(hipStreamSynchronize(ix->stream));
     HIPCHK(hipGetLastError());
     time_reset(ix);
     ix->tail_on_host = true;
     return PK_OK;
+}
+
+static int read_tail(pk_indexer *ix) {
+    HIPCHK(hipMemcpyAsync(&ix->pin->tail, ix->tail.p, sizeof(pk_indexer::Tail), hipMemcpyDeviceToHost, ix->stream));
+    return wait_tail(ix);
 }
 
 static void hist_with_zeros(const unsigned long long *h, uint64_t n, uint64_t hist256_out[256]) {
@@ -396,6 +414,7 @@
     if ((rc = ix->tail.reserve(sizeof(pk_indexer::Tail)))) return rc;
     if ((rc = ix->tail0.reserve(sizeof(pk_indexer::Tail)))) return rc;
     HIPCHK(hipHostMalloc(&ix->pin, sizeof(*ix->pin), hipHostMallocDefault));
+    HIPCHK(hipHostGetDevicePointer((void **)&ix->pin_dev, ix->pin, 0));
     {
         Carry c;
         memset(&c, 0, sizeof c);
@@ -484,6 +503,8 @@
     part_workspace(pl, n_bytes, ix->ws.p, &pb);
     Carry *carry = &ix->tail.p->carry;
     const Events &ev = ix->ev;
+    const HostTail to_host = {reinterpret_cast<const unsigned long long *>(ix->tail.p), reinterpret_cast<unsigned long long *>(&ix->pin_dev->tail),
+                              (uint32_t)(sizeof(pk_indexer::Tail) / 8), ix->pin_dev->flags};
     HIPCHK(hipEventRecord(ev.scan_begin, ix->stream));
     launch_chunk_l1(f, n_bytes, ix->c_l1.p, n_chunks, ix->stream);
     launch_scan_l1(ix->c_l1.p, n_chunks, carry, ix->c_l1s.p, ix->t_l1.p, pb.signals, ix->stream);
@@ -504,12 +525,11 @@
             HIPCHK(hipEventRecord(ev.squeeze_end, ix->stream));
         }
         if ((rc = launch_partitioned(pl, pb, ix->c_l2s.p, n_bytes, stride, carry, ix->table8.p, ix->tail.p->hist, ix->hist_rep.p, ix->table_fresh,
-                                     {ev.sort_begin, ev.sort_end, ev.part_end}, ix->stream)))
+                                     {ev.sort_begin, ev.sort_end, ev.part_end}, to_host, ix->stream)))
             return rc;
         HIPCHK(hipEventRecord(ev.bucket_end, ix->stream));
         volatile uint32_t *got = ix->pin->flags;
-        HIPCHK(hipMemcpyAsync(ix->pin->flags, pb.flags, sizeof ix->pin->flags, hipMemcpyDeviceToHost, ix->stream));
-        if ((rc = read_tail(ix))) return rc;
+        if ((rc = wait_tail(ix))) return rc;
         if (!got[0]) { ix->recounted += got[1]; break; }
         if (attempt >= 3) return fail(PK_ERR_HIP, "the feed's layout did not settle (internal error, flag %u)", got[0]);
         if (got[0] == 2u) {
diff --git a/pykmer_amd/csrc/pk_kernels.h b/pykmer_amd/csrc/pk_kernels.h
--- a/pykmer_amd/csrc/pk_kernels.h
+++ b/pykmer_amd/csrc/pk_kernels.h
@@ -15,7 +15,7 @@
 struct Carry {
     L2 l2;
     L1 l1;
-    uint32_t pad;
+    uint32_t ticket;
     uint64_t n_recs;
     uint64_t total_bp;
     uint64_t num_kmers;
@@ -25,7 +25,23 @@
 struct PartSignals {
     unsigned long long side_n;
     uint32_t flags[4];
+    uint32_t ticket[4];
 };
+
+__device__ __forceinline__ bool last_workgroup(uint32_t *ticket, uint32_t n_workgroups) {
+    __shared__ uint32_t drawn_last;
+    __threadfence();
+    __syncthreads();
+    if (threadIdx.x == 0) {
+        const uint32_t t = atomicAdd(ticket, 1u);
+        drawn_last = t + 1u == n_workgroups ? 1u : 0u;
+        if (drawn_last) *ticket = 0u;
+    }
+    __syncthreads();
+    const bool last = drawn_last != 0u;
+    if (last) __threadfence();
+    return last;
+}
 
 void launch_chunk_l1(const uint8_t *fasta, uint64_t n, L1 *chunk_l1, uint32_t n_chunks, hipStream_t s);
 void launch_scan_l1(const L1 *in, uint32_t n_chunks, Carry *carry, L1 *out, L1 *tile_ws, PartSignals *zeroed, hipStream_t s);
@@ -33,6 +49,8 @@
                      uint32_t k, hipStream_t s);
 void launch_scan_l2(const L2 *in, uint32_t n_chunks, Carry *carry, L2 *out, L2 *tile_ws, uint32_t k, hipStream_t s);
 void launch_hist8(const uint8_t *table8, uint64_t n, unsigned long long *hist, hipStream_t s);
+struct ZeroSpans { void *p[4]; uint64_t bytes[4]; };
+void launch_reset(void *copy_dst, const void *copy_src, uint64_t copy_bytes, const ZeroSpans &zero, hipStream_t s);
 
 constexpr uint32_t SLOT_CODE_WORDS = 1024;
 constexpr uint32_t SLOT_RST_WORDS = 512;
@@ -66,6 +84,7 @@
     PartSignals *signals;
     uint32_t *flags;
 };
+struct HostTail { const unsigned long long *src; unsigned long long *dst; uint32_t words; uint32_t *flags; };
 struct PartEvents { hipEvent_t sort_begin, sort_end, part_end; };
 PartPlan make_part_plan(uint32_t k, uint64_t n_bytes, uint32_t slice_bits, uint32_t slice_index);
 int part_plan_check(const PartPlan &pl, uint64_t n_bytes);
@@ -78,7 +97,7 @@
 void launch_provision(const PartPlan &pl, const PartBuffers &b, const L2 *st2, uint32_t stride, const Carry *carry, hipStream_t s);
 void launch_walk_sort(const PartPlan &pl, const PartBuffers &b, const L2 *st2, const Carry *carry, hipStream_t s);
 int launch_partitioned(const PartPlan &pl, const PartBuffers &b, const L2 *st2, uint64_t n_bytes, uint32_t stride, const Carry *carry, uint8_t *table8,
-                       unsigned long long *hist, unsigned long long *hist_rep, bool fresh, const PartEvents &ev, hipStream_t s);
+                       unsigned long long *hist, unsigned long long *hist_rep, bool fresh, const PartEvents &ev, const HostTail &to_host, hipStream_t s);
 
 constexpr uint32_t QUERY_MAX_TABLES = 16;
 struct QueryTables { const uint8_t *t[QUERY_MAX_TABLES]; };
```

Measured after the change: 213.4 billion bp/s. 1.5% lower.
